# sparisi/pvr_habitat

Hardware: AMD Instinct MI355X
Metric: frames/sec embedded (ResNet50, 256x256) (higher is better)
Workload: dtype f16

## Files before the change

### include/pvr_hip.h

```cpp
#ifndef PVR_HIP_H
#define PVR_HIP_H

#include <stddef.h>
#include <stdint.h>

#ifdef __cplusplus
extern "C" {
#endif

typedef int pvr_status;
#define PVR_OK 0
#define PVR_ERR_INVALID 1
#define PVR_ERR_MISSING_WEIGHT 2
#define PVR_ERR_HIP 3
#define PVR_ERR_STATE 4

#define PVR_BF16 0
#define PVR_F16 1
#define PVR_F32 2

#define PVR_ARCH_RESNET50 0
#define PVR_ARCH_RESNET50_L4 1
#define PVR_ARCH_RESNET50_L3 2
#define PVR_ARCH_CLIP_VIT_B32 3
#define PVR_ARCH_CLIP_VIT_B16 4
#define PVR_ARCH_RANDOM5 6
#define PVR_ARCH_MAE_VIT_L16 7
#define PVR_ARCH_MAE_VIT_H14 8
#define PVR_ARCH_CLIP_RN50 9
#define PVR_ARCH_RESNET18 10
#define PVR_ARCH_RESNET34 11
#define PVR_ARCH_MAE_VIT_B16 5

const char *pvr_version(void);
int32_t pvr_has_experiments(void);
int32_t pvr_debug_stem_u8_geometry_ok(const void *frames, int32_t h, int32_t w, int32_t top, int32_t left);
float pvr_debug_sample_uniform(uint32_t bits);
size_t pvr_last_error(char *buf, size_t cap);

typedef struct pvr_encoder pvr_encoder;

typedef struct pvr_encoder_desc {
    int32_t arch;
    int32_t dtype;
    int32_t max_batch;
    int32_t chunk;
    int32_t resize;
    int32_t crop;
    float mean[3];
    float std_[3];
} pvr_encoder_desc;

pvr_status pvr_encoder_create(const pvr_encoder_desc *desc, pvr_encoder **out);
pvr_status pvr_encoder_load_weights(pvr_encoder *enc, const char *name, const float *host_data,
                                    const int64_t *shape, int32_t ndim);
pvr_status pvr_encoder_finalize(pvr_encoder *enc);
pvr_status pvr_encoder_set_host_backend(pvr_encoder *enc, int32_t on);
int32_t pvr_encoder_out_size(const pvr_encoder *enc);
pvr_status pvr_encoder_forward(pvr_encoder *enc, const uint8_t *frames_dev, int32_t n, int32_t h,
                               int32_t w, float *out_dev, int64_t out_stride, void *hip_stream);
pvr_status pvr_encoder_tap(pvr_encoder *enc, const char *name, float *out_dev, int64_t cap,
                           int64_t *count, void *hip_stream);
pvr_status pvr_encoder_debug_set_fusion(pvr_encoder *enc, int32_t on);
int32_t pvr_encoder_launch_name(const pvr_encoder *enc, int32_t index, char *buf, int32_t cap);
pvr_status pvr_encoder_set_crop_position(pvr_encoder *enc, int32_t pos);
pvr_status pvr_encoder_forward_lane(pvr_encoder *enc, int32_t lane, const uint8_t *frames_dev, int32_t n, int32_t h,
                                    int32_t w, float *out_dev, int64_t out_stride, void *hip_stream);
pvr_status pvr_encoder_set_low_latency(pvr_encoder *enc, int32_t on);
pvr_status pvr_encoder_debug_stop_after(pvr_encoder *enc, const char *tap);
pvr_status pvr_encoder_profile(pvr_encoder *enc, const uint8_t *frames_dev, int32_t n, int32_t h, int32_t w,
                               float *out_dev, int64_t out_stride, void *hip_stream, float *op_ms,
                               double *op_flops, int32_t cap, int32_t *n_ops);
pvr_status pvr_encoder_profile_span(pvr_encoder *enc, const uint8_t *frames_dev, int32_t n, int32_t h, int32_t w, float *out_dev,
                                    int64_t out_stride, void *hip_stream, int32_t first_op, int32_t last_op, float *span_ms);
pvr_status pvr_encoder_check_range(pvr_encoder *enc, const uint8_t *frames_dev, int32_t n, int32_t h, int32_t w, float *out_dev, int64_t out_stride,
                                   void *hip_stream, int32_t *first_bad);
pvr_status pvr_encoder_debug_set_switch(pvr_encoder *enc, const char *name, int32_t value);
int32_t pvr_encoder_launch_kernel(const pvr_encoder *enc, int32_t n, int32_t index, char *buf, int32_t cap);
void pvr_encoder_destroy(pvr_encoder *enc);

pvr_status pvr_op_preprocess(const uint8_t *frames_dev, int32_t n, int32_t h, int32_t w, int32_t resize,
                             int32_t crop, void *out_dev, int32_t dtype, void *hip_stream);
pvr_status pvr_op_stem(const void *img_dev, const void *wgt_dev, const float *bias_dev, void *out_dev,
                       int32_t n, int32_t dtype, void *hip_stream);
pvr_status pvr_op_maxpool(const void *in_dev, void *out_dev, int32_t n, int32_t h, int32_t w, int32_t c,
                          int32_t dtype, void *hip_stream);
pvr_status pvr_op_conv2d(const void *in_dev, const void *wgt_dev, const float *bias_dev,
                         const void *residual_dev, void *out_dev, int32_t n, int32_t h, int32_t w,
                         int32_t cin, int32_t cout, int32_t kh, int32_t kw, int32_t stride, int32_t pad,
                         int32_t relu, int32_t out_f32, int32_t dtype, void *hip_stream);
pvr_status pvr_op_bneck_frame(const void *t1_dev, const void *w2_dev, const float *b2_dev, const void *w3_dev, const float *b3_dev,
                              const void *residual_dev, void *y_dev, void *t2_out_dev, const void *w1n_dev, const float *b1n_dev, void *t1n_dev,
                              const void *w1f_dev, const float *b1f_dev, int32_t n, int32_t phases, int32_t dtype, void *hip_stream);
pvr_status pvr_op_pack_frag_weights(const void *w_dev, void *out_dev, int32_t rows, int32_t k, void *hip_stream);
pvr_status pvr_debug_bneck_frame_stamps(const void *t1_dev, const void *w2_dev, const float *b2_dev, const void *w3_dev, const float *b3_dev,
                                        const void *residual_dev, void *y_dev, const void *w1n_dev, const float *b1n_dev, void *t1n_dev,
                                        const void *w1f_dev, const float *b1f_dev, int32_t n, int32_t dtype, uint64_t *stamps_dev, void *hip_stream);
int64_t pvr_debug_bneck_frame_launches(void);
pvr_status pvr_debug_set_frame64(int32_t mode);
int64_t pvr_debug_bneck_frame64_launches(void);
pvr_status pvr_debug_bneck_frame64_stamps(const void *w1f_dev, const float *b1f_dev, const void *w2_dev, const float *b2_dev, const void *w3_dev, const float *b3_dev,
                                          const void *x_dev, void *y_dev, int32_t n, int32_t dtype, uint64_t *stamps_dev, void *hip_stream);
pvr_status pvr_op_conv_wfrag(const void *in_dev, const void *wgt_packed_dev, const float *bias_dev, const void *residual_dev, void *out_dev, int32_t n,
                             int32_t h, int32_t w, int32_t cin, int32_t cout, int32_t kh, int32_t kw, int32_t stride, int32_t pad, int32_t relu,
                             int32_t out_f32, int32_t dtype, void *hip_stream);
pvr_status pvr_op_conv2d_dual(const void *in_dev, const void *in2_dev, const void *wgt_dev, const float *bias_dev, void *out_dev, int32_t n, int32_t h,
                              int32_t w, int32_t cin, int32_t cout, int32_t kh, int32_t kw, int32_t stride, int32_t pad, int32_t h2, int32_t w2,
                              int32_t cin2, int32_t stride2, int32_t relu, int32_t dtype, void *hip_stream);
pvr_status pvr_op_conv_wfrag_pool(const void *in_dev, const void *wgt_packed_dev, const float *bias_dev, const void *residual_dev, float *pool_out_dev,
                                  int64_t pool_stride, int32_t n, int32_t cin, int32_t cout, int32_t dtype, void *hip_stream);
int64_t pvr_debug_conv_wfrag_launches(void);
pvr_status pvr_op_split16_pack_weights(const float *w_dev, void *out_dev, int32_t rows, int32_t k, void *hip_stream);
pvr_status pvr_op_conv2d_split16(const float *in_dev, const void *wgt_split_dev, const float *bias_dev, const float *residual_dev, float *out_dev, int32_t n,
                                 int32_t h, int32_t w, int32_t cin, int32_t cout, int32_t k, int32_t stride, int32_t pad, int32_t relu, void *hip_stream);
pvr_status pvr_op_conv2d_f32(const float *in_dev, const float *wgt_dev, const float *bias_dev, const float *residual_dev, float *out_dev, int32_t n,
                             int32_t h, int32_t w, int32_t cin, int32_t cout, int32_t k, int32_t stride, int32_t pad, int32_t relu, void *hip_stream);
int64_t pvr_debug_conv_split16_launches(void);
int64_t pvr_debug_chain_wave128_launches(void);
pvr_status pvr_debug_set_stem_regpool(int32_t mode);
pvr_status pvr_debug_set_conv_algo(int32_t algo);
pvr_status pvr_file_sizes(const char *const *paths, int32_t n, int64_t *sizes, int32_t threads);
pvr_status pvr_read_files(const char *const *paths, int32_t n, uint8_t *dst, const int64_t *offsets, int32_t threads);
pvr_status pvr_stage_copy(void *dst, const void *src, int64_t rows, int64_t row_bytes, int64_t src_row_stride, int64_t run_bytes,
                          int64_t run_stride, int32_t threads);
int64_t pvr_png_scratch_bytes(int32_t n, int32_t h, int32_t w);
pvr_status pvr_png_decode(const uint8_t *files_dev, const int64_t *offsets_dev, int32_t n, int32_t h, int32_t w, uint8_t *out_dev,
                          uint8_t *scratch_dev, int64_t scratch_bytes, int32_t *status_dev, void *hip_stream);

int64_t pvr_debug_conv_expand_launches(void);
int64_t pvr_debug_pp_persistent_launches(void);
pvr_status pvr_op_avgpool(const void *in_dev, float *out_dev, int64_t out_stride, int32_t n, int32_t hw,
                          int32_t c, int32_t in_f32, int32_t dtype, void *hip_stream);
pvr_status pvr_op_nonfinite_flag(const float *x_dev, int64_t rows, int64_t cols, int64_t stride, int32_t *flag_dev, void *hip_stream);

pvr_status pvr_debug_convert(const float *src, uint16_t *dst, int64_t n, int32_t dtype);


#ifdef __cplusplus
}
#endif
#endif
```

### pvr_habitat_amd/_lib.py

```python
import ctypes as C
import os

_HERE = os.path.dirname(os.path.abspath(__file__))
LIB_PATH = os.environ.get('PVR_LIB') or os.path.join(_HERE, 'lib', 'libpvr_hip.so')

PVR_BF16, PVR_F16, PVR_F32 = 0, 1, 2
ARCH_RESNET50, ARCH_RESNET50_L4, ARCH_RESNET50_L3 = 0, 1, 2


class EncoderDesc(C.Structure):
    _fields_ = [('arch', C.c_int32), ('dtype', C.c_int32), ('max_batch', C.c_int32), ('chunk', C.c_int32),
                ('resize', C.c_int32), ('crop', C.c_int32), ('mean', C.c_float * 3), ('std_', C.c_float * 3)]


_lib = None

_SIGS = {
    'pvr_version': (C.c_char_p, []),
    'pvr_has_experiments': (C.c_int32, []),
    'pvr_debug_stem_u8_geometry_ok': (C.c_int32, [C.c_void_p, C.c_int32, C.c_int32, C.c_int32, C.c_int32]),
    'pvr_encoder_set_host_backend': (C.c_int, [C.c_void_p, C.c_int32]),
    'pvr_stage_copy': (C.c_int, [C.c_void_p, C.c_void_p, C.c_int64, C.c_int64, C.c_int64, C.c_int64, C.c_int64, C.c_int32]),
    'pvr_last_error': (C.c_size_t, [C.c_char_p, C.c_size_t]),
    'pvr_encoder_create': (C.c_int, [C.POINTER(EncoderDesc), C.POINTER(C.c_void_p)]),
    'pvr_encoder_load_weights': (C.c_int, [C.c_void_p, C.c_char_p, C.c_void_p, C.POINTER(C.c_int64), C.c_int32]),
    'pvr_encoder_finalize': (C.c_int, [C.c_void_p]),
    'pvr_encoder_out_size': (C.c_int32, [C.c_void_p]),
    'pvr_encoder_forward': (C.c_int, [C.c_void_p, C.c_void_p, C.c_int32, C.c_int32, C.c_int32, C.c_void_p, C.c_int64, C.c_void_p]),
    'pvr_encoder_forward_lane': (C.c_int, [C.c_void_p, C.c_int32, C.c_void_p, C.c_int32, C.c_int32, C.c_int32, C.c_void_p, C.c_int64, C.c_void_p]),
    'pvr_debug_set_conv_algo': (C.c_int, [C.c_int32]),
    'pvr_file_sizes': (C.c_int, [C.c_void_p, C.c_int32, C.c_void_p, C.c_int32]),
    'pvr_read_files': (C.c_int, [C.c_void_p, C.c_int32, C.c_void_p, C.c_void_p, C.c_int32]),
    'pvr_png_scratch_bytes': (C.c_int64, [C.c_int32, C.c_int32, C.c_int32]),
    'pvr_png_decode': (C.c_int, [C.c_void_p, C.c_void_p, C.c_int32, C.c_int32, C.c_int32, C.c_void_p, C.c_void_p, C.c_int64, C.c_void_p, C.c_void_p]),
    'pvr_debug_conv_expand_launches': (C.c_int64, []),
    'pvr_debug_pp_persistent_launches': (C.c_int64, []),
    'pvr_encoder_set_crop_position': (C.c_int, [C.c_void_p, C.c_int32]),
    'pvr_encoder_set_low_latency': (C.c_int, [C.c_void_p, C.c_int32]),
    'pvr_encoder_tap': (C.c_int, [C.c_void_p, C.c_char_p, C.c_void_p, C.c_int64, C.POINTER(C.c_int64), C.c_void_p]),
    'pvr_encoder_debug_stop_after': (C.c_int, [C.c_void_p, C.c_char_p]),
    'pvr_encoder_debug_set_fusion': (C.c_int, [C.c_void_p, C.c_int32]),
    'pvr_encoder_launch_name': (C.c_int32, [C.c_void_p, C.c_int32, C.c_char_p, C.c_int32]),
    'pvr_encoder_destroy': (None, [C.c_void_p]),
    'pvr_encoder_profile': (C.c_int, [C.c_void_p, C.c_void_p, C.c_int32, C.c_int32, C.c_int32, C.c_void_p, C.c_int64, C.c_void_p,
                                      C.c_void_p, C.c_void_p, C.c_int32, C.POINTER(C.c_int32)]),
    'pvr_encoder_profile_span': (C.c_int, [C.c_void_p, C.c_void_p, C.c_int32, C.c_int32, C.c_int32, C.c_void_p, C.c_int64, C.c_void_p, C.c_int32, C.c_int32,
                                           C.POINTER(C.c_float)]),
    'pvr_op_preprocess': (C.c_int, [C.c_void_p, C.c_int32, C.c_int32, C.c_int32, C.c_int32, C.c_int32, C.c_void_p, C.c_int32, C.c_void_p]),
    'pvr_op_stem': (C.c_int, [C.c_void_p, C.c_void_p, C.c_void_p, C.c_void_p, C.c_int32, C.c_int32, C.c_void_p]),
    'pvr_op_maxpool': (C.c_int, [C.c_void_p, C.c_void_p, C.c_int32, C.c_int32, C.c_int32, C.c_int32, C.c_int32, C.c_void_p]),
    'pvr_op_conv2d': (C.c_int, [C.c_void_p, C.c_void_p, C.c_void_p, C.c_void_p, C.c_void_p] + [C.c_int32] * 12 + [C.c_void_p]),
    'pvr_op_avgpool': (C.c_int, [C.c_void_p, C.c_void_p, C.c_int64, C.c_int32, C.c_int32, C.c_int32, C.c_int32, C.c_int32, C.c_void_p]),
    'pvr_debug_convert': (C.c_int, [C.c_void_p, C.c_void_p, C.c_int64, C.c_int32]),
    'pvr_op_bneck_frame': (C.c_int, [C.c_void_p] * 13 + [C.c_int32] * 3 + [C.c_void_p]),
    'pvr_debug_bneck_frame_launches': (C.c_int64, []),
    'pvr_debug_set_frame64': (C.c_int, [C.c_int32]),
    'pvr_debug_bneck_frame64_launches': (C.c_int64, []),
    'pvr_debug_bneck_frame64_stamps': (C.c_int, [C.c_void_p] * 8 + [C.c_int32] * 2 + [C.c_void_p] * 2),
    'pvr_op_conv_wfrag': (C.c_int, [C.c_void_p] * 5 + [C.c_int32] * 12 + [C.c_void_p]),
    'pvr_debug_conv_wfrag_launches': (C.c_int64, []),
    'pvr_op_conv_wfrag_pool': (C.c_int, [C.c_void_p] * 5 + [C.c_int64] + [C.c_int32] * 4 + [C.c_void_p]),
    'pvr_op_conv2d_dual': (C.c_int, [C.c_void_p] * 5 + [C.c_int32] * 15 + [C.c_void_p]),
    'pvr_op_pack_frag_weights': (C.c_int, [C.c_void_p, C.c_void_p, C.c_int32, C.c_int32, C.c_void_p]),
    'pvr_debug_bneck_frame_stamps': (C.c_int, [C.c_void_p] * 12 + [C.c_int32] * 2 + [C.c_void_p] * 2),
    'pvr_encoder_check_range': (C.c_int, [C.c_void_p, C.c_void_p, C.c_int32, C.c_int32, C.c_int32, C.c_void_p, C.c_int64, C.c_void_p, C.POINTER(C.c_int32)]),
    'pvr_encoder_debug_set_switch': (C.c_int, [C.c_void_p, C.c_char_p, C.c_int32]),
    'pvr_encoder_launch_kernel': (C.c_int32, [C.c_void_p, C.c_int32, C.c_int32, C.c_char_p, C.c_int32]),
    'pvr_op_split16_pack_weights': (C.c_int, [C.c_void_p, C.c_void_p, C.c_int32, C.c_int32, C.c_void_p]),
    'pvr_op_conv2d_split16': (C.c_int, [C.c_void_p] * 5 + [C.c_int32] * 9 + [C.c_void_p]),
    'pvr_op_conv2d_f32': (C.c_int, [C.c_void_p] * 5 + [C.c_int32] * 9 + [C.c_void_p]),
    'pvr_debug_conv_split16_launches': (C.c_int64, []),
    'pvr_debug_set_stem_regpool': (C.c_int, [C.c_int32]),
    'pvr_debug_chain_wave128_launches': (C.c_int64, []),
    'pvr_op_nonfinite_flag': (C.c_int, [C.c_void_p, C.c_int64, C.c_int64, C.c_int64, C.c_void_p, C.c_void_p]),
}


def lib():
    global _lib
    if _lib is None:
        if not os.path.isfile(LIB_PATH):
            raise RuntimeError('libpvr_hip.so not found at %s: build it with `make -C pvr_habitat_amd/csrc` '
                               '(there is no CPU fallback for the HIP path)' % LIB_PATH)
        l = C.CDLL(LIB_PATH)
        for name, (res, args) in _SIGS.items():
            if not hasattr(l, name):
                continue
            f = getattr(l, name)
            f.restype, f.argtypes = res, args
        _lib = l
    return _lib


def last_error():
    buf = C.create_string_buffer(1024)
    lib().pvr_last_error(buf, 1024)
    return buf.value.decode(errors='replace')


def check(status):
    if status != 0:
        raise RuntimeError('libpvr_hip: %s (status %d)' % (last_error(), status))


def stream_ptr():
    import torch
    return C.c_void_p(torch.cuda.current_stream().cuda_stream)


def require_gpu():
    import torch
    if not torch.cuda.is_available():
        raise RuntimeError('pvr_habitat_amd needs an MI355X (gfx950) visible to PyTorch-ROCm; there is no CPU path')
```

### pvr_habitat_amd/csrc/api.hip

```cpp
#include <stdarg.h>
#include "common.h"
#include "sample_rng.h"
#include <dlfcn.h>

namespace pvr {

static thread_local std::string g_err;

void set_error(const char *fmt, ...) {
    char buf[1024];
    va_list ap;
    va_start(ap, fmt);
    vsnprintf(buf, sizeof buf, fmt, ap);
    va_end(ap);
    g_err = buf;
}
const std::string &last_error() { return g_err; }

namespace {
typedef int (*roctx_push_fn)(const char *);
typedef int (*roctx_pop_fn)();
struct Roctx {
    roctx_push_fn push = nullptr;
    roctx_pop_fn pop = nullptr;
    Roctx() {
        const char *e = getenv("PVR_ROCTX");
        if (!e || atoi(e) == 0) return;
        for (const char *name : {"librocprofiler-sdk-roctx.so", "librocprofiler-sdk-roctx.so.1", "libroctx64.so", "libroctx64.so.4"}) {
            if (void *h = dlopen(name, RTLD_NOW | RTLD_GLOBAL)) {
                push = (roctx_push_fn)dlsym(h, "roctxRangePushA");
                pop = (roctx_pop_fn)dlsym(h, "roctxRangePop");
                if (push && pop) return;
                push = nullptr; pop = nullptr;
            }
        }
    }
};
const Roctx &roctx() { static Roctx r; return r; }
}
void trace_push(const char *name) { if (roctx().push) roctx().push(name); }
void trace_pop() { if (roctx().pop) roctx().pop(); }

pvr_status launch_preprocess(const uint8_t *, int, int, int, int, int, void *, int, hipStream_t, int crop_pos = 0);
pvr_status launch_stem(const void *, const void *, const float *, void *, int, int, int, hipStream_t);
pvr_status launch_maxpool(const void *, void *, int, int, int, int, int, hipStream_t);
pvr_status launch_avgpool(const void *, float *, int64_t, int, int, int, int, int, hipStream_t);
bool stem_pool_u8_ok(const void *, int, int, int, int);
pvr_status launch_conv(const void *, const void *, const float *, const void *, void *, const void *, int, int, int, int,
                       int, int, int, int, int, int, int, int, hipStream_t);

void set_conv_algo(int a);
long long conv_expand_launches();
long long bneck_frame_launches();
pvr_status launch_pack_frag_weights(const void *w, void *out, int rows, int K, hipStream_t stream);
pvr_status launch_bneck_frame(const void *t1, const void *w2, const float *b2, const void *w3, const float *b3, const void *res, void *y,
                              void *t2_out, int n, int phases, int dtype, hipStream_t stream, unsigned long long *stamps = nullptr,
                              const void *w1np = nullptr, const float *b1n = nullptr, void *t1n = nullptr, const void *w1fp = nullptr, const float *b1f = nullptr);
pvr_status launch_bneck_frame64(const void *w1p, const float *b1, const void *w2p, const float *b2, const void *w3p, const float *b3, const void *x, void *y, int n,
                                int dtype, hipStream_t stream, unsigned long long *stamps);
void set_frame64(int mode);
long long bneck_frame64_launches();
long long pp_persistent_launches();
pvr_status launch_conv_pp256(const void *in, const void *wgt, const float *bias, const void *res, void *out, int n, int h, int w, int cin,
                             int cout, int kh, int kw, int stride, int pad, int act, int out_f32, int res_f32, int dtype, int bm, hipStream_t stream,
                             const void *in2 = nullptr, int h2 = 0, int w2 = 0, int cin2 = 0, int stride2 = 1);
long long conv_wfrag_launches();
pvr_status launch_conv_wfrag(const void *in, const void *wp, const float *bias, const void *res, void *out, int n, int h, int w, int cin, int cout,
                             int kh, int kw, int stride, int pad, int act, int out_f32, int dtype, hipStream_t stream, float *pool_out = nullptr,
                             int64_t pool_stride = 0);

void set_stem_regpool(int v);
long long conv_split16_launches();
long long chain_wave128_launches();
pvr_status launch_split16_pack(const float *w, void *out, int rows, int K, hipStream_t stream);
pvr_status launch_conv_split16(const float *in, const void *wsp, const float *bias, const float *res, float *out, int n, int h, int w, int cin,
                               int cout, int k, int stride, int pad, int relu, hipStream_t stream, float *out2 = nullptr, int n1 = 0, void *out16 = nullptr,
                               int terms = 3);
pvr_status launch_conv_f32(const float *, const float *, const float *, const float *, float *, int, int, int, int, int, int, int, int, int, hipStream_t);

static void *g_zero = nullptr;
static pvr_status zero_page(void **out) {
    if (!g_zero) {
        PVR_HIP_TRY(hipMalloc(&g_zero, 256));
        PVR_HIP_TRY(hipMemset(g_zero, 0, 256));
        PVR_HIP_TRY(hipDeviceSynchronize());
    }
    *out = g_zero;
    return PVR_OK;
}

}

using namespace pvr;

extern "C" {

const char *pvr_version(void) { return "pvr_hip 0.1.0 (gfx950)"; }

int64_t pvr_debug_conv_expand_launches(void) { return (int64_t)conv_expand_launches(); }
int64_t pvr_debug_bneck_frame_launches(void) { return (int64_t)bneck_frame_launches(); }
pvr_status pvr_op_pack_frag_weights(const void *w, void *out, int32_t rows, int32_t k, void *stream) {
    return launch_pack_frag_weights(w, out, rows, k, (hipStream_t)stream);
}

pvr_status pvr_op_bneck_frame(const void *t1, const void *w2, const float *b2, const void *w3, const float *b3, const void *residual, void *y,
                              void *t2_out, const void *w1n, const float *b1n, void *t1n, const void *w1f, const float *b1f, int32_t n, int32_t phases,
                              int32_t dtype, void *stream) {
    PVR_REQUIRE(n > 0 && n <= 1300, "pvr_op_bneck_frame: n must be 1..1300");
    return launch_bneck_frame(t1, w2, b2, w3, b3, residual, y, t2_out, n, phases, dtype, (hipStream_t)stream, nullptr, w1n, b1n, t1n, w1f, b1f);
}
pvr_status pvr_debug_bneck_frame_stamps(const void *t1, const void *w2, const float *b2, const void *w3, const float *b3, const void *residual, void *y,
                                        const void *w1n, const float *b1n, void *t1n, const void *w1f, const float *b1f, int32_t n, int32_t dtype,
                                        uint64_t *stamps_dev, void *stream) {
    PVR_REQUIRE(stamps_dev && n > 8, "pvr_debug_bneck_frame_stamps: needs a stamp buffer and more than 8 frames");
    return launch_bneck_frame(t1, w2, b2, w3, b3, residual, y, nullptr, n, (w1n ? 7 : 3) | (w1f ? 8 : 0), dtype, (hipStream_t)stream, (unsigned long long *)stamps_dev,
                              w1n, b1n, t1n, w1f, b1f);
}
pvr_status pvr_debug_set_frame64(int32_t mode) {
    PVR_REQUIRE(mode >= -1 && mode <= 1, "pvr_debug_set_frame64: -1 (environment: PVR_FRAME64, default off), 0 or 1");
    set_frame64(mode);
    return PVR_OK;
}
int64_t pvr_debug_bneck_frame64_launches(void) { return (int64_t)bneck_frame64_launches(); }
pvr_status pvr_debug_bneck_frame64_stamps(const void *w1f, const float *b1f, const void *w2, const float *b2, const void *w3, const float *b3, const void *x, void *y,
                                          int32_t n, int32_t dtype, uint64_t *stamps_dev, void *stream) {
    PVR_REQUIRE(stamps_dev && n > 8, "pvr_debug_bneck_frame64_stamps: needs a stamp buffer and more than 8 frames");
    return launch_bneck_frame64(w1f, b1f, w2, b2, w3, b3, x, y, n, dtype, (hipStream_t)stream, (unsigned long long *)stamps_dev);
}
pvr_status pvr_op_conv_wfrag(const void *in, const void *wgt_packed, const float *bias, const void *residual, void *out, int32_t n, int32_t h, int32_t w,
                             int32_t cin, int32_t cout, int32_t kh, int32_t kw, int32_t stride, int32_t pad, int32_t relu, int32_t out_f32, int32_t dtype,
                             void *stream) {
    PVR_REQUIRE(n > 0 && h > 0 && w > 0, "pvr_op_conv_wfrag: empty input");
    return launch_conv_wfrag(in, wgt_packed, bias, residual, out, n, h, w, cin, cout, kh, kw, stride, pad, relu, out_f32, dtype, (hipStream_t)stream);
}
pvr_status pvr_op_conv2d_dual(const void *in, const void *in2, const void *wgt, const float *bias, void *out, int32_t n, int32_t h, int32_t w, int32_t cin,
                              int32_t cout, int32_t kh, int32_t kw, int32_t stride, int32_t pad, int32_t h2, int32_t w2, int32_t cin2, int32_t stride2,
                              int32_t relu, int32_t dtype, void *stream) {
    PVR_REQUIRE(in && in2 && wgt && bias && out && n > 0, "pvr_op_conv2d_dual: null argument");
    PVR_REQUIRE(dtype == PVR_BF16 || dtype == PVR_F16, "pvr_op_conv2d_dual: 16-bit storage types only");
    return launch_conv_pp256(in, wgt, bias, nullptr, out, n, h, w, cin, cout, kh, kw, stride, pad, relu, 0, 0, dtype, 224, (hipStream_t)stream, in2, h2, w2,
                             cin2, stride2);
}
pvr_status pvr_op_conv_wfrag_pool(const void *in, const void *wgt_packed, const float *bias, const void *residual, float *pool_out, int64_t pool_stride,
                                  int32_t n, int32_t cin, int32_t cout, int32_t dtype, void *stream) {
    PVR_REQUIRE(n > 0 && pool_out, "pvr_op_conv_wfrag_pool: empty input");
    return launch_conv_wfrag(in, wgt_packed, bias, residual, nullptr, n, 7, 7, cin, cout, 1, 1, 1, 0, 1, 1, dtype, (hipStream_t)stream, pool_out, pool_stride);
}
int64_t pvr_debug_conv_wfrag_launches(void) { return (int64_t)conv_wfrag_launches(); }
pvr_status pvr_op_split16_pack_weights(const float *w, void *out, int32_t rows, int32_t k, void *stream) {
    return launch_split16_pack(w, out, rows, k, (hipStream_t)stream);
}
pvr_status pvr_op_conv2d_split16(const float *in, const void *wgt_split, const float *bias, const float *residual, float *out, int32_t n, int32_t h,
                                 int32_t w, int32_t cin, int32_t cout, int32_t k, int32_t stride, int32_t pad, int32_t relu, void *stream) {
    PVR_REQUIRE(n > 0 && h > 0 && w > 0, "pvr_op_conv2d_split16: empty input");
    return launch_conv_split16(in, wgt_split, bias, residual, out, n, h, w, cin, cout, k, stride, pad, relu, (hipStream_t)stream);
}
pvr_status pvr_op_conv2d_f32(const float *in, const float *wgt, const float *bias, const float *residual, float *out, int32_t n, int32_t h, int32_t w,
                             int32_t cin, int32_t cout, int32_t k, int32_t stride, int32_t pad, int32_t relu, void *stream) {
    PVR_REQUIRE(in && wgt && bias && out && n > 0, "pvr_op_conv2d_f32: null argument");
    return launch_conv_f32(in, wgt, bias, residual, out, n, h, w, cin, cout, k, stride, pad, relu, (hipStream_t)stream);
}
int64_t pvr_debug_conv_split16_launches(void) { return (int64_t)conv_split16_launches(); }
pvr_status pvr_debug_set_stem_regpool(int32_t mode) {
    PVR_REQUIRE(mode >= -1 && mode <= 1, "pvr_debug_set_stem_regpool: -1 (environment: PVR_STEM_REGPOOL, default on), 0 (LDS-tile pooling) or 1 (register pooling)");
    set_stem_regpool(mode);
    return PVR_OK;
}
int64_t pvr_debug_chain_wave128_launches(void) { return (int64_t)chain_wave128_launches(); }
int64_t pvr_debug_pp_persistent_launches(void) { return (int64_t)pp_persistent_launches(); }

size_t pvr_last_error(char *buf, size_t cap) {
    const std::string &e = last_error();
    if (buf && cap) {
        size_t n = e.size() < cap - 1 ? e.size() : cap - 1;
        memcpy(buf, e.data(), n);
        buf[n] = 0;
    }
    return e.size();
}

pvr_status pvr_op_preprocess(const uint8_t *frames, int32_t n, int32_t h, int32_t w, int32_t resize, int32_t crop,
                             void *out, int32_t dtype, void *stream) {
    PVR_REQUIRE(frames && out, "pvr_op_preprocess: null pointer");
    hipStream_t st = (hipStream_t)stream;
    PVR_HIP_TRY(hipMemsetAsync(out, 0, (size_t)n * (crop + 6) * (crop + 8) * 4 * 2, st));
    return launch_preprocess(frames, n, h, w, resize, crop, out, dtype, st);
}

pvr_status pvr_op_stem(const void *img, const void *wgt, const float *bias, void *out, int32_t n, int32_t dtype,
                       void *stream) {
    PVR_REQUIRE(img && wgt && bias && out, "pvr_op_stem: null pointer");
    return launch_stem(img, wgt, bias, out, n, 224, dtype, (hipStream_t)stream);
}

pvr_status pvr_op_maxpool(const void *in, void *out, int32_t n, int32_t h, int32_t w, int32_t c, int32_t dtype,
                          void *stream) {
    PVR_REQUIRE(in && out, "pvr_op_maxpool: null pointer");
    return launch_maxpool(in, out, n, h, w, c, dtype, (hipStream_t)stream);
}

pvr_status pvr_op_conv2d(const void *in, const void *wgt, const float *bias, const void *residual, void *out, int32_t n,
                         int32_t h, int32_t w, int32_t cin, int32_t cout, int32_t kh, int32_t kw, int32_t stride,
                         int32_t pad, int32_t relu, int32_t out_f32, int32_t dtype, void *stream) {
    PVR_REQUIRE(in && wgt && bias && out, "pvr_op_conv2d: null pointer");
    void *z;
    pvr_status s = zero_page(&z);
    if (s) return s;
    return launch_conv(in, wgt, bias, residual, out, z, n, h, w, cin, cout, kh, kw, stride, pad, relu, out_f32, dtype,
                       (hipStream_t)stream);
}

pvr_status pvr_debug_set_conv_algo(int32_t algo) {
    PVR_REQUIRE(algo >= -1 && algo <= 4, "pvr_debug_set_conv_algo: algo must be -1 (auto), 0 (conv_igemm), 1 / 2 / 3 (conv_pp256 with 256- / 128- / 224-pixel tiles), 4 (conv_w4)");
#ifndef PVR_EXPERIMENTS
    PVR_REQUIRE(algo != 4, "pvr_debug_set_conv_algo: conv_w4 is an experiment kernel; this library was built without it (make EXPERIMENTS=1)");
#endif
    set_conv_algo(algo);
    return PVR_OK;
}

pvr_status pvr_op_avgpool(const void *in, float *out, int64_t out_stride, int32_t n, int32_t hw, int32_t c, int32_t in_f32,
                          int32_t dtype, void *stream) {
    PVR_REQUIRE(in && out, "pvr_op_avgpool: null pointer");
    return launch_avgpool(in, out, out_stride, n, hw, c, in_f32, dtype, (hipStream_t)stream);
}

__global__ __launch_bounds__(256) void nonfinite_flag_kernel(const float *x, long long rows, long long cols, long long stride, int *flag) {
    const long long n = rows * cols;
    bool bad = false;
    for (long long i = (long long)blockIdx.x * 256 + threadIdx.x; i < n; i += (long long)gridDim.x * 256) {
        const float v = x[(i / cols) * stride + (i % cols)];
        bad |= (__builtin_bit_cast(unsigned, v) & 0x7f800000u) == 0x7f800000u;
    }
    if (__builtin_amdgcn_ballot_w64(bad) != 0 && (threadIdx.x & 63) == 0) atomicOr(flag, 1);
}

pvr_status pvr_op_nonfinite_flag(const float *x, int64_t rows, int64_t cols, int64_t stride, int32_t *flag, void *stream) {
    PVR_REQUIRE(x && flag && rows >= 0 && cols > 0 && stride >= cols, "pvr_op_nonfinite_flag: bad argument");
    if (rows == 0) return PVR_OK;
    const long long n = rows * cols;
    const int blocks = (int)((n + 255) / 256 < 2048 ? (n + 255) / 256 : 2048);
    hipLaunchKernelGGL(nonfinite_flag_kernel, dim3(blocks), dim3(256), 0, (hipStream_t)stream, x, (long long)rows, (long long)cols, (long long)stride, flag);
    PVR_LAUNCH_CHECK();
    return PVR_OK;
}

int32_t pvr_debug_stem_u8_geometry_ok(const void *frames, int32_t h, int32_t w, int32_t top, int32_t left) { return stem_pool_u8_ok(frames, h, w, top, left) ? 1 : 0; }

float pvr_debug_sample_uniform(uint32_t bits) { return pvr::uniform_open01(bits); }

int32_t pvr_has_experiments(void) {
#ifdef PVR_EXPERIMENTS
    return 1;
#else
    return 0;
#endif
}

pvr_status pvr_debug_convert(const float *src, uint16_t *dst, int64_t n, int32_t dtype) {
    PVR_REQUIRE(src && dst, "pvr_debug_convert: null pointer");
    for (int64_t i = 0; i < n; ++i) dst[i] = f32_to_h(src[i], dtype);
    return PVR_OK;
}

}
```

### pvr_habitat_amd/csrc/bottleneck_chain.hip

```cpp
#include "chain_params.h"

namespace pvr {


__device__ __forceinline__ void ch_dma16(__amdgpu_buffer_rsrc_t rs, char *lds, int voff, int soff) {
    __builtin_amdgcn_raw_ptr_buffer_load_lds(rs, (__attribute__((address_space(3))) void *)lds, 16, voff, soff, 0, 0);
}

#ifdef CHAIN_STAMP
__device__ unsigned long long chain_stamps[8192][12];
#define CH_T(i_) { if (threadIdx.x == 0) ch_tt[i_] = __builtin_amdgcn_s_memrealtime(); }
#else
#define CH_T(i_)
#endif

#ifndef CH_KNOCK
#define CH_KNOCK 0
#endif
template <int AUX = 0>
__device__ __forceinline__ void store_b128_imm(u32x4 v, __amdgpu_buffer_rsrc_t rs, int voff, int imm) {
    if constexpr (!(CH_KNOCK & 1)) __builtin_amdgcn_raw_buffer_store_b128(v, rs, voff + imm, 0, AUX);
}

template <int CM, int CMN, bool F16, int RD, int OCC, bool HALO, bool DS = false, int PFK = -1>
// ... 273 lines not shown
        for (int j = 0; j < TM; ++j) {
            const int row = wm * 64 + j * 16 + fr;
            const f32x4 a = acc2[i][j];
            const unsigned lo = pack2_h<F16>(fmaxf(a[0] + bv.x, 0.f), fmaxf(a[1] + bv.y, 0.f));
            const unsigned hi = pack2_h<F16>(fmaxf(a[2] + bv.z, 0.f), fmaxf(a[3] + bv.w, 0.f));
            const int cc = c & 63;
            char *dst = smem + T2_OFF + (c >> 6) * 16384 + row * 128 + ((((cc >> 3) ^ ((row >> 1) & 7))) << 4) + (cc & 4) * 2;
            *reinterpret_cast<uint2 *>(dst) = make_uint2(lo, hi);
        }
    }
#pragma unroll
    for (int i = 0; i < W3_CH; ++i) *reinterpret_cast<u32x4 *>(smem + W3_L(i)) = w3r[i];
    if constexpr (CMN > 0) {
#pragma unroll
        for (int i = 0; i < W1_CH; ++i) *reinterpret_cast<u32x4 *>(smem + W1_L(i)) = w1r[i];
    }
    if (G > 1) {
#pragma unroll
        for (int i = 0; i < W3_CH; ++i)
            w3r[i] = __builtin_bit_cast(u32x4, __builtin_amdgcn_raw_buffer_load_b128(rs_w3, W3_G(i), 64 * CM * 2, 0));
        if constexpr (CMN > 0) {
#pragma unroll
            for (int i = 0; i < W1_CH; ++i) w1r[i] = __builtin_bit_cast(u32x4, __builtin_amdgcn_raw_buffer_load_b128(rs_w1, W1_G(i), 128, 0));
        }
    }
    __syncthreads();
    CH_T(3);

    int w3_rd[2][2], w1_rd[2][CMN ? TN1 : 1], yg_wr[TM];
#pragma unroll
    for (int ks = 0; ks < 2; ++ks) {
#pragma unroll
        for (int t = 0; t < 2; ++t) {
            const int row = wn * 32 + t * 16 + fr;
            w3_rd[ks][t] = W3_OFF + row * 128 + (((ks * 4 + fq) ^ ((row >> 1) & 7)) << 4);
        }
        if constexpr (CMN > 0) {
#pragma unroll
            for (int i = 0; i < TN1; ++i) {
                const int row = wn * (CMN / 2) + i * 16 + fr;
                w1_rd[ks][i] = W1_OFF + row * 128 + (((ks * 4 + fq) ^ ((row >> 1) & 7)) << 4);
            }
        }
    }
#pragma unroll
    for (int j = 0; j < TM; ++j) {
        const int row = wm * 64 + j * 16 + fr;
        yg_wr[j] = YG_OFF + row * 128 + (((wn * 4 + fq) ^ ((row >> 1) & 7)) << 4);
    }
    f32x4 acc1[CMN ? TN1 : 1][TM];
    if constexpr (CMN > 0) {
#pragma unroll
        for (int i = 0; i < TN1; ++i)
#pragma unroll
            for (int j = 0; j < TM; ++j) acc1[i][j] = f32x4{0.f, 0.f, 0.f, 0.f};
    }

#pragma unroll
    for (int g = 0; g < G; ++g) {
        if (g == 1) CH_T(6);
        f32x4 acc3[2][TM];
#pragma unroll
        for (int t = 0; t < 2; ++t)
#pragma unroll
            for (int j = 0; j < TM; ++j) acc3[t][j] = f32x4{0.f, 0.f, 0.f, 0.f};
#pragma unroll
        for (int s = 0; s < KS3; ++s)
#pragma unroll
            for (int ks = 0; ks < 2; ++ks) {
                V8 xa[TM], wb[2];
#pragma unroll
                for (int j = 0; j < TM; ++j) xa[j] = *reinterpret_cast<const V8 *>(smem + T2_OFF + s * 16384 + x_rd[ks][j]);
#pragma unroll
                for (int t = 0; t < 2; ++t) wb[t] = *reinterpret_cast<const V8 *>(smem + s * 8192 + w3_rd[ks][t]);
#pragma unroll
                for (int t = 0; t < 2; ++t)
#pragma unroll
                    for (int j = 0; j < TM; ++j) acc3[t][j] = mfma16<F16>(wb[t], xa[j], acc3[t][j]);
            }
        if constexpr (DS) {
#pragma unroll
            for (int ks = 0; ks < 2; ++ks)
#pragma unroll
                for (int t = 0; t < 2; ++t)
#pragma unroll
                    for (int j = 0; j < TM; ++j) acc3[t][j] = mfma16<F16>(wdr[t][ks], xd[ks][j], acc3[t][j]);
            if (g + 1 < G) {
#pragma unroll
                for (int t = 0; t < 2; ++t)
#pragma unroll
                    for (int ks = 0; ks < 2; ++ks)
                        wdr[t][ks] = __builtin_bit_cast(V8, __builtin_amdgcn_raw_buffer_load_b128(rs_wd, wd_off[t] + ks * 64, (g + 1) * 8192, 0));
            }
        }
        if (g == 1) CH_T(7);
        const int c0 = g * 64 + wn * 32 + fq * 8;
        const float4 bA = *reinterpret_cast<const float4 *>(p.b3 + c0), bB = *reinterpret_cast<const float4 *>(p.b3 + c0 + 4);
#pragma unroll
        for (int j = 0; j < TM; ++j) {
            const f32x4 lo = acc3[0][j], hi = acc3[1][j];
            float v[8] = {lo[0] + bA.x, lo[1] + bA.y, lo[2] + bA.z, lo[3] + bA.w, hi[0] + bB.x, hi[1] + bB.y, hi[2] + bB.z, hi[3] + bB.w};
            u32x4 o;
            if constexpr (DS) {
#pragma unroll
                for (int e = 0; e < 4; ++e)
                    o[e] = pack2_h<F16>(fmaxf(v[2 * e], 0.f), fmaxf(v[2 * e + 1], 0.f));
            } else {
                const u32x4 r = rres[g % RD][j];
#pragma unroll
                for (int e = 0; e < 4; ++e) {
                    const float v0 = fmaxf(v[2 * e] + from_h<F16>((u16)(r[e] & 0xffffu)), 0.f);
                    const float v1 = fmaxf(v[2 * e + 1] + from_h<F16>((u16)(r[e] >> 16)), 0.f);
                    o[e] = pack2_h<F16>(v0, v1);
                }
            }
            if (p.y_blk) store_b128_imm<PVR_NT_AUX(4)>(o, rs_y, Y_OFF(j) + g * y_gs, 0);
            else store_b128_imm(o, rs_y, Y_OFF(j) + g * y_gs, 0);
            if constexpr (CMN > 0) *reinterpret_cast<u32x4 *>(smem + yg_wr[j]) = o;
        }
        if (!DS && g + RD < G) {
#pragma unroll
            for (int j = 0; j < TM; ++j)
                rres[g % RD][j] = __builtin_bit_cast(u32x4, __builtin_amdgcn_raw_buffer_load_b128(rs_res, (CH_KNOCK & 2) ? OOB : R_OFF(j), (g + RD) * r_gs, DS ? 0 : PVR_NT_AUX(16)));
        }
        if (g == 1) CH_T(8);
        __syncthreads();
        if (g == 1) CH_T(9);
        if (g + 1 < G) {
#pragma unroll
            for (int i = 0; i < W3_CH; ++i) *reinterpret_cast<u32x4 *>(smem + W3_L(i)) = w3r[i];
            if (g + 2 < G) {
#pragma unroll
                for (int i = 0; i < W3_CH; ++i)
                    w3r[i] = __builtin_bit_cast(u32x4, __builtin_amdgcn_raw_buffer_load_b128(rs_w3, W3_G(i), (g + 2) * (64 * CM * 2), 0));
            }
        }
        if (g == 1) CH_T(10);
        if constexpr (CMN == 0) __syncthreads();
        if constexpr (CMN > 0) {
#pragma unroll
            for (int ks = 0; ks < 2; ++ks) {
                V8 xa[TM], wb[TN1];
#pragma unroll
                for (int j = 0; j < TM; ++j) xa[j] = *reinterpret_cast<const V8 *>(smem + YG_OFF + x_rd[ks][j]);
#pragma unroll
                for (int i = 0; i < TN1; ++i) wb[i] = *reinterpret_cast<const V8 *>(smem + w1_rd[ks][i]);
#pragma unroll
                for (int i = 0; i < TN1; ++i)
#pragma unroll
                    for (int j = 0; j < TM; ++j) acc1[i][j] = mfma16<F16>(wb[i], xa[j], acc1[i][j]);
            }
            __syncthreads();
            if (g == 1) CH_T(11);
            if (g + 1 < G) {
#pragma unroll
                for (int i = 0; i < W1_CH; ++i) *reinterpret_cast<u32x4 *>(smem + W1_L(i)) = w1r[i];
                if (g + 2 < G) {
#pragma unroll
                    for (int i = 0; i < W1_CH; ++i)
                        w1r[i] = __builtin_bit_cast(u32x4, __builtin_amdgcn_raw_buffer_load_b128(rs_w1, W1_G(i), (g + 2) * 128, 0));
                }
            }
        }
    }

    CH_T(4);
    if constexpr (CMN > 0) {
#pragma unroll
        for (int q = 0; q < TN1 / 2; ++q) {
            const int c0 = wn * (CMN / 2) + q * 32 + fq * 8;
            const float4 bA = *reinterpret_cast<const float4 *>(p.b1n + c0), bB = *reinterpret_cast<const float4 *>(p.b1n + c0 + 4);
#pragma unroll
            for (int j = 0; j < TM; ++j) {
                const f32x4 lo = acc1[2 * q][j], hi = acc1[2 * q + 1][j];
                const float v[8] = {lo[0] + bA.x, lo[1] + bA.y, lo[2] + bA.z, lo[3] + bA.w, hi[0] + bB.x, hi[1] + bB.y, hi[2] + bB.z, hi[3] + bB.w};
                u32x4 o;
#pragma unroll
                for (int e = 0; e < 4; ++e)
                    o[e] = pack2_h<F16>(fmaxf(v[2 * e], 0.f), fmaxf(v[2 * e + 1], 0.f));
                if (p.t_blk) store_b128_imm<0>(o, rs_t, T_OFF(j) + q * 1024, 0);
                else store_b128_imm<PVR_NT_AUX(8)>(o, rs_t, T_OFF(j), q * 64);
            }
        }
    }
#undef PVR_PHASE_B_PREFETCH
#undef W3_G
#undef W3_L
#undef W1_G
#undef W1_L
#undef Y_OFF
#undef R_OFF
#undef T_OFF
#ifdef CHAIN_STAMP
    CH_T(5);
    if (threadIdx.x == 0 && blockIdx.x < 8192) { _Pragma("unroll") for (int k = 0; k < 12; ++k) chain_stamps[blockIdx.x][k] = ch_tt[k]; }
#endif
}

template <int CM, int CMN, bool F16, int RD, int OCC, bool HALO, bool DS = false, int PFK = -1>
static pvr_status launch_chain_one(ChainP &p, hipStream_t stream) {
    const int grid = (p.M + 127) / 128;
    const size_t pipe = HALO ? (size_t)(CM / 64) * (CM == 64 ? 256 : 192) * 128 + (size_t)2 * CM * 128 : (size_t)2 * (128 + CM) * 128;
    const size_t phase_b = (CM / 64) * 16384 + 16384 + (CM / 64) * 8192 + CMN * 128;
    const size_t lds = phase_b <= pipe ? pipe : phase_b;
    static DeviceOnce attr_done;
    if (attr_done.needed()) {
        PVR_HIP_TRY(hipFuncSetAttribute((const void *)bottleneck_chain_kernel<CM, CMN, F16, RD, OCC, HALO, DS, PFK>,
                                        hipFuncAttributeMaxDynamicSharedMemorySize, (int)lds));
        attr_done.mark();
    }
    hipLaunchKernelGGL((bottleneck_chain_kernel<CM, CMN, F16, RD, OCC, HALO, DS, PFK>), dim3(grid), dim3(256), lds, stream, p);
    PVR_LAUNCH_CHECK();
    return PVR_OK;
}

static bool chain_halo_enabled() {
    static int v = -1;
    if (v < 0) { const char *e = getenv("PVR_CHAIN_HALO"); v = e ? atoi(e) : 1; }
    return v != 0;
}

static int chain_ds_occ() {
    static int v = -1;
    if (v < 0) { const char *e = getenv("PVR_CHAIN_DS_OCC"); v = e ? atoi(e) : 3; }
    return v;
}

static int chain_pfk() {
    static int v = -2;
    if (v < -1) { const char *e = getenv("PVR_CHAIN_PFK"); v = e ? atoi(e) : 12; }
    return v;
}

template <int CM, int CMN, bool F16, int RD, int OCC, bool DS = false>
static pvr_status launch_chain_inst(ChainP &p, hipStream_t stream) {
    const bool halo = p.stride == 1 && 128 + 2 * p.W + 2 <= (CM == 64 ? 256 : 192) - 1 && chain_halo_enabled();
    if constexpr (DS) {
        if (halo) return chain_ds_occ() == 3 ? launch_chain_one<CM, CMN, F16, RD, 3, true, true>(p, stream) : launch_chain_one<CM, CMN, F16, RD, 2, true, true>(p, stream);
        return launch_chain_one<CM, CMN, F16, RD, 2, false, true>(p, stream);
    } else {
        if (halo) {
            if constexpr (CM == 128) {
                if (chain_pfk() == 12) return launch_chain_one<CM, CMN, F16, RD, 2, true, false, 12>(p, stream);
            }
            return launch_chain_one<CM, CMN, F16, RD, (CM == 64 ? OCC : 2), true>(p, stream);
        }
        return launch_chain_one<CM, CMN, F16, RD, OCC, false>(p, stream);
    }
}

static int chain_cfg() {
    static int v = -1;
    if (v < 0) { const char *e = getenv("PVR_CHAIN_CFG"); v = e ? atoi(e) : 12; }
    return v;
}

template <bool F16>
static pvr_status launch_chain_dt(ChainP &p, int cm, int cmn, hipStream_t stream) {
    if (p.xds) {
        if (cm == 64 && cmn == 64) return launch_chain_inst<64, 64, F16, 1, 2, true>(p, stream);
        set_error("bottleneck chain with downsample: no instance for Cm=%d, next Cm=%d", cm, cmn);
        return PVR_ERR_INVALID;
    }
    const int cfg = chain_cfg();
#define PVR_CHAIN64(CMN_)                                                                 \
    switch (cfg) {                                                                        \
    case 12: return launch_chain_inst<64, CMN_, F16, 1, 2>(p, stream);                    \
    case 13: return launch_chain_inst<64, CMN_, F16, 1, 3>(p, stream);                    \
    case 22: return launch_chain_inst<64, CMN_, F16, 2, 2>(p, stream);                    \
    case 23: return launch_chain_inst<64, CMN_, F16, 2, 3>(p, stream);                    \
    default: return launch_chain_inst<64, CMN_, F16, 4, 2>(p, stream);                    \
    }
    if (cm == 64 && cmn == 64) PVR_CHAIN64(64)
    if (cm == 64 && cmn == 128) {
        if (cfg / 10 == 1) return launch_chain_inst<64, 128, F16, 1, 2>(p, stream);
        if (cfg / 10 == 2) return launch_chain_inst<64, 128, F16, 2, 2>(p, stream);
        return launch_chain_inst<64, 128, F16, 4, 2>(p, stream);
    }
    if (cm == 64 && cmn == 0) PVR_CHAIN64(0)
#undef PVR_CHAIN64
    if (cm == 128 && cmn == 128) return launch_chain_inst<128, 128, F16, 1, 2>(p, stream);
    if (cm == 128 && cmn == 0) return launch_chain_inst<128, 0, F16, 1, 2>(p, stream);
    set_error("bottleneck chain: no instance for Cm=%d, next Cm=%d", cm, cmn);
    return PVR_ERR_INVALID;
}

static bool chain_wave_enabled() {
    const char *e = getenv("PVR_CHAIN_WAVE");
    return !e || atoi(e) != 0;
}

bool chain_uses_wave_form(int cm, int cmn, int stride, bool ds) { return chain_wave_enabled() && chain_wave_supported(cm, cmn, stride, ds); }

bool chain_uses_wave128(int cm, int cmn, int stride, int64_t M) { return chain_wave_enabled() && chain_wave128_supported(cm, cmn, stride, M); }

bool chain_ds_supported(int cm, int cmn, int cin, int stride) { return cm == 64 && cmn == 64 && cin == 64 && stride == 1; }
bool chain_supported(int cm, int cmn) { return (cm == 64 && (cmn == 0 || cmn == 64 || cmn == 128)) || (cm == 128 && (cmn == 0 || cmn == 128)); }

int chain_row_source(int row) { return (row & ~31) + 8 * ((row >> 2) & 3) + 4 * ((row >> 4) & 1) + (row & 3); }

pvr_status launch_bottleneck_chain(const void *t1, const void *w2, const float *b2, const void *w3p, const float *b3, const void *res,
                                   void *y, const void *w1np, const float *b1n, void *t1n, int n, int h, int w, int cm, int cmn,
                                   int stride, int dtype, hipStream_t stream, const void *xds, const void *wdsp, const void *w3pb, const void *wdspb,
                                   int wave, int in_blk, int out_blk, const void *wpk) {
    PVR_REQUIRE(chain_supported(cm, cmn), "bottleneck chain: unsupported widths Cm=%d next=%d", cm, cmn);
    PVR_REQUIRE(t1 && w2 && b2 && w3p && b3 && (res || xds) && y && (cmn == 0 || (w1np && b1n && t1n)), "bottleneck chain: null argument");
    PVR_REQUIRE(!xds || (wdsp && chain_ds_supported(cm, cmn, 64, stride)), "bottleneck chain with downsample: unsupported shape");
    ChainP p;
    p.in = (const u16 *)t1; p.w2 = (const u16 *)w2; p.w3 = (const u16 *)w3p; p.w1n = (const u16 *)w1np; p.res = (const u16 *)res;
    p.b2 = b2; p.b3 = b3; p.b1n = b1n; p.y = (u16 *)y; p.t1n = (u16 *)t1n;
    p.N = n; p.H = h; p.W = w; p.stride = stride;
    p.Ho = (h + 2 - 3) / stride + 1; p.Wo = (w + 2 - 3) / stride + 1;
    const int64_t M = (int64_t)n * p.Ho * p.Wo;
    const int64_t inb = (int64_t)n * h * w * cm * 2, yb = M * 4 * cm * 2, tb = M * (cmn ? cmn : 1) * 2;
    PVR_REQUIRE(inb < 0x7ffffff0ll && yb < 0x7ffffff0ll && tb < 0x7ffffff0ll, "bottleneck chain: operand larger than 2 GiB (use a smaller chunk)");
    p.M = (int)M; p.in_bytes = (unsigned)inb; p.y_bytes = (unsigned)yb; p.t1n_bytes = (unsigned)tb;
    p.xds = (const u16 *)xds; p.wds = (const u16 *)wdsp;
    p.xds_bytes = xds ? (unsigned)(M * 64 * 2) : 0; p.wds_bytes = xds ? (unsigned)(4 * cm * 64 * 2) : 0;
    p.w2_bytes = (unsigned)(cm * 9 * cm * 2); p.w3_bytes = (unsigned)(4 * cm * cm * 2); p.w1n_bytes = (unsigned)(cmn * 4 * cm * 2);
    if (wave == 2) {
        PVR_REQUIRE(chain_wave128_supported(cm, cmn, stride, M) && !xds, "bottleneck chain: no layer2 wave form for Cm=%d next=%d stride=%d", cm, cmn, stride);
        p.wpk = (const u16 *)wpk; p.in_blk = in_blk; p.out_blk = out_blk & 1;
        return launch_chain_wave128(p, cmn, dtype, stream);
    }
    if (wave) {
        PVR_REQUIRE(chain_wave_supported(cm, cmn, stride, xds != nullptr), "bottleneck chain: no wave form for Cm=%d next=%d stride=%d", cm, cmn, stride);
        p.w3b = (const u16 *)w3pb; p.wdsb = (const u16 *)wdspb; p.in_blk = in_blk; p.out_blk = out_blk;
        return launch_chain_wave(p, cmn, dtype, stream);
    }
    PVR_REQUIRE(!(in_blk || out_blk) || M % 16 == 0, "bottleneck chain: the blocked layout needs a multiple of 16 pixels");
    p.res_blk = xds ? 0 : in_blk; p.y_blk = out_blk & 1;
    p.t_blk = (out_blk & 2) && cmn > 0;
    return dtype == PVR_F16 ? launch_chain_dt<true>(p, cm, cmn, stream) : launch_chain_dt<false>(p, cm, cmn, stream);
}

}
```

### pvr_habitat_amd/csrc/chain_params.h

```cpp
#pragma once
#include "common.h"

namespace pvr {

struct ChainP {
    const u16 *in, *w2, *w3, *w1n, *res;
    const float *b2, *b3, *b1n;
    u16 *y, *t1n;
    int N, H, W, Ho, Wo, stride, M;
    unsigned in_bytes, w2_bytes, w3_bytes, w1n_bytes, y_bytes, t1n_bytes;
    const u16 *xds = nullptr, *wds = nullptr;
    unsigned xds_bytes = 0, wds_bytes = 0;
    int in_blk = 0, out_blk = 0;
    int res_blk = 0, y_blk = 0;
    const u16 *w3b = nullptr, *wdsb = nullptr;
    const u16 *wpk = nullptr;
    unsigned wpk_bytes = 0;
    int t_blk = 0;
};

bool chain_supported(int cm, int cmn);
bool chain_ds_supported(int cm, int cmn, int cin, int stride);
bool chain_uses_wave_form(int cm, int cmn, int stride, bool ds);
int chain_row_source(int row);
pvr_status launch_bottleneck_chain(const void *t1, const void *w2, const float *b2, const void *w3p, const float *b3, const void *res,
                                   void *y, const void *w1np, const float *b1n, void *t1n, int n, int h, int w, int cm, int cmn,
                                   int stride, int dtype, hipStream_t stream, const void *xds = nullptr, const void *wdsp = nullptr,
                                   const void *w3pb = nullptr, const void *wdspb = nullptr, int wave = 0, int in_blk = 0, int out_blk = 0,
                                   const void *wpk = nullptr);


bool chain_wave_supported(int cm, int cmn, int stride, bool ds);
bool chain_wave_blocked_ok(int cmn_first, int h, int w);
bool chain_wave_halo_enabled();
pvr_status launch_chain_wave(ChainP &p, int cmn, int dtype, hipStream_t stream);

bool chain_wave128_supported(int cm, int cmn, int stride, int64_t M);
bool chain_uses_wave128(int cm, int cmn, int stride, int64_t M);
size_t chain_wave128_pack_bytes();
pvr_status launch_chain_wave128_pack(const void *w2, const void *w3p, const void *w1np, void *out, hipStream_t stream);
pvr_status launch_chain_wave128(ChainP &p, int cmn, int dtype, hipStream_t stream);

}
```

### pvr_habitat_amd/csrc/chain_wave.hip

```cpp
#include "chain_params.h"

namespace pvr {

__device__ __forceinline__ int cw_row_source(int row) { return (row & ~31) + 8 * ((row >> 2) & 3) + 4 * ((row >> 4) & 1) + (row & 3); }

#ifndef CW_KNOCK
#define CW_KNOCK 0
#endif
#ifndef CW_AUX_ST
#define CW_AUX_ST PVR_NT_AUX(1)
#endif
#ifndef CW_AUX_RES
#define CW_AUX_RES PVR_NT_AUX(2)
#endif
template <int AUX = CW_AUX_ST>
__device__ __forceinline__ void cw_store(u32x4 v, __amdgpu_buffer_rsrc_t rs, int voff, int imm, int never = 0) {
    if constexpr (CW_KNOCK & 1) { if (never) __builtin_amdgcn_raw_buffer_store_b128(v, rs, voff + imm, 0, AUX); }
    else __builtin_amdgcn_raw_buffer_store_b128(v, rs, voff + imm, 0, AUX);
}
#ifndef CW_AUX_T1
#define CW_AUX_T1 CW_AUX_ST
#endif

typedef float cw_f32x2 __attribute__((ext_vector_type(2)));
typedef __bf16 cw_bf16x2 __attribute__((ext_vector_type(2)));
typedef _Float16 cw_f16x2 __attribute__((ext_vector_type(2)));
template <bool F16> __device__ __forceinline__ unsigned cw_pack2(float a, float b) {
    const cw_f32x2 v = {a, b};
    if constexpr (F16) return __builtin_bit_cast(unsigned, __builtin_convertvector(v, cw_f16x2));
    else return __builtin_bit_cast(unsigned, __builtin_convertvector(v, cw_bf16x2));
}

__device__ __forceinline__ u32x4 cw_m2f(char *slot, int lane, int foff, u32x4 v) {
    *reinterpret_cast<u32x4 *>(slot + lane * 16) = v;
    return *reinterpret_cast<const u32x4 *>(slot + foff);
}
__device__ __forceinline__ void cw_f2m_pair(char *slot, int lane, u32x4 even, u32x4 odd, u32x4 &lo, u32x4 &hi) {
    const int fr = lane & 15, fq = lane >> 4, base = fr * 128, sw = fr & 7;
    *reinterpret_cast<u32x4 *>(slot + base + ((fq ^ sw) << 4)) = even;
    *reinterpret_cast<u32x4 *>(slot + base + (((4 + fq) ^ sw) << 4)) = odd;
    lo = *reinterpret_cast<const u32x4 *>(slot + lane * 16);
    hi = *reinterpret_cast<const u32x4 *>(slot + 1024 + lane * 16);
}

__device__ __forceinline__ unsigned cw_row_shift(unsigned lo, unsigned hi, int d) {
#define CW_SH(D_) case D_: { const int a_ = __builtin_amdgcn_update_dpp(0, (int)lo, 0x100 + D_, 0xf, 0xf, true); \
                             return (unsigned)__builtin_amdgcn_update_dpp(a_, (int)hi, 0x110 + (16 - D_), 0xf, 0xf, false); }
    switch (d) {
        CW_SH(1) CW_SH(2) CW_SH(3) CW_SH(4) CW_SH(5) CW_SH(6) CW_SH(7) CW_SH(8) CW_SH(9) CW_SH(10) CW_SH(11) CW_SH(12) CW_SH(13) CW_SH(14) CW_SH(15)
        default: return lo;
    }
#undef CW_SH
}

struct CwTile {
    int xb[2];
    int mk[2];
    int yi[2];
    int yo[2];
    int to[2];
    int hb;
    int xs[2];
};

template <int CMN, bool INB, bool OUTB>
__device__ __forceinline__ void cw_setup(CwTile &a, int m0, int lane, int M, int H, int W) {
    const int fr = lane & 15, fq = lane >> 4, lp = lane >> 2, lc = (lane & 3) ^ ((lane >> 3) & 3);
    a.hb = ((m0 >> 4) - 4) * 2048 + fq * 256 + fr * 16;
#pragma unroll
    for (int j = 0; j < 2; ++j) {
        const int m = m0 + 16 * j + (INB ? fr : lp);
        const bool ok = m < M;
        const int mm = ok ? m : 0;
        const int wo = mm % W, ho = (mm / W) % H;
        int hb = 0, wb = 0;
#pragma unroll
        for (int t3 = 0; t3 < 3; ++t3) {
            hb |= (int)(ok && (unsigned)(ho - 1 + t3) < (unsigned)H) << t3;
            wb |= (int)((unsigned)(wo - 1 + t3) < (unsigned)W) << t3;
        }
        int mask = 0;
#pragma unroll
        for (int t3 = 0; t3 < 3; ++t3) mask |= ((hb >> t3) & 1) ? (wb << (t3 * 3)) : 0;
        a.mk[j] = mask;
        a.xb[j] = INB ? m : m * 128 + lc * 16;
        a.xs[j] = (m0 + 16 * j + lp) * 128 + lc * 16;
        const int blk = (m0 >> 4) + j;
        a.yi[j] = INB ? blk * 8192 + fq * 256 + fr * 16 : (m0 + 16 * j + lp) * 512 + lc * 16;
        a.yo[j] = OUTB ? blk * 8192 + fq * 256 + fr * 16 : (m0 + 16 * j + (lane >> 3)) * 512 + (((lane & 7) ^ (lane >> 3)) << 4);
        a.to[j] = OUTB ? blk * (CMN * 32) + fq * 256 + fr * 16 : (m0 + 16 * j + (lane >> 3)) * (CMN * 2) + (((lane & 7) ^ (lane >> 3)) << 4);
    }
}

template <int CMN, bool F16, bool DS, bool W3G, bool INB, bool OUTB, bool HALO, int XD, int RD, int WD>
__global__ __launch_bounds__(512, 2) void chain_wave_kernel(ChainP p) {
    typedef typename HT<F16>::V8 V8;
    constexpr int WW = 56, HB = 10;
    constexpr int NH = 8, NK = 18;
    constexpr int TN1 = CMN / 16;
    constexpr int W2L = 0, W3L = 73728, W1L = W3G ? 73728 : 73728 + 32768;
    constexpr int B2L = W1L + CMN * 512, B3L = B2L + 256, B1L = B3L + 1024, SCR = B1L + 512;
    constexpr int OOB = 0x7ffffff0;
    constexpr int YH = INB ? 1024 : 64;
    static_assert(XD >= 1 && XD <= NK && RD >= 1 && RD <= NH && NH % RD == 0 && WD >= 1 && WD <= NH, "prefetch depths (the residual ring must close over a tile)");
    static_assert(!HALO || INB, "the halo form reads the blocked layout");
    extern __shared__ __attribute__((aligned(16))) char smem[];

    const int tid = threadIdx.x, lane = tid & 63, wave = tid >> 6, fr = lane & 15, fq = lane >> 4;
    const int foff = fr * 64 + ((fq ^ ((fr >> 1) & 3)) << 4);
    char *const slot0 = smem + SCR + wave * 2048, *const slot1 = slot0 + 1024;
    const auto rs_in = __builtin_amdgcn_make_buffer_rsrc(const_cast<u16 *>(p.in), 0, p.in_bytes, 0x00020000);
    const auto rs_w2 = __builtin_amdgcn_make_buffer_rsrc(const_cast<u16 *>(p.w2), 0, p.w2_bytes, 0x00020000);
    const auto rs_w3 = __builtin_amdgcn_make_buffer_rsrc(const_cast<u16 *>(p.w3), 0, p.w3_bytes, 0x00020000);
    const auto rs_w1 = __builtin_amdgcn_make_buffer_rsrc(const_cast<u16 *>(p.w1n), 0, p.w1n_bytes, 0x00020000);
    const auto rs_res = __builtin_amdgcn_make_buffer_rsrc(const_cast<u16 *>(DS ? p.xds : p.res), 0, DS ? p.xds_bytes : p.y_bytes, 0x00020000);
    const auto rs_wd = __builtin_amdgcn_make_buffer_rsrc(const_cast<u16 *>(DS ? p.wdsb : p.w3b), 0, DS ? p.wds_bytes : p.w3_bytes, 0x00020000);
    const auto rs_y = __builtin_amdgcn_make_buffer_rsrc(p.y, 0, p.y_bytes, 0x00020000);
    const auto rs_t = __builtin_amdgcn_make_buffer_rsrc(p.t1n, 0, p.t1n_bytes, 0x00020000);

#pragma unroll
    for (int q = 0; q < 9; ++q) {
        const int r = tid >> 3, c = tid & 7;
        const u32x4 v = __builtin_bit_cast(u32x4, __builtin_amdgcn_raw_buffer_load_b128(rs_w2, (cw_row_source(r) * 576 + c * 8) * 2, q * 128, 0));
        *reinterpret_cast<u32x4 *>(smem + W2L + q * 8192 + r * 128 + ((c ^ ((r >> 1) & 7)) << 4)) = v;
    }
    if constexpr (!W3G) {
#pragma unroll
        for (int q = 0; q < 4; ++q) {
            const int idx = tid + 512 * q, r = idx >> 3, c = idx & 7;
            const u32x4 v = __builtin_bit_cast(u32x4, __builtin_amdgcn_raw_buffer_load_b128(rs_w3, idx * 16, 0, 0));
            *reinterpret_cast<u32x4 *>(smem + W3L + r * 128 + ((c ^ ((r >> 1) & 7)) << 4)) = v;
        }
    }
    if constexpr (CMN > 0) {
#pragma unroll
        for (int q = 0; q < CMN * 32 / 512; ++q) {
            const int idx = tid + 512 * q, r = idx >> 5, c32 = idx & 31;
            const u32x4 v = __builtin_bit_cast(u32x4, __builtin_amdgcn_raw_buffer_load_b128(rs_w1, idx * 16, 0, 0));
            *reinterpret_cast<u32x4 *>(smem + W1L + (c32 >> 3) * (CMN * 128) + r * 128 + (((c32 & 7) ^ ((r >> 1) & 7)) << 4)) = v;
        }
    }
    if (tid < 64) *reinterpret_cast<float *>(smem + B2L + tid * 4) = p.b2[tid];
    if (tid < 256) *reinterpret_cast<float *>(smem + B3L + tid * 4) = p.b3[tid];
    if constexpr (CMN > 0) { if (tid < CMN) *reinterpret_cast<float *>(smem + B1L + tid * 4) = p.b1n[tid]; }
    __syncthreads();

    const int nch = (p.M + 255) >> 8, cx = (nch + 7) >> 3, L = gridDim.x >> 3;
    const int xcd = blockIdx.x & 7, c_end = min((xcd + 1) * cx, nch);
    int chunk = xcd * cx + (blockIdx.x >> 3);
    if (chunk >= c_end) return;

    int lb0 = fr * 128 + ((fq ^ ((fr >> 1) & 7)) << 4), lb1 = lb0 ^ 64;
    const int Wb = p.W * 128;

    CwTile cur, nxt;
    cw_setup<CMN, INB, OUTB>(cur, chunk * 256 + wave * 32, lane, p.M, p.H, p.W);

    u32x4 xr[HALO ? 1 : XD][2];
    u32x4 xh[HALO ? HB : 1][2];
    u32x4 rres[DS ? 1 : RD][2];
    V8 xd[2][2];
    u32x4 wg[(W3G || DS) ? WD : 1][2][2];
#define CW_ISSUE_X(slot_, kt_, A_)                                                                                      \
    {                                                                                                                   \
        const int tp_ = (kt_) >> 1;                                                                                     \
        _Pragma("unroll") for (int j = 0; j < 2; ++j) {                                                                 \
            int vo_;                                                                                                    \
            if constexpr (INB) {                                   \
                const int pm_ = A_.xb[j] + (tp_ / 3 - 1) * p.W + (tp_ % 3 - 1);                                         \
                vo_ = (pm_ >> 4) * 2048 + (pm_ & 15) * 16 + (((kt_) & 1) * 4 + fq) * 256;                               \
            } else vo_ = A_.xb[j] + (tp_ / 3 - 1) * Wb + (tp_ % 3 - 1) * 128 + ((kt_) & 1) * 64;                        \
            vo_ = ((A_.mk[j] >> tp_) & 1) ? vo_ : OOB;                                                                  \
            if constexpr (CW_KNOCK & 4) vo_ = OOB;                                                                      \
            xr[slot_][j] = __builtin_bit_cast(u32x4, __builtin_amdgcn_raw_buffer_load_b128(rs_in, vo_, 0, 0));          \
        }                                                                                                               \
    }
#define CW_ISSUE_HALO(A_)                                                                                               \
    {                                                                                                                   \
        _Pragma("unroll") for (int k = 0; k < HB; ++k)                                                                  \
            _Pragma("unroll") for (int ks = 0; ks < 2; ++ks)                                                            \
                xh[k][ks] = __builtin_bit_cast(u32x4, __builtin_amdgcn_raw_buffer_load_b128(rs_in, (CW_KNOCK & 4) ? OOB : A_.hb + k * 2048 + ks * 1024, 0, 0)); \
    }
#define CW_FRAG(dst_, kt_, j_)                                                                                          \
    {                                                                                                                   \
        const int tp_ = (kt_) >> 1, ks_ = (kt_) & 1, o_ = 64 + 16 * (j_) + (tp_ / 3 - 1) * WW + tp_ % 3 - 1, k0_ = o_ >> 4, d_ = o_ & 15; \
        const bool in_ = (cur.mk[j_] >> tp_) & 1;                                                                       \
        _Pragma("unroll") for (int e = 0; e < 4; ++e) {                                                                 \
            const unsigned v_ = cw_row_shift(xh[k0_][ks_][e], xh[k0_ + 1 < HB ? k0_ + 1 : k0_][ks_][e], d_);            \
            dst_[e] = in_ ? v_ : 0u;                                                                                    \
        }                                                                                                               \
    }
#define CW_ISSUE_RES(slot_, h_, A_)                                                                                     \
    {                                                                                                                   \
        _Pragma("unroll") for (int j = 0; j < 2; ++j)                                                                   \
            rres[slot_][j] = __builtin_bit_cast(u32x4, __builtin_amdgcn_raw_buffer_load_b128(rs_res, (CW_KNOCK & 2) ? OOB : A_.yi[j], (h_) * YH, CW_AUX_RES)); \
    }
#define CW_ISSUE_WG(slot_, h_)                                                                                          \
    {                                                                                                                   \
        _Pragma("unroll") for (int t = 0; t < 2; ++t)                                                                   \
            _Pragma("unroll") for (int ks = 0; ks < 2; ++ks)                                                            \
                wg[slot_][t][ks] = __builtin_bit_cast(u32x4, __builtin_amdgcn_raw_buffer_load_b128(rs_wd, wg_off + t * 2048 + ks * 1024, (h_) * 4096, 0)); \
    }
    const int wg_off = fq * 256 + fr * 16;

    if constexpr (HALO) CW_ISSUE_HALO(cur)
    else {
#pragma unroll
        for (int k = 0; k < XD; ++k) CW_ISSUE_X(k, k, cur);
    }
    if constexpr (!DS) {
#pragma unroll
        for (int d = 0; d < RD; ++d) CW_ISSUE_RES(d, d, cur);
    }

    for (;;) {
        const int chunk_n = chunk + L;
        const bool more = chunk_n < c_end;
        asm volatile("" : "+v"(lb0), "+v"(lb1));

        u32x4 xdr[2][2];
        if constexpr (DS) {
#pragma unroll
            for (int ks = 0; ks < 2; ++ks)
#pragma unroll
                for (int j = 0; j < 2; ++j)
                    xdr[ks][j] = __builtin_bit_cast(u32x4, __builtin_amdgcn_raw_buffer_load_b128(rs_res, cur.xs[j], ks * 64, 0));
        }

        f32x4 acc2[4][2];
#pragma unroll
        for (int i = 0; i < 4; ++i)
#pragma unroll
            for (int j = 0; j < 2; ++j) acc2[i][j] = f32x4{0.f, 0.f, 0.f, 0.f};
        u32x4 xc[2], xn[2];
        if constexpr (HALO) { CW_FRAG(xc[0], 0, 0); CW_FRAG(xc[1], 0, 1); }
        else {
#pragma unroll
            for (int j = 0; j < 2; ++j) xc[j] = INB ? xr[0][j] : cw_m2f(j ? slot1 : slot0, lane, foff, xr[0][j]);
            if (XD < NK) CW_ISSUE_X(0, XD, cur);
        }
#pragma unroll
        for (int kt = 0; kt < NK; ++kt) {
            if (kt + 1 < NK) {
                if constexpr (HALO) { CW_FRAG(xn[0], kt + 1, 0); CW_FRAG(xn[1], kt + 1, 1); }
                else {
#pragma unroll
                    for (int j = 0; j < 2; ++j) xn[j] = INB ? xr[(kt + 1) % XD][j] : cw_m2f(j ? slot1 : slot0, lane, foff, xr[(kt + 1) % XD][j]);
                    if (kt + 1 + XD < NK) CW_ISSUE_X((kt + 1) % XD, kt + 1 + XD, cur);
                }
            }
            const char *wbase = smem + W2L + (kt >> 1) * 8192 + ((kt & 1) ? lb1 : lb0);
            V8 wb[4];
#pragma unroll
            for (int i = 0; i < 4; ++i) wb[i] = *reinterpret_cast<const V8 *>(wbase + i * 2048);
#pragma unroll
            for (int i = 0; i < 4; ++i) {
                acc2[i][0] = mfma16<F16>(wb[i], __builtin_bit_cast(V8, xc[0]), acc2[i][0]);
                acc2[i][1] = mfma16<F16>(wb[i], __builtin_bit_cast(V8, xc[1]), acc2[i][1]);
            }
            if (kt + 1 < NK) { xc[0] = xn[0]; xc[1] = xn[1]; }
            __builtin_amdgcn_sched_barrier(0);
        }
        u32x4 t2[2][2];
#pragma unroll
        for (int q = 0; q < 2; ++q) {
            const float4 bA = *reinterpret_cast<const float4 *>(smem + B2L + (32 * q + 8 * fq) * 4);
            const float4 bB = *reinterpret_cast<const float4 *>(smem + B2L + (32 * q + 8 * fq + 4) * 4);
#pragma unroll
            for (int j = 0; j < 2; ++j) {
                const f32x4 lo = acc2[2 * q][j], hi = acc2[2 * q + 1][j];
                const float v[8] = {lo[0] + bA.x, lo[1] + bA.y, lo[2] + bA.z, lo[3] + bA.w, hi[0] + bB.x, hi[1] + bB.y, hi[2] + bB.z, hi[3] + bB.w};
                u32x4 o;
#pragma unroll
                for (int e = 0; e < 4; ++e)
                    o[e] = cw_pack2<F16>(fmaxf(v[2 * e], 0.f), fmaxf(v[2 * e + 1], 0.f));
                t2[q][j] = o;
            }
        }

        cw_setup<CMN, INB, OUTB>(nxt, more ? chunk_n * 256 + wave * 32 : ((p.M + 31) & ~31), lane, p.M, p.H, p.W);
        if (!more) nxt.hb = OOB;
        if constexpr (HALO) CW_ISSUE_HALO(nxt)
        else {
#pragma unroll
            for (int k = 0; k < XD; ++k) CW_ISSUE_X(k, k, nxt);
        }
        if constexpr (W3G || DS) {
#pragma unroll
            for (int d = 0; d < WD; ++d) CW_ISSUE_WG(d, d);
        }
        if constexpr (DS) {
#pragma unroll
            for (int ks = 0; ks < 2; ++ks)
#pragma unroll
                for (int j = 0; j < 2; ++j) xd[ks][j] = __builtin_bit_cast(V8, cw_m2f(j ? slot1 : slot0, lane, foff, xdr[ks][j]));
        }

        f32x4 acc1[CMN ? TN1 : 1][2];
        if constexpr (CMN > 0) {
#pragma unroll
            for (int i = 0; i < TN1; ++i)
#pragma unroll
                for (int j = 0; j < 2; ++j) acc1[i][j] = f32x4{0.f, 0.f, 0.f, 0.f};
        }
        u32x4 oe[2];
#pragma unroll
        for (int h = 0; h < NH; ++h) {
            u32x4 rp[2], wp[2][2];
            if constexpr (!DS) {
#pragma unroll
                for (int j = 0; j < 2; ++j) rp[j] = INB ? rres[h % RD][j] : cw_m2f(j ? slot1 : slot0, lane, foff, rres[h % RD][j]);
                if (h + RD < NH) CW_ISSUE_RES(h % RD, h + RD, cur)
                else CW_ISSUE_RES(h % RD, h + RD - NH, nxt)
            }
            if constexpr (W3G || DS) {
#pragma unroll
                for (int t = 0; t < 2; ++t)
#pragma unroll
                    for (int ks = 0; ks < 2; ++ks) wp[t][ks] = wg[h % WD][t][ks];
                if (h + WD < NH) CW_ISSUE_WG(h % WD, h + WD);
            }
            f32x4 acc3[2][2];
#pragma unroll
            for (int t = 0; t < 2; ++t)
#pragma unroll
                for (int j = 0; j < 2; ++j) acc3[t][j] = f32x4{0.f, 0.f, 0.f, 0.f};
#pragma unroll
            for (int ks = 0; ks < 2; ++ks) {
                V8 wb[2];
#pragma unroll
                for (int t = 0; t < 2; ++t) {
                    if constexpr (W3G) wb[t] = __builtin_bit_cast(V8, wp[t][ks]);
                    else wb[t] = *reinterpret_cast<const V8 *>(smem + W3L + h * 4096 + t * 2048 + (ks ? lb1 : lb0));
                }
#pragma unroll
                for (int t = 0; t < 2; ++t)
#pragma unroll
                    for (int j = 0; j < 2; ++j) acc3[t][j] = mfma16<F16>(wb[t], __builtin_bit_cast(V8, t2[ks][j]), acc3[t][j]);
            }
            if constexpr (DS) {
#pragma unroll
                for (int ks = 0; ks < 2; ++ks)
#pragma unroll
                    for (int t = 0; t < 2; ++t)
#pragma unroll
                        for (int j = 0; j < 2; ++j) acc3[t][j] = mfma16<F16>(__builtin_bit_cast(V8, wp[t][ks]), xd[ks][j], acc3[t][j]);
            }
            const float4 bA = *reinterpret_cast<const float4 *>(smem + B3L + (32 * h + 8 * fq) * 4);
            const float4 bB = *reinterpret_cast<const float4 *>(smem + B3L + (32 * h + 8 * fq + 4) * 4);
            u32x4 o[2];
#pragma unroll
            for (int j = 0; j < 2; ++j) {
                const f32x4 lo = acc3[0][j], hi = acc3[1][j];
                const float v[8] = {lo[0] + bA.x, lo[1] + bA.y, lo[2] + bA.z, lo[3] + bA.w, hi[0] + bB.x, hi[1] + bB.y, hi[2] + bB.z, hi[3] + bB.w};
                if constexpr (DS) {
#pragma unroll
                    for (int e = 0; e < 4; ++e)
                        o[j][e] = cw_pack2<F16>(fmaxf(v[2 * e], 0.f), fmaxf(v[2 * e + 1], 0.f));
                } else {
                    const u32x4 r = rp[j];
#pragma unroll
                    for (int e = 0; e < 4; ++e) {
                        const float v0 = fmaxf(v[2 * e] + from_h<F16>((u16)(r[e] & 0xffffu)), 0.f);
                        const float v1 = fmaxf(v[2 * e + 1] + from_h<F16>((u16)(r[e] >> 16)), 0.f);
                        o[j][e] = cw_pack2<F16>(v0, v1);
                    }
                }
            }
#pragma unroll
            for (int j = 0; j < 2; ++j) {
                if constexpr (OUTB) cw_store(o[j], rs_y, cur.yo[j], h * 1024, p.stride == 77);
                else if (h & 1) {
                    u32x4 lo, hi;
                    cw_f2m_pair(slot0, lane, oe[j], o[j], lo, hi);
                    cw_store(lo, rs_y, cur.yo[j], (h >> 1) * 128, p.stride == 77);
                    cw_store(hi, rs_y, cur.yo[j], (h >> 1) * 128 + 8 * 512, p.stride == 77);
                } else oe[j] = o[j];
            }
            if constexpr (CMN > 0) {
#pragma unroll
                for (int i = 0; i < TN1; ++i) {
                    const V8 wb = *reinterpret_cast<const V8 *>(smem + W1L + (h >> 1) * (CMN * 128) + i * 2048 + ((h & 1) ? lb1 : lb0));
#pragma unroll
                    for (int j = 0; j < 2; ++j) acc1[i][j] = mfma16<F16>(wb, __builtin_bit_cast(V8, o[j]), acc1[i][j]);
                }
            }
            __builtin_amdgcn_sched_barrier(0);
        }

        if constexpr (CMN > 0) {
            u32x4 te[2];
#pragma unroll
            for (int q = 0; q < TN1 / 2; ++q) {
                const float4 bA = *reinterpret_cast<const float4 *>(smem + B1L + (32 * q + 8 * fq) * 4);
                const float4 bB = *reinterpret_cast<const float4 *>(smem + B1L + (32 * q + 8 * fq + 4) * 4);
#pragma unroll
                for (int j = 0; j < 2; ++j) {
                    const f32x4 lo = acc1[2 * q][j], hi = acc1[2 * q + 1][j];
                    const float v[8] = {lo[0] + bA.x, lo[1] + bA.y, lo[2] + bA.z, lo[3] + bA.w, hi[0] + bB.x, hi[1] + bB.y, hi[2] + bB.z, hi[3] + bB.w};
                    u32x4 o;
#pragma unroll
                    for (int e = 0; e < 4; ++e) o[e] = cw_pack2<F16>(fmaxf(v[2 * e], 0.f), fmaxf(v[2 * e + 1], 0.f));
                    if constexpr (OUTB) cw_store<CW_AUX_T1>(o, rs_t, cur.to[j], q * 1024, p.stride == 77);
                    else if (q & 1) {
                        u32x4 l0, l1;
                        cw_f2m_pair(slot0, lane, te[j], o, l0, l1);
                        cw_store<CW_AUX_T1>(l0, rs_t, cur.to[j], (q >> 1) * 128, p.stride == 77);
                        cw_store<CW_AUX_T1>(l1, rs_t, cur.to[j], (q >> 1) * 128 + 8 * (CMN * 2), p.stride == 77);
                    } else te[j] = o;
                }
            }
        }
        if (!more) break;
        cur = nxt;
        chunk = chunk_n;
    }
#undef CW_ISSUE_X
#undef CW_ISSUE_HALO
#undef CW_FRAG
#undef CW_ISSUE_RES
#undef CW_ISSUE_WG
}

static int cw_num_cus() {
    static int v = 0;
    if (!v) {
        int dev = 0, n = 0;
        if (hipGetDevice(&dev) == hipSuccess && hipDeviceGetAttribute(&n, hipDeviceAttributeMultiprocessorCount, dev) == hipSuccess && n > 0) v = n;
        else v = 256;
    }
    return v;
}

template <int CMN, bool F16, bool DS, bool W3G, bool INB, bool OUTB, bool HALO, int XD, int RD, int WD>
static pvr_status launch_cw_one(ChainP &p, hipStream_t stream) {
    const size_t lds = (size_t)(W3G ? 73728 : 73728 + 32768) + (size_t)CMN * 512 + 256 + 1024 + 512 + 8 * 2048;
    static DeviceOnce attr_done;
    if (attr_done.needed()) {
        PVR_HIP_TRY(hipFuncSetAttribute((const void *)chain_wave_kernel<CMN, F16, DS, W3G, INB, OUTB, HALO, XD, RD, WD>, hipFuncAttributeMaxDynamicSharedMemorySize, (int)lds));
        attr_done.mark();
    }
    const int nch = (p.M + 255) / 256;
    int grid = cw_num_cus() & ~7;
    if (grid < 8) grid = 8;
    const int need = ((nch + 7) / 8) * 8;
    if (grid > need) grid = need;
    hipLaunchKernelGGL((chain_wave_kernel<CMN, F16, DS, W3G, INB, OUTB, HALO, XD, RD, WD>), dim3(grid), dim3(512), lds, stream, p);
    PVR_LAUNCH_CHECK();
    return PVR_OK;
}

static int cw_halo() {
    const char *e = getenv("PVR_CHAIN_WAVE_HALO");
    return e ? atoi(e) : 1;
}

template <bool F16>
static pvr_status launch_cw_dt(ChainP &p, int cmn, hipStream_t stream) {
    const bool ib = p.in_blk, ob = p.out_blk, halo = ib && p.W == 56 && cw_halo();
    if (p.xds) {
        if (cmn == 64 && halo && ob) return launch_cw_one<64, F16, true, false, true, true, true, 1, 1, 2>(p, stream);
        if (cmn == 64 && !ib) return ob ? launch_cw_one<64, F16, true, false, false, true, false, 4, 1, 2>(p, stream)
                                        : launch_cw_one<64, F16, true, false, false, false, false, 4, 1, 2>(p, stream);
    } else if (cmn == 64) {
        if (ib && ob) return halo ? launch_cw_one<64, F16, false, false, true, true, true, 1, 4, 1>(p, stream)
                                  : launch_cw_one<64, F16, false, false, true, true, false, 4, 4, 1>(p, stream);
        if (!ib && !ob) return launch_cw_one<64, F16, false, false, false, false, false, 4, 4, 1>(p, stream);
        if (!ib && ob) return launch_cw_one<64, F16, false, false, false, true, false, 4, 4, 1>(p, stream);
        return halo ? launch_cw_one<64, F16, false, false, true, false, true, 1, 4, 1>(p, stream)
                    : launch_cw_one<64, F16, false, false, true, false, false, 4, 4, 1>(p, stream);
    } else if (cmn == 128 && !ob) {
        if (halo) return launch_cw_one<128, F16, false, true, true, false, true, 1, 1, 1>(p, stream);
        return ib ? launch_cw_one<128, F16, false, true, true, false, false, 3, 4, 2>(p, stream)
                  : launch_cw_one<128, F16, false, true, false, false, false, 3, 4, 2>(p, stream);
    } else if (cmn == 0 && !ob) {
        if (ib) return halo ? launch_cw_one<0, F16, false, false, true, false, true, 1, 4, 1>(p, stream)
                            : launch_cw_one<0, F16, false, false, true, false, false, 4, 4, 1>(p, stream);
        return launch_cw_one<0, F16, false, false, false, false, false, 4, 4, 1>(p, stream);
    }
    set_error("bottleneck chain (wave form): no instance for next Cm=%d%s, blocked in/out %d/%d", cmn, p.xds ? " with downsample" : "", (int)ib, (int)ob);
    return PVR_ERR_INVALID;
}

bool chain_wave_supported(int cm, int cmn, int stride, bool ds) {
    if (cm != 64 || stride != 1) return false;
    if (ds) return cmn == 64;
    if (cmn == 128) { const char *e = getenv("PVR_CHAIN_WAVE_128"); return !e || atoi(e) != 0; }
    return cmn == 0 || cmn == 64;
}

bool chain_wave_blocked_ok(int cmn_first, int h, int w) { return cmn_first == 64 && (h * w) % 32 == 0; }
bool chain_wave_halo_enabled() { return cw_halo() != 0; }

pvr_status launch_chain_wave(ChainP &p, int cmn, int dtype, hipStream_t stream) {
    PVR_REQUIRE((int64_t)(p.M + 64) * 512 < 0x7ffffff0ll, "bottleneck chain (wave form): operand larger than 2 GiB (use a smaller chunk)");
    PVR_REQUIRE(p.xds ? p.wdsb != nullptr : (cmn != 128 || p.w3b != nullptr), "bottleneck chain (wave form): the blocked copy of W3 / Wd is missing");
    PVR_REQUIRE(!(p.in_blk || p.out_blk) || p.M % 32 == 0, "bottleneck chain (wave form): the blocked layout needs a multiple of 32 pixels");
    return dtype == PVR_F16 ? launch_cw_dt<true>(p, cmn, stream) : launch_cw_dt<false>(p, cmn, stream);
}

}
```

### pvr_habitat_amd/csrc/encoder.hip

```cpp
#include "encoder_internal.h"

namespace pvr {

pvr_status launch_split16_pack(const float *w, void *out, int rows, int K, hipStream_t stream);
bool conv_split16_supported(int cin, int cout, int k);
pvr_status launch_conv_split16(const float *in, const void *wsp, const float *bias, const float *res, float *out, int n, int h, int w, int cin,
                               int cout, int k, int stride, int pad, int relu, hipStream_t stream, float *out2 = nullptr, int n1 = 0, void *out16 = nullptr,
                               int terms = 3);

static void read_switches(PlanSwitches &sw) {
    auto get = [](const char *name, int def) { const char *v = getenv(name); return v ? atoi(v) : def; };
    sw.pool_fuse = get("PVR_POOL_FUSE", 1);
    sw.stem_u8 = get("PVR_STEM_U8", 1);
    sw.stem_lds = get("PVR_STEM_LDS", 1);
    sw.frame_front1 = get("PVR_FRAME_FRONT1", 1);
    sw.frame_next1 = get("PVR_FRAME_NEXT1", 0);
    sw.dual_ds = get("PVR_DUAL_DS", 1);
    sw.chain_ds = get("PVR_CHAIN_DS", 1);
    sw.chain_blocked = get("PVR_CHAIN_BLOCKED", 1);
    sw.splitk = get("PVR_SPLITK", 1);
    sw.smallk_div = get("PVR_SMALLK_DIV", 4);
    if (sw.smallk_div < 1) sw.smallk_div = 1;
    sw.frame_min_n = get("PVR_FRAME_MIN_N", 128);
    sw.frame_run = get("PVR_FRAME_RUN", 0);
    sw.frame_stagger = get("PVR_FRAME_RUN_STAGGER", 0);
    sw.split16 = get("PVR_SPLIT16", 1);
    sw.stem_conv1 = get("PVR_STEM_CONV1", 1);
    sw.resid32 = get("PVR_RESID32", 1);
    sw.tail_f32 = get("PVR_TAIL_F32", 1);
    sw.fuse = get("PVR_FUSE", 1);
}

template <bool F32>
__global__ __launch_bounds__(256) void range_flag_kernel(const void *x, size_t n8, int dtype, int *flags, int idx) {
    bool bad = false;
    for (size_t i = (size_t)blockIdx.x * 256 + threadIdx.x; i < n8; i += (size_t)gridDim.x * 256) {
        if constexpr (F32) {
            const u32x4 a = reinterpret_cast<const u32x4 *>(x)[2 * i], b = reinterpret_cast<const u32x4 *>(x)[2 * i + 1];
#pragma unroll
            for (int e = 0; e < 4; ++e) bad |= (a[e] & 0x7f800000u) == 0x7f800000u || (b[e] & 0x7f800000u) == 0x7f800000u;
        } else {
            const u32x4 a = reinterpret_cast<const u32x4 *>(x)[i];
            const unsigned em = dtype == PVR_F16 ? 0x7c00u : 0x7f80u;
#pragma unroll
            for (int e = 0; e < 4; ++e) bad |= ((a[e] & em) == em) || (((a[e] >> 16) & em) == em);
        }
    }
    if (__builtin_amdgcn_ballot_w64(bad) != 0 && (threadIdx.x & 63) == 0) atomicOr(flags + idx, 1);
}

const char *launch_kind_name(int k) {
    static const char *nm[] = {"conv", "bneck_frame(front1)", "bneck_frame", "bneck_frame(run)", "(in the run)", "frame_members", "conv_pp256(dual)", "dual_members", "chain", "cast",
                               "conv_f32", "conv_split16", "conv_split16(pair)", "conv_split16(in32)", "splitk(small)", "splitk", "conv_expand(blocked)",
                               "conv_wfrag(pool)", "conv_wfrag"};
    return k >= 0 && k < (int)(sizeof nm / sizeof nm[0]) ? nm[k] : "?";
}

static void add_conv(pvr_encoder *e, const std::string &conv, const std::string &bn, int in_buf, int out_buf,
                     int res_buf, int h, int w, int cin, int cin_real, int cout, int cout_real, int k, int stride,
                     int relu, int out_f32 = 0) {
    ConvOp op;
    op.conv = conv; op.bn = bn; op.in_buf = in_buf; op.out_buf = out_buf; op.res_buf = res_buf;
    op.h = h; op.w = w; op.cin = cin; op.cin_real = cin_real; op.cout = cout; op.cout_real = cout_real;
    op.k = k; op.stride = stride; op.pad = k / 2; op.relu = relu; op.out_f32 = out_f32;
    e->ops.push_back(op);
}

static void add_cast(pvr_encoder *e, int in_buf, int out_buf, int hw, int c) {
    ConvOp op;
    op.kind = 2; op.conv = "cast"; op.in_buf = in_buf; op.out_buf = out_buf; op.res_buf = B_NONE;
    op.h = hw; op.w = hw; op.cin = op.cout = op.cout_real = c; op.cin_real = 0; op.k = 1; op.stride = 1; op.pad = 0; op.relu = 0; op.out_f32 = 0;
    e->ops.push_back(op);
}

static void build_resnet50(pvr_encoder *e) {
    const int arch = e->desc.arch;
    const int stages = arch == PVR_ARCH_RESNET50_L3 ? 3 : 4;
    const int nblk[4] = {3, 4, 6, 3};
    e->resid32 = e->desc.dtype == PVR_F16 && arch != PVR_ARCH_RESNET50 && e->sw.resid32 != 0;
    e->tail32 = e->resid32 && e->sw.tail_f32 != 0;
    const int r32_from = e->tail32 ? 1 : 2;
    const bool in32 = e->resid32 && e->sw.split16 != 0;
    bool x_is_32 = false;
    int hw = 56, inpl = 64, x = B_X0, x32 = B_NONE;
    for (int li = 0; li < stages; ++li) {
        const int planes = 64 << li;
        const bool nested = (arch == PVR_ARCH_RESNET50_L4 && li == 3) || (arch == PVR_ARCH_RESNET50_L3 && li == 2);
        const bool r32 = e->resid32 && li >= r32_from;
        const bool f32stage = e->tail32 && li == stages - 1;
        for (int bi = 0; bi < nblk[li]; ++bi) {
            char pfx[64];
            if (nested) snprintf(pfx, sizeof pfx, "layer%d.0.%d", li + 1, bi);
            else snprintf(pfx, sizeof pfx, "layer%d.%d", li + 1, bi);
            const std::string p = pfx;
            const int stride = (bi == 0 && li > 0) ? 2 : 1;
            const int ohw = hw / stride;
            const int y = x == B_X0 ? B_X1 : B_X0;
            const bool last = (li == stages - 1 && bi == nblk[li] - 1);
            char tn[16]; snprintf(tn, sizeof tn, "layer%d", li + 1);
            if (f32stage) {
                const size_t first = e->ops.size();
                const int y32 = x32 == B_Y0 ? B_Y1 : B_Y0;
                add_conv(e, p + ".conv1", p + ".bn1", x32, B_T1, B_NONE, hw, hw, inpl, inpl, planes, planes, 1, 1, 1);
                add_conv(e, p + ".conv2", p + ".bn2", B_T1, B_T2, B_NONE, hw, hw, planes, planes, planes, planes, 3, stride, 1);
                int res32 = x32;
                if (bi == 0) {
                    add_conv(e, p + ".downsample.0", p + ".downsample.1", x32, B_DS, B_NONE, hw, hw, inpl, inpl, planes * 4, planes * 4, 1, stride, 0, 1);
                    res32 = B_DS;
                }
                add_conv(e, p + ".conv3", p + ".bn3", B_T2, y32, res32, ohw, ohw, planes, planes, planes * 4, planes * 4, 1, 1, 1, 1 | 2);
                for (size_t i = first; i < e->ops.size(); ++i) e->ops[i].f32op = true;
                if (bi == nblk[li] - 1) {
                    e->ops.back().tap = tn;
                    e->taps[tn] = {y32, {ohw, ohw, planes * 4, 1}};
                }
                x32 = y32; hw = ohw; inpl = planes * 4;
                continue;
            }
            add_conv(e, p + ".conv1", p + ".bn1", x_is_32 ? x32 : x, B_T1, B_NONE, hw, hw, inpl, inpl, planes, planes, 1, 1, 1);
            e->ops.back().from32 = x_is_32;
            add_conv(e, p + ".conv2", p + ".bn2", B_T1, B_T2, B_NONE, hw, hw, planes, planes, planes, planes, 3, stride, 1);
            int res = r32 ? x32 : x;
            if (bi == 0) {
                add_conv(e, p + ".downsample.0", p + ".downsample.1", x_is_32 ? x32 : x, B_DS, B_NONE, hw, hw, inpl, inpl, planes * 4,
                         planes * 4, 1, stride, 0, r32 ? 1 : 0);
                e->ops.back().from32 = x_is_32;
                res = B_DS;
            }
            if (r32) {
                const int y32 = x32 == B_Y0 ? B_Y1 : B_Y0;
                add_conv(e, p + ".conv3", p + ".bn3", B_T2, y32, res, ohw, ohw, planes, planes, planes * 4, planes * 4, 1, 1, 1, 1 | 2);
                const bool next_f32 = e->tail32 && li == stages - 2 && bi == nblk[li] - 1;
                if (!last && !next_f32 && !in32) add_cast(e, y32, y, ohw, planes * 4);
                if (bi == nblk[li] - 1) {
                    e->ops.back().tap = tn;
                    e->taps[tn] = {y32, {ohw, ohw, planes * 4, 1}};
                }
                x32 = y32; x = y; hw = ohw; inpl = planes * 4;
                x_is_32 = in32;
                continue;
            }
            const int f32 = (last && arch == PVR_ARCH_RESNET50) ? 1 : 0;
            add_conv(e, p + ".conv3", p + ".bn3", B_T2, f32 ? B_F32 : y, res, ohw, ohw, planes, planes, planes * 4,
                     planes * 4, 1, 1, 1, f32);
            if (bi == nblk[li] - 1) {
                e->ops.back().tap = tn;
                e->taps[tn] = {f32 ? B_F32 : y, {ohw, ohw, planes * 4, f32}};
            }
            x = y; hw = ohw; inpl = planes * 4;
        }
    }
    if (arch == PVR_ARCH_RESNET50) {
        e->out_size = 2048; e->final_hw = 49; e->final_c = 2048; e->final_creal = 2048;
        return;
    }
    const int cin = arch == PVR_ARCH_RESNET50_L3 ? 1024 : 2048;
    const int c = arch == PVR_ARCH_RESNET50_L3 ? 11 : 42;
    const std::string p = arch == PVR_ARCH_RESNET50_L3 ? "layer3.1" : "layer4.1";
    const int hx = e->resid32 ? x32 : x;
    add_conv(e, p + ".conv1", p + ".bn1", hx, B_T1, B_NONE, hw, hw, cin, cin, 64, c, 3, 1, 1);
    add_conv(e, p + ".downsample.0", p + ".downsample.1", hx, B_DS, B_NONE, hw, hw, cin, cin, 64, c, 3, 1, 0);
    add_conv(e, p + ".conv2", p + ".bn2", B_T1, B_F32, B_DS, hw, hw, 64, c, 64, c, 3, 1, 1, 1);
    if (e->resid32) for (size_t i = e->ops.size() - 3; i < e->ops.size(); ++i) e->ops[i].f32op = true;
    e->out_size = c * hw * hw; e->final_hw = hw * hw; e->final_c = 64; e->final_creal = c;
}

static void build_basic_resnet(pvr_encoder *e) {
    const int nb18[4] = {2, 2, 2, 2}, nb34[4] = {3, 4, 6, 3};
    const int *nblk = e->desc.arch == PVR_ARCH_RESNET18 ? nb18 : nb34;
    int hw = 56, inpl = 64, x = B_X0;
    for (int li = 0; li < 4; ++li) {
        const int planes = 64 << li;
        for (int bi = 0; bi < nblk[li]; ++bi) {
            char pfx[64];
            snprintf(pfx, sizeof pfx, "layer%d.%d", li + 1, bi);
            const std::string p = pfx;
            const int stride = (bi == 0 && li > 0) ? 2 : 1;
            const int ohw = hw / stride;
            const int y = x == B_X0 ? B_X1 : B_X0;
            const bool last = (li == 3 && bi == nblk[li] - 1);
            add_conv(e, p + ".conv1", p + ".bn1", x, B_T1, B_NONE, hw, hw, inpl, inpl, planes, planes, 3, stride, 1);
            int res = x;
            if (stride > 1 || inpl != planes) {
                add_conv(e, p + ".downsample.0", p + ".downsample.1", x, B_DS, B_NONE, hw, hw, inpl, inpl, planes, planes, 1, stride, 0);
                res = B_DS;
            }
            add_conv(e, p + ".conv2", p + ".bn2", B_T1, last ? B_F32 : y, res, ohw, ohw, planes, planes, planes, planes, 3, 1, 1, last ? 1 : 0);
            if (bi == nblk[li] - 1) {
                char tn[16]; snprintf(tn, sizeof tn, "layer%d", li + 1);
                e->ops.back().tap = tn;
                e->taps[tn] = {last ? B_F32 : y, {ohw, ohw, planes, last ? 1 : 0}};
            }
            x = y; hw = ohw; inpl = planes;
        }
    }
    e->out_size = 512; e->final_hw = 49; e->final_c = 512; e->final_creal = 512;
}

static void add_pool(pvr_encoder *e, int in_buf, int out_buf, int h, int c) {
    ConvOp op;
    op.kind = 1; op.conv = "avgpool2"; op.in_buf = in_buf; op.out_buf = out_buf; op.res_buf = B_NONE;
    op.h = h; op.w = h; op.cin = op.cin_real = op.cout = op.cout_real = c; op.k = 2; op.stride = 2; op.pad = 0; op.relu = 0; op.out_f32 = 0;
    e->ops.push_back(op);
}

static void build_clip_rn50(pvr_encoder *e) {
    const std::string v = "visual.";
    add_conv(e, v + "conv2", v + "bn2", B_STEM, B_X0, B_NONE, 112, 112, 64, 32, 64, 32, 3, 1, 1);
    add_conv(e, v + "conv3", v + "bn3", B_X0, B_X1, B_NONE, 112, 112, 64, 32, 64, 64, 3, 1, 1);
    add_pool(e, B_X1, B_X0, 112, 64);
    e->ops.back().tap = "stem3";
    e->taps["stem3"] = {B_X0, {56, 56, 64, 0}};
    const int nblk[4] = {3, 4, 6, 3};
    int hw = 56, inpl = 64, x = B_X0;
    for (int li = 0; li < 4; ++li) {
        const int planes = 64 << li;
        for (int bi = 0; bi < nblk[li]; ++bi) {
            char pfx[64];
            snprintf(pfx, sizeof pfx, "visual.layer%d.%d", li + 1, bi);
            const std::string p = pfx;
            const int stride = (bi == 0 && li > 0) ? 2 : 1;
            const int ohw = hw / stride;
            const int y = x == B_X0 ? B_X1 : B_X0;
            const bool last = (li == 3 && bi == nblk[li] - 1);
            add_conv(e, p + ".conv1", p + ".bn1", x, B_T1, B_NONE, hw, hw, inpl, inpl, planes, planes, 1, 1, 1);
            add_conv(e, p + ".conv2", p + ".bn2", B_T1, B_T2, B_NONE, hw, hw, planes, planes, planes, planes, 3, 1, 1);
            int c3_in = B_T2, res = x;
            if (stride > 1) { add_pool(e, B_T2, B_T1, hw, planes); c3_in = B_T1; }
            if (stride > 1 || inpl != planes * 4) {
                int ds_in = x;
                if (stride > 1) { add_pool(e, x, B_T2, hw, inpl); ds_in = B_T2; }
                add_conv(e, p + ".downsample.0", p + ".downsample.1", ds_in, B_DS, B_NONE, ohw, ohw, inpl, inpl, planes * 4, planes * 4, 1, 1, 0);
                res = B_DS;
            }
            add_conv(e, p + ".conv3", p + ".bn3", c3_in, last ? B_F32 : y, res, ohw, ohw, planes, planes, planes * 4, planes * 4, 1, 1, 1, last ? 1 : 0);
            if (bi == nblk[li] - 1) {
                char tn[16]; snprintf(tn, sizeof tn, "layer%d", li + 1);
                e->ops.back().tap = tn;
                e->taps[tn] = {last ? B_F32 : y, {ohw, ohw, planes * 4, last ? 1 : 0}};
            }
            x = y; hw = ohw; inpl = planes * 4;
        }
    }
    e->out_size = 1024; e->final_hw = 49; e->final_c = 2048; e->final_creal = 2048;
}

const HostTensor *enc_find(pvr_encoder *e, const std::string &name) {
    auto it = e->weights.find(name);
    return it == e->weights.end() ? nullptr : &it->second;
}

pvr_status enc_need(pvr_encoder *e, const std::string &name, const HostTensor **out, size_t numel) {
    const HostTensor *t = enc_find(e, name);
    if (!t) { set_error("missing weight: %s", name.c_str()); return PVR_ERR_MISSING_WEIGHT; }
    if (t->data.size() != numel) {
        set_error("weight %s has %zu elements, expected %zu", name.c_str(), t->data.size(), numel);
        return PVR_ERR_INVALID;
    }
    *out = t;
    return PVR_OK;
}

static pvr_status bn_fold(pvr_encoder *e, const std::string &bn, int c, std::vector<float> &scale,
                          std::vector<float> &shift) {
    const HostTensor *g, *b, *m, *v;
    pvr_status s;
    if ((s = enc_need(e, bn + ".weight", &g, c))) return s;
    if ((s = enc_need(e, bn + ".bias", &b, c))) return s;
    if ((s = enc_need(e, bn + ".running_mean", &m, c))) return s;
    if ((s = enc_need(e, bn + ".running_var", &v, c))) return s;
    scale.resize(c); shift.resize(c);
    for (int i = 0; i < c; ++i) {
        scale[i] = g->data[i] / sqrtf(v->data[i] + 1e-5f);
        shift[i] = b->data[i] - m->data[i] * scale[i];
    }
    return PVR_OK;
}


static pvr_status finalize_conv(pvr_encoder *e, ConvOp &op) {
    const int k = op.k, cr = op.cin_real, cor = op.cout_real;
    const HostTensor *w;
    pvr_status s;
    if ((s = enc_need(e, op.conv + ".weight", &w, (size_t)cor * cr * k * k))) return s;
    std::vector<float> scale, shift;
    if ((s = bn_fold(e, op.bn, cor, scale, shift))) return s;
    if (const HostTensor *cb = enc_find(e, op.conv + ".bias")) {
        if ((int)cb->data.size() != cor) { set_error("bad bias size for %s", op.conv.c_str()); return PVR_ERR_INVALID; }
        for (int i = 0; i < cor; ++i) shift[i] += scale[i] * cb->data[i];
    }
    const int cout_pad = (op.cout + 63) / 64 * 64;
    const size_t K = (size_t)k * k * op.cin;
    std::vector<u16> hw(cout_pad * K, 0);
    for (int co = 0; co < cor; ++co)
        for (int ci = 0; ci < cr; ++ci)
            for (int a = 0; a < k; ++a)
                for (int b = 0; b < k; ++b) {
                    const float v = w->data[(((size_t)co * cr + ci) * k + a) * k + b] * scale[co];
                    hw[co * K + ((size_t)a * k + b) * op.cin + ci] = f32_to_h(v, e->desc.dtype);
                }
    std::vector<float> hb(cout_pad, 0.f);
    for (int co = 0; co < cor; ++co) hb[co] = shift[co];
    if (e->desc.dtype == PVR_F32 || op.f32op || op.from32) {
        std::vector<float> hf(cout_pad * K, 0.f);
        for (int co = 0; co < cor; ++co)
            for (int ci = 0; ci < cr; ++ci)
                for (int a = 0; a < k; ++a)
                    for (int b = 0; b < k; ++b)
                        hf[co * K + ((size_t)a * k + b) * op.cin + ci] = w->data[(((size_t)co * cr + ci) * k + a) * k + b] * scale[co];
        if ((s = enc_upload(&op.d_wf, hf))) return s;
        if ((op.f32op || op.from32) && e->desc.dtype == PVR_F16 && e->sw.split16 && conv_split16_supported(op.cin, op.cout, op.k)) {
            PVR_HIP_TRY(hipMalloc((void **)&op.d_wsp, (size_t)cout_pad * K * 4));
            if ((s = launch_split16_pack(op.d_wf, op.d_wsp, cout_pad, (int)K, nullptr))) return s;
        }
        if (op.from32 && !op.d_wsp) { set_error("%s: a convolution that reads the fp32 stream needs the conv_split16 weight image (cin %d, cout %d)", op.conv.c_str(), op.cin, op.cout); return PVR_ERR_INVALID; }
        op.h_b = hb;
        return enc_upload(&op.d_b, hb);
    }
    if ((s = enc_upload(&op.d_w, hw))) return s;
    op.h_w = std::move(hw);
    op.h_b = hb;
    return enc_upload(&op.d_b, hb);
}

static bool ends_with(const std::string &s, const char *suf) {
    const size_t n = strlen(suf);
    return s.size() >= n && s.compare(s.size() - n, n, suf) == 0;
}

static void plan_splitk(pvr_encoder *e) {
    if (!e->sw.splitk || e->desc.dtype == PVR_F32) return;
    const int n = (int)e->ops.size();
    for (int i = 0; i < n; ++i) {
        ConvOp &op = e->ops[i];
        if (op.kind != 0 || op.f32op || op.from32 || op.cout > 64 || op.k * op.k * op.cin < 16384 || (op.out_f32 & 2)) continue;
        const int ho = (op.h + 2 * op.pad - op.k) / op.stride + 1;
        const size_t need = (size_t)8 * e->desc.chunk * ho * ho * op.cout * sizeof(float);
        if (need > e->buf_elems * 2) continue;
        for (int b = 0; b < B_F32 && op.ks_buf == B_NONE; ++b) {
            if (b == op.in_buf || b == op.out_buf || b == op.res_buf) continue;
            bool dead = true;
            for (int j = i + 1; j < n; ++j) {
                if (e->ops[j].in_buf == b || e->ops[j].res_buf == b) { dead = false; break; }
                if (e->ops[j].out_buf == b) break;
            }
            if (dead) { op.ks_buf = b; op.ksplit = 8; }
        }

    }
}

static pvr_status build_schedules(pvr_encoder *e) {
    const int n = (int)e->ops.size();
    for (int i = 0; i < n; ++i) { Launch l; l.conv2 = i; e->sched_plain.push_back(l); }
    if (e->desc.dtype == PVR_F32 || e->desc.arch == PVR_ARCH_CLIP_RN50) { e->sched_fused = e->sched_plain; return PVR_OK; }
    int cur_t1 = B_T1;
    bool conv1_done = false;
    int conv1_frame_out = -1;
    for (int i = 0; i < n;) {
        ConvOp &op = e->ops[i];
        if (ends_with(op.conv, ".conv1") && conv1_done) { conv1_done = false; ++i; continue; }
        auto chain_end = [&](int j) -> int {
            if (j < 0 || j >= n) return -1;
            const ConvOp &o2 = e->ops[j];
            if (!(ends_with(o2.conv, ".conv2") && o2.k == 3 && o2.cin == o2.cout && o2.cin_real == o2.cin && o2.cout_real == o2.cout) || o2.f32op) return -1;
            int c = j + 1;
            if (c < n && ends_with(e->ops[c].conv, ".downsample.0")) ++c;
            if (!(c < n && ends_with(e->ops[c].conv, ".conv3") && e->ops[c].cout == 4 * o2.cout && e->ops[c].relu &&
                  !e->ops[c].out_f32 && e->ops[c].res_buf != B_NONE && chain_supported(o2.cout, 0)))
                return -1;
            return c;
        };
        {
            const bool front_on = e->sw.frame_front1 && !e->sw.frame_next1;
            if (front_on && ends_with(op.conv, ".conv1") && op.k == 1 && op.stride == 1 && op.relu == 1 && !op.f32op && !op.out_f32 && op.tap.empty() && i + 2 < n &&
                op.cin_real == op.cin && op.cout_real == op.cout) {
                const ConvOp &o2 = e->ops[i + 1], &o3 = e->ops[i + 2];
                if (ends_with(o2.conv, ".conv2") && o2.k == 3 && !o2.f32op && o2.relu == 1 && o2.cin == o2.cout && o2.cin_real == o2.cin && o2.in_buf == op.out_buf &&
                    ends_with(o3.conv, ".conv3") && !o3.f32op && !o3.out_f32 && o3.relu == 1 && o3.res_buf == op.in_buf && o3.cout == op.cin && o3.cout_real == o3.cout &&
                    o3.in_buf == o2.out_buf && op.cout == o2.cin && bneck_frame_supported(e->desc.chunk, o2.h, o2.w, o2.cout, o3.cout, o2.stride)) {
                    Launch l;
                    l.conv1 = i; l.conv2 = i + 1; l.conv3 = i + 2; l.frame = 1; l.t1_in = op.out_buf;
                    e->sched_fused.push_back(l);
                    for (int oi : {l.conv1, l.conv2, l.conv3}) {
                        ConvOp &o = e->ops[oi];
                        if (o.d_wfb) continue;
                        const size_t K = (size_t)o.k * o.k * o.cin;
                        PVR_HIP_TRY(hipMalloc((void **)&o.d_wfb, (size_t)o.cout * K * 2));
                        pvr_status s = launch_pack_frag_weights(o.d_w, o.d_wfb, o.cout, (int)K, nullptr);
                        if (s) return s;
                    }
                    i += 3;
                    continue;
                }
            }
        }
        if (ends_with(op.conv, ".conv2") && op.k == 3 && !op.f32op && i + 1 < n && ends_with(e->ops[i + 1].conv, ".conv3") && !e->ops[i + 1].f32op &&
            !e->ops[i + 1].out_f32 && e->ops[i + 1].relu == 1 && e->ops[i + 1].res_buf != B_NONE && op.relu == 1 && op.cin == op.cout && op.cin_real == op.cin &&
            e->ops[i + 1].cout_real == e->ops[i + 1].cout && bneck_frame_supported(e->desc.chunk, op.h, op.w, op.cout, e->ops[i + 1].cout, op.stride)) {
            Launch l;
            l.conv2 = i; l.conv3 = i + 1; l.frame = 1; l.t1_in = conv1_frame_out >= 0 ? conv1_frame_out : op.in_buf;
            conv1_frame_out = -1;
            const bool next1_on = e->sw.frame_next1 != 0;
            const int nx = i + 2;
            if (next1_on && nx + 2 < n && ends_with(e->ops[nx].conv, ".conv1") && e->ops[nx].k == 1 && e->ops[nx].stride == 1 && e->ops[nx].relu == 1 && !e->ops[nx].f32op &&
                e->ops[nx].cin == e->ops[i + 1].cout && e->ops[nx].cout == op.cout && e->ops[nx].in_buf == e->ops[i + 1].out_buf && e->ops[nx].cout_real == e->ops[nx].cout &&
                e->ops[i + 1].tap.empty() && ends_with(e->ops[nx + 1].conv, ".conv2") && ends_with(e->ops[nx + 2].conv, ".conv3") &&
                bneck_frame_supported(e->desc.chunk, e->ops[nx + 1].h, e->ops[nx + 1].w, e->ops[nx + 1].cout, e->ops[nx + 2].cout, e->ops[nx + 1].stride)) {
                l.next1 = nx;
                l.t1_out = l.t1_in == B_T1 ? B_T2 : B_T1;
                conv1_frame_out = l.t1_out;
                conv1_done = true;
            }
            e->sched_fused.push_back(l);
            for (int oi : {l.conv2, l.conv3, l.next1}) {
                if (oi < 0 || e->ops[oi].d_wfb) continue;
                ConvOp &o = e->ops[oi];
                const size_t K = (size_t)o.k * o.k * o.cin;
                PVR_HIP_TRY(hipMalloc((void **)&o.d_wfb, (size_t)o.cout * K * 2));
                pvr_status s = launch_pack_frag_weights(o.d_w, o.d_wfb, o.cout, (int)K, nullptr);
                if (s) return s;
            }
            i += 2;
            continue;
        }
        const int c3 = chain_end(i);
        if (c3 < 0) {
            const bool dual_on = e->sw.dual_ds != 0;
            if (dual_on && ends_with(op.conv, ".downsample.0") && op.kind == 0 && !op.f32op && op.k == 1 && op.pad == 0 && !op.relu && !op.out_f32 &&
                op.res_buf == B_NONE && op.tap.empty() && op.cin_real == op.cin && op.cout_real == op.cout && op.cin % 64 == 0 && i + 1 < n) {
                ConvOp &o3 = e->ops[i + 1];
                if (ends_with(o3.conv, ".conv3") && o3.kind == 0 && !o3.f32op && o3.k == 1 && o3.stride == 1 && o3.pad == 0 && o3.relu == 1 && !o3.out_f32 &&
                    o3.res_buf == op.out_buf && o3.cout == op.cout && o3.cout_real == o3.cout && o3.cin_real == o3.cin && o3.cin % 64 == 0 &&
                    (op.h - 1) / op.stride + 1 == o3.h && (op.w - 1) / op.stride + 1 == o3.w && o3.cout >= 256 && o3.ksplit <= 1 && op.ksplit <= 1) {
                    const size_t K1 = (size_t)o3.cin, K2 = (size_t)op.cin, cp = ((size_t)o3.cout + 63) / 64 * 64;
                    std::vector<u16> wc(cp * (K1 + K2), 0);
                    for (int r = 0; r < o3.cout; ++r) {
                        memcpy(&wc[(size_t)r * (K1 + K2)], &o3.h_w[(size_t)r * K1], K1 * 2);
                        memcpy(&wc[(size_t)r * (K1 + K2) + K1], &op.h_w[(size_t)r * K2], K2 * 2);
                    }
                    std::vector<float> bs(cp, 0.f);
                    for (int c = 0; c < o3.cout; ++c) bs[c] = o3.h_b[c] + op.h_b[c];
                    pvr_status s = enc_upload(&o3.d_wcat, wc);
                    if (!s) s = enc_upload(&o3.d_bsum, bs);
                    if (s) return s;
                    Launch l; l.conv2 = i + 1; l.ds = i;
                    e->sched_fused.push_back(l);
                    i += 2;
                    continue;
                }
            }
            if (op.f32op && op.d_wsp && op.d_wf && i + 1 < n) {
                ConvOp &od = e->ops[i + 1];
                if (od.f32op && od.d_wsp && od.d_wf && od.in_buf == op.in_buf && od.k == op.k && od.stride == op.stride && od.pad == op.pad && od.cin == op.cin && od.h == op.h &&
                    op.cout == 64 && od.cout == 64 && op.relu == 1 && od.relu == 0 && op.res_buf == B_NONE && od.res_buf == B_NONE && op.tap.empty() && od.tap.empty() &&
                    ends_with(op.conv, ".conv1") && ends_with(od.conv, ".downsample.0")) {
                    const size_t K = (size_t)op.k * op.k * op.cin;
                    float *cat = nullptr;
                    PVR_HIP_TRY(hipMalloc((void **)&cat, 128 * K * 4));
                    PVR_HIP_TRY(hipMemcpy(cat, op.d_wf, 64 * K * 4, hipMemcpyDeviceToDevice));
                    PVR_HIP_TRY(hipMemcpy(cat + 64 * K, od.d_wf, 64 * K * 4, hipMemcpyDeviceToDevice));
                    PVR_HIP_TRY(hipMalloc((void **)&op.d_wsp_pair, 128 * K * 4));
                    pvr_status s = launch_split16_pack(cat, op.d_wsp_pair, 128, (int)K, nullptr);
                    PVR_HIP_TRY(hipDeviceSynchronize());
                    (void)hipFree(cat);
                    if (s) return s;
                    std::vector<float> bb(128, 0.f);
                    for (int c = 0; c < 64; ++c) { bb[c] = op.h_b[c]; bb[64 + c] = od.h_b[c]; }
                    if ((s = enc_upload(&op.d_b_pair, bb))) return s;
                    Launch l; l.conv2 = i; l.pair = i + 1;
                    e->sched_fused.push_back(l);
                    i += 2;
                    continue;
                }
            }
            Launch l; l.conv2 = i;
            e->sched_fused.push_back(l);
            if (op.kind == 0 && !op.f32op && !op.from32 && !op.d_wfb && op.h == op.w && op.h <= 14 && op.cout_real == op.cout && (int64_t)op.k * op.k * op.cin >= 512 &&
                conv_wfrag_supported(1, 1, op.cin, op.cout, op.k, op.k, op.pad, op.relu, op.out_f32)) {
                const size_t K = (size_t)op.k * op.k * op.cin;
                PVR_HIP_TRY(hipMalloc((void **)&op.d_wfb, (size_t)op.cout * K * 2));
                pvr_status s = launch_pack_frag_weights(op.d_w, op.d_wfb, op.cout, (int)K, nullptr);
                if (s) return s;
            }
            if (ends_with(op.conv, ".conv1")) cur_t1 = B_T1;
            ++i;
            continue;
        }
        Launch l;
        l.conv2 = i; l.conv3 = c3; l.t1_in = cur_t1;
        const int nx = c3 + 1;
        const bool ds_on = e->sw.chain_ds != 0;
        if (c3 == i + 2 && ds_on && nx < n) {
            const ConvOp &d = e->ops[i + 1];
            if (d.k == 1 && d.pad == 0 && !d.relu && !d.out_f32 && !d.f32op && d.cin_real == d.cin && d.cout == 4 * op.cout &&
                d.out_buf == e->ops[c3].res_buf && chain_ds_supported(op.cout, e->ops[nx].cout, d.cin, d.stride) && op.stride == 1)
                l.ds = i + 1;
        }
        if (l.ds < 0)
            for (int d = i + 1; d < c3; ++d) { Launch l2; l2.conv2 = d; e->sched_fused.push_back(l2); }
        if (nx < n && ends_with(e->ops[nx].conv, ".conv1") && e->ops[nx].k == 1 && e->ops[nx].stride == 1 && e->ops[nx].relu &&
            e->ops[nx].cin == 4 * op.cout && e->ops[nx].in_buf == e->ops[c3].out_buf && e->ops[nx].cout_real == e->ops[nx].cout &&
            chain_supported(op.cout, e->ops[nx].cout) && chain_end(nx + 1) >= 0) {
            l.next1 = nx;
            l.t1_out = cur_t1 == B_T1 ? B_T2 : B_T1;
            cur_t1 = l.t1_out;
            conv1_done = true;
        }
        if (l.ds >= 0 && l.next1 < 0) {
            for (int d = i + 1; d < c3; ++d) { Launch l2; l2.conv2 = d; e->sched_fused.push_back(l2); }
            l.ds = -1;
        }
        e->sched_fused.push_back(l);
        if (l.ds >= 0) {
            ConvOp &o3 = e->ops[c3];
            std::vector<float> bs(o3.h_b);
            for (size_t c = 0; c < bs.size(); ++c) bs[c] += e->ops[l.ds].h_b[c];
            pvr_status s = enc_upload(&o3.d_bsum, bs);
            if (s) return s;
        }
        for (int which = 0; which < 3; ++which) {
            const int oi = which == 0 ? c3 : which == 1 ? l.next1 : l.ds;
            if (oi < 0) continue;
            ConvOp &o = e->ops[oi];
            if (o.d_wp) continue;
            const size_t K = (size_t)o.cin;
            std::vector<u16> hp((size_t)o.cout * K);
            for (int r = 0; r < o.cout; ++r) memcpy(&hp[(size_t)r * K], &o.h_w[(size_t)chain_row_source(r) * K], K * 2);
            pvr_status s = enc_upload(&o.d_wp, hp);
            if (s) return s;
            if (which != 1) {
                std::vector<u16> hb(hp.size());
                for (int r = 0; r < o.cout; ++r)
                    for (size_t c = 0; c < K; ++c) hb[(((size_t)(r >> 4) * (K / 8) + (c >> 3)) * 16 + (r & 15)) * 8 + (c & 7)] = hp[(size_t)r * K + c];
                if ((s = enc_upload(&o.d_wpb, hb))) return s;
            }
        }
        i = c3 + 1;
    }
    for (Launch &l : e->sched_fused)
        if (l.conv3 >= 0 && !l.frame) {
            const ConvOp &c2 = e->ops[l.conv2];
            l.wave = chain_uses_wave_form(c2.cout, l.next1 >= 0 ? e->ops[l.next1].cout : 0, c2.stride, l.ds >= 0);
        }
    {
        std::vector<Launch> &sc = e->sched_fused;
        const int ns = (int)sc.size();
        auto linked = [&](int a, int b) {
            if (a < 0 || b >= ns) return false;
            const Launch &A = sc[a], &B = sc[b];
            if (A.conv3 < 0 || B.conv3 < 0 || A.next1 < 0 || A.frame || B.frame || B.ds >= 0) return false;
            const ConvOp &a2 = e->ops[A.conv2], &a3 = e->ops[A.conv3], &b2 = e->ops[B.conv2], &b3 = e->ops[B.conv3];
            return B.t1_in == A.t1_out && b3.res_buf == a3.out_buf && a3.tap.empty() && b2.h == a2.h / a2.stride && b2.w == a2.w / a2.stride && A.next1 + 1 == B.conv2;
        };
        auto eligible = [&](int b) {
            const Launch &B = sc[b];
            if (B.conv3 < 0 || B.frame || B.ds >= 0 || B.wave) return false;
            const ConvOp &b2 = e->ops[B.conv2];
            return (b2.h * b2.w) % 16 == 0 && e->sw.chain_blocked && chain_uses_wave128(b2.cout, B.next1 >= 0 ? e->ops[B.next1].cout : 0, b2.stride, (int64_t)b2.h * b2.w);
        };
        std::vector<char> can(ns, 0);
        for (int b = ns - 1; b >= 1; --b)
            can[b] = eligible(b) && linked(b - 1, b) && (sc[b].next1 < 0 || (b + 1 < ns && can[b + 1] && linked(b, b + 1)));
        for (int b = 1; b < ns; ++b) {
            if (!can[b] || !(sc[b - 1].wave == 0 || sc[b - 1].wave == 2)) continue;
            Launch &B = sc[b];
            B.wave = 2;
            ConvOp &c2 = e->ops[B.conv2];
            if (!c2.d_wpk) {
                PVR_HIP_TRY(hipMalloc((void **)&c2.d_wpk, chain_wave128_pack_bytes()));
                pvr_status s = launch_chain_wave128_pack(c2.d_w, e->ops[B.conv3].d_wp, B.next1 >= 0 ? e->ops[B.next1].d_wp : nullptr, c2.d_wpk, nullptr);
                if (s) return s;
            }
        }
    }
    for (size_t a = 0; a + 1 < e->sched_fused.size(); ++a) {
        Launch &A = e->sched_fused[a], &B = e->sched_fused[a + 1];
        if (A.conv3 < 0 || B.conv3 < 0 || A.next1 < 0 || B.ds >= 0 || A.frame || B.frame) continue;
        const ConvOp &a2 = e->ops[A.conv2], &a3 = e->ops[A.conv3], &b2 = e->ops[B.conv2], &b3 = e->ops[B.conv3];
        const int a_cmn = e->ops[A.next1].cout;
        if (!e->sw.chain_blocked) continue;
        if (B.t1_in != A.t1_out || b3.res_buf != a3.out_buf || !a3.tap.empty() || b2.h != a2.h / a2.stride || b2.w != a2.w / a2.stride || b2.stride != 1) continue;
        if (B.wave == 2) {
            A.out_blk = A.wave == 2 ? 1 : 3; B.in_blk = 1;
            continue;
        }
        if (!A.wave && !B.wave) {
            if ((b2.h * b2.w) % 16 == 0) { A.out_blk = 1; B.in_blk = 1; }
            continue;
        }
        if (!A.wave || !B.wave) continue;
        if (!chain_wave_blocked_ok(a_cmn, a2.h, a2.w)) continue;
        A.out_blk = 1; B.in_blk = 1;
        if (A.ds >= 0 && a > 0 && a2.w == 56 && chain_wave_halo_enabled()) {
            Launch &C = e->sched_fused[a - 1];
            if (C.conv3 < 0 && C.conv2 >= 0) {
                const ConvOp &c1 = e->ops[C.conv2];
                if (c1.kind == 0 && !c1.f32op && c1.k == 1 && c1.stride == 1 && c1.out_buf == A.t1_in && c1.tap.empty() && c1.res_buf == B_NONE && !c1.out_f32 &&
                    c1.ksplit <= 1) { C.out_blk = 1; A.in_blk = 1; }
            }
        }
    }
    if (e->sw.stem_conv1 && !e->sched_fused.empty() && (e->desc.arch == PVR_ARCH_RESNET50 || e->desc.arch == PVR_ARCH_RESNET50_L3 || e->desc.arch == PVR_ARCH_RESNET50_L4)) {
        const Launch &L0 = e->sched_fused[0];
        if (L0.conv3 < 0 && L0.ds < 0 && L0.pair < 0 && !L0.frame && L0.conv2 == 0) {
            const ConvOp &c1 = e->ops[0];
            if (c1.kind == 0 && !c1.f32op && !c1.from32 && c1.k == 1 && c1.stride == 1 && c1.cin == 64 && c1.cout == 64 && c1.cin_real == 64 && c1.cout_real == 64 && c1.relu == 1 &&
                c1.in_buf == B_X0 && c1.out_buf == B_T1 && c1.res_buf == B_NONE && !c1.out_f32 && c1.tap.empty() && c1.ksplit <= 1 && c1.h == 56 && (int)c1.h_w.size() == 64 * 64) {
                std::vector<u16> img(64 * 64);
                stem_c1_pack(c1.h_w.data(), img.data());
                pvr_status s = enc_upload(&e->d_stem_c1w, img);
                if (s) return s;
                e->stem_c1 = 0; e->stem_c1_blk = L0.out_blk;
                e->sched_fused.erase(e->sched_fused.begin());
            }
        }
    }
    return PVR_OK;
}

static pvr_status finalize_stem(pvr_encoder *e, const std::string &conv_name = "conv1.weight", const std::string &bn_name = "bn1",
                                int cout_real = 64, int ks = 7) {
    const HostTensor *w;
    pvr_status s;
    if ((s = enc_need(e, conv_name, &w, (size_t)cout_real * 3 * ks * ks))) return s;
    std::vector<float> scale, shift;
    if ((s = bn_fold(e, bn_name, cout_real, scale, shift))) return s;
    scale.resize(64, 0.f); shift.resize(64, 0.f);
    const int t0 = (7 - ks) / 2;
    auto wat = [&](int co, int c, int a, int b) -> double {
        const int aa = a - t0, bb = b - t0;
        if (co >= cout_real || aa < 0 || aa >= ks || bb < 0 || bb >= ks) return 0.0;
        return (double)w->data[(((size_t)co * 3 + c) * ks + aa) * ks + bb];
    };
    if (e->desc.dtype == PVR_F32) {
        std::vector<float> hf(64 * 49 * 4, 0.f);
        for (int co = 0; co < 64; ++co)
            for (int c = 0; c < 3; ++c)
                for (int t = 0; t < 49; ++t) hf[((size_t)co * 49 + t) * 4 + c] = (float)wat(co, c, t / 7, t % 7) * scale[co];
        if ((s = enc_upload(&e->d_stem_wf, hf))) return s;
        return enc_upload(&e->d_stem_b, shift);
    }
    std::vector<u16> hw(64 * 224, 0);
    for (int co = 0; co < 64; ++co)
        for (int a = 0; a < 7; ++a)
            for (int b = 0; b < 7; ++b) {
                double vsum = 0.0;
                for (int c = 0; c < 3; ++c) {
                    const double wv = wat(co, c, a, b) * scale[co];
                    hw[co * 224 + (a * 8 + b) * 4 + c] = f32_to_h((float)(wv / (255.0 * e->desc.std_[c])), e->desc.dtype);
                    vsum += wv * (128.0 - 255.0 * e->desc.mean[c]) / (255.0 * e->desc.std_[c]);
                }
                hw[co * 224 + (a * 8 + b) * 4 + 3] = f32_to_h((float)vsum, e->desc.dtype);
            }
    if ((s = enc_upload(&e->d_stem_w, hw))) return s;
    return enc_upload(&e->d_stem_b, shift);
}

static pvr_status finalize_attnpool(pvr_encoder *e) {
    const int C = 2048, O = 1024, dt = e->desc.dtype;
    const std::string a = "visual.attnpool.";
    pvr_status s;
    std::vector<u16> wq((size_t)3 * C * C);
    std::vector<float> bq((size_t)3 * C);
    const char *nm[3] = {"q_proj", "k_proj", "v_proj"};
    for (int i = 0; i < 3; ++i) {
        const HostTensor *w, *b;
        if ((s = enc_need(e, a + nm[i] + ".weight", &w, (size_t)C * C))) return s;
        if ((s = enc_need(e, a + nm[i] + ".bias", &b, (size_t)C))) return s;
        for (size_t k = 0; k < (size_t)C * C; ++k) wq[(size_t)i * C * C + k] = f32_to_h(w->data[k], dt);
        for (int k = 0; k < C; ++k) bq[(size_t)i * C + k] = b->data[k];
    }
    const HostTensor *wc, *bc, *pos;
    if ((s = enc_need(e, a + "c_proj.weight", &wc, (size_t)O * C))) return s;
    if ((s = enc_need(e, a + "c_proj.bias", &bc, (size_t)O))) return s;
    if ((s = enc_need(e, a + "positional_embedding", &pos, (size_t)50 * C))) return s;
    std::vector<u16> wch((size_t)O * C);
    for (size_t k = 0; k < wch.size(); ++k) wch[k] = f32_to_h(wc->data[k], dt);
    if ((s = enc_upload(&e->ap_wqkv, wq)) || (s = enc_upload(&e->ap_bqkv, bq)) || (s = enc_upload(&e->ap_wc, wch)) ||
        (s = enc_upload(&e->ap_bc, bc->data)) || (s = enc_upload(&e->ap_pos, pos->data))) return s;
    PVR_HIP_TRY(hipMalloc((void **)&e->ap_out, (size_t)e->desc.chunk * O * sizeof(float) * PVR_MAX_LANES));
    return PVR_OK;
}

}

static bool pooled_head(const pvr_encoder *enc) {
    return enc->desc.arch == PVR_ARCH_RESNET50 || enc->desc.arch == PVR_ARCH_RESNET18 || enc->desc.arch == PVR_ARCH_RESNET34;
}

static void *bufp(pvr_encoder *enc, int id) { return id == B_STEM ? (void *)enc->d_stem : enc->d_buf[id]; }

constexpr size_t SMALLK_BYTES = (size_t)32 << 20;
static int small_batch_ksplit(const pvr_encoder *enc, const ConvOp &op, int nb) {
    if (!enc->low_latency || nb > 4 || op.kind != 0 || op.f32op || op.from32 || op.ksplit > 1 || op.relu > 1 || (op.out_f32 & 2)) return 0;
    const int K = op.k * op.k * op.cin, nk = K / 64;
    if (nk < 8) return 0;
    const int ho = (op.h + 2 * op.pad - op.k) / op.stride + 1;
    const long long M = (long long)nb * ho * ho, blocks = ((M + 127) / 128) * ((op.cout + 127) / 128);
    if (blocks > 64) return 0;
    const int div = enc->sw.smallk_div;
    int ks = nk / div;
    if (ks > (div >= 4 ? 16 : 32)) ks = div >= 4 ? 16 : 32;
    if ((size_t)ks * M * op.cout * sizeof(float) > SMALLK_BYTES) return 0;
    return ks;
}

static pvr_status ensure_smallk(pvr_encoder *enc) {
    if (!enc->low_latency || enc->vit || enc->rnd || enc->host) return PVR_OK;
    for (int l = 0; l < PVR_MAX_LANES; ++l)
        if (enc->lane_ws[l].valid && !enc->d_smallk[l]) PVR_HIP_TRY(hipMalloc((void **)&enc->d_smallk[l], SMALLK_BYTES));
    return PVR_OK;
}

static uint8_t resolve_kind(const pvr_encoder *enc, const std::vector<Launch> &plan, size_t li, int nb, bool allow_pool = true) {
    const Launch &l = plan[li];
    const ConvOp &op = enc->ops[l.conv3 >= 0 ? l.conv3 : l.conv2];
    const bool ll = enc->low_latency && nb <= 4;
    const bool autoalgo = conv_algo() == -1;
    if (l.frame) {
        if (nb >= enc->sw.frame_min_n && !enc->low_latency) return l.conv1 >= 0 ? LK_FRAME_FRONT1 : LK_FRAME;
        return LK_FRAME_MEMBERS;
    }
    if (l.conv3 < 0 && l.ds >= 0) return (!ll && autoalgo) ? LK_DUAL : LK_DUAL_MEMBERS;
    if (l.conv3 >= 0) return LK_CHAIN;
    if (op.kind == 2) return LK_CAST;
    if (l.pair >= 0) return LK_SPLIT16_PAIR;
    if (op.f32op) return op.d_wsp ? LK_SPLIT16 : LK_F32;
    if (op.from32) return LK_SPLIT16_IN32;
    if (small_batch_ksplit(enc, op, nb)) return LK_SPLITK_SMALL;
    if (op.ksplit > 1) return LK_SPLITK;
    const int ho = (op.h + 2 * op.pad - op.k) / op.stride + 1, wo = (op.w + 2 * op.pad - op.k) / op.stride + 1;
    if (l.out_blk && autoalgo && op.cin == 64 &&
        conv_expand_supported((int64_t)nb * op.h * op.w, op.h, op.w, op.cin, op.cout, 1, 1, 1, 0, op.relu, 0, false))
        return LK_EXPAND_BLOCKED;
    if (allow_pool && enc->sw.pool_fuse && li + 1 == plan.size() && op.d_wfb && pooled_head(enc) && enc->final_hw == 49 && op.h == 7 && op.w == 7 && op.k == 1 &&
        op.stride == 1 && op.relu == 1 && (op.out_f32 & 1) && !(op.out_f32 & 2) && op.res_buf != B_NONE && op.out_buf == B_F32 && enc->final_c == op.cout &&
        autoalgo && !ll)
        return LK_WFRAG_POOL;
    if (op.d_wfb && autoalgo && !ll && conv_wfrag_preferred((int64_t)nb * ho * wo, op.cin, op.cout, op.k, op.k) &&
        conv_wfrag_supported((int64_t)nb * ho * wo, (int64_t)nb * op.h * op.w * op.cin * 2, op.cin, op.cout, op.k, op.k, op.pad, op.relu, op.out_f32))
        return LK_WFRAG;
    return LK_CONV;
}

static const std::vector<Launch> &cur_plan(const pvr_encoder *enc) { return enc->fuse ? enc->sched_fused : enc->sched_plain; }

static void resolve_kinds(pvr_encoder *enc) {
    const std::vector<Launch> &plan = cur_plan(enc);
    const int chunk = enc->desc.chunk;
    enc->kinds_stride = plan.size();
    enc->kinds.assign((size_t)chunk * plan.size(), LK_CONV);
    if (enc->desc.dtype == PVR_F32 || enc->desc.arch == PVR_ARCH_CLIP_RN50 || enc->vit || enc->rnd || enc->host) { enc->kinds_algo = conv_algo(); return; }
    for (int nb = 1; nb <= chunk; ++nb)
        for (size_t i = 0; i < plan.size(); ++i) enc->kinds[(size_t)(nb - 1) * plan.size() + i] = resolve_kind(enc, plan, i, nb);
    if (enc->sw.frame_run)
        for (int nb = 1; nb <= chunk; ++nb) {
            uint8_t *k = enc->kinds.data() + (size_t)(nb - 1) * plan.size();
            for (size_t i = 0; i + 1 < plan.size(); ++i) {
                if (k[i] != LK_FRAME_FRONT1) continue;
                size_t j = i;
                while (j + 1 < plan.size() && j + 1 - i < 6 && k[j + 1] == LK_FRAME_FRONT1 &&
                       enc->ops[plan[j + 1].conv3].res_buf == enc->ops[plan[j].conv3].out_buf && enc->ops[plan[j + 1].conv1].in_buf == enc->ops[plan[j].conv3].out_buf) ++j;
                if (j > i) { k[i] = LK_FRAME_RUN; for (size_t t = i + 1; t <= j; ++t) k[t] = LK_FRAME_RUN_TAIL; }
                i = j;
            }
        }
    enc->kinds_algo = conv_algo();
}

static pvr_status alloc_workspace(pvr_encoder *enc) {
    const int C = enc->desc.chunk, crop = enc->desc.crop;
    const bool f32 = enc->desc.dtype == PVR_F32;
    const size_t esz = f32 ? 4 : 2;
    const size_t img = (size_t)C * (crop + 6) * (crop + 8) * 4;
    PVR_HIP_TRY(hipMalloc((void **)&enc->d_img, img * 2));
    PVR_HIP_TRY(hipMemset(enc->d_img, 0, img * 2));
    PVR_HIP_TRY(hipMalloc((void **)&enc->d_stem, (size_t)C * 112 * 112 * 64 * esz));
    if (f32) PVR_HIP_TRY(hipMalloc((void **)&enc->d_imgf, (size_t)C * crop * crop * 4 * sizeof(float)));
    enc->buf_elems = (size_t)C * 56 * 56 * 256;
    for (int b = 0; b < B_COUNT; ++b) {
        size_t bytes = enc->buf_elems * esz;
        if (b == B_F32) bytes = (size_t)C * enc->final_hw * enc->final_c * 4;
        if ((b == B_Y0 || b == B_Y1) && !enc->resid32) continue;
        PVR_HIP_TRY(hipMalloc(&enc->d_buf[b], bytes));
    }
    return PVR_OK;
}
static void save_lane(pvr_encoder *enc, int lane) {
    auto &l = enc->lane_ws[lane];
    l.d_img = enc->d_img; l.d_stem = enc->d_stem; l.d_imgf = enc->d_imgf;
    for (int b = 0; b < B_COUNT; ++b) l.d_buf[b] = enc->d_buf[b];
    l.valid = true; enc->cur_lane = lane;
}
static pvr_status use_lane(pvr_encoder *enc, int lane) {
    if (lane == enc->cur_lane) return PVR_OK;
    if (!enc->lane_ws[lane].valid) {
        const int prev = enc->cur_lane;
        enc->d_img = nullptr; enc->d_stem = nullptr; enc->d_imgf = nullptr;
        for (int b = 0; b < B_COUNT; ++b) enc->d_buf[b] = nullptr;
        pvr_status s = alloc_workspace(enc);
        if (!s && hipDeviceSynchronize() != hipSuccess) { set_error("use_lane: device sync failed"); s = PVR_ERR_HIP; }
        if (s) {
            for (int b = 0; b < B_COUNT; ++b) if (enc->d_buf[b]) (void)hipFree(enc->d_buf[b]);
            if (enc->d_img) (void)hipFree(enc->d_img);
            if (enc->d_stem) (void)hipFree(enc->d_stem);
            if (enc->d_imgf) (void)hipFree(enc->d_imgf);
            const auto &l = enc->lane_ws[prev];
            enc->d_img = l.d_img; enc->d_stem = l.d_stem; enc->d_imgf = l.d_imgf;
            for (int b = 0; b < B_COUNT; ++b) enc->d_buf[b] = l.d_buf[b];
            return s;
        }
        save_lane(enc, lane);
        return ensure_smallk(enc);
    }
    const auto &l = enc->lane_ws[lane];
    enc->d_img = l.d_img; enc->d_stem = l.d_stem; enc->d_imgf = l.d_imgf;
    for (int b = 0; b < B_COUNT; ++b) enc->d_buf[b] = l.d_buf[b];
    enc->cur_lane = lane;
    return PVR_OK;
}

extern "C" {

pvr_status pvr_encoder_create(const pvr_encoder_desc *desc, pvr_encoder **out) {
    PVR_REQUIRE(desc && out, "pvr_encoder_create: null argument");
    PVR_REQUIRE(desc->arch >= PVR_ARCH_RESNET50 && desc->arch <= PVR_ARCH_RESNET34, "unknown arch %d", desc->arch);
    PVR_REQUIRE(desc->dtype == PVR_BF16 || desc->dtype == PVR_F16 || (desc->dtype == PVR_F32 && (desc->arch <= PVR_ARCH_RESNET50_L3 || desc->arch == PVR_ARCH_RESNET18 || desc->arch == PVR_ARCH_RESNET34)),
                "dtype must be PVR_BF16 or PVR_F16 (PVR_F32 is built for the ResNet50 family only)");
    PVR_REQUIRE(desc->max_batch > 0, "max_batch must be positive");
    PVR_REQUIRE(desc->crop == 224, "crop must be 224 (reference embeddings.py:82; CLIP input_resolution 224)");
    PVR_REQUIRE(desc->resize >= desc->crop, "resize must be >= crop");
    pvr_encoder *e = new pvr_encoder();
    e->desc = *desc;
    read_switches(e->sw);
    if (e->desc.chunk <= 0 || e->desc.chunk > e->desc.max_batch) e->desc.chunk = e->desc.max_batch;
    if (e->desc.arch == PVR_ARCH_RANDOM5) {
        random5_create(e);
    } else if (e->desc.arch == PVR_ARCH_RESNET18 || e->desc.arch == PVR_ARCH_RESNET34) {
        build_basic_resnet(e);
    } else if (e->desc.arch == PVR_ARCH_CLIP_RN50) {
        build_clip_rn50(e);
        resizer_create(e);
    } else if (e->desc.arch >= PVR_ARCH_CLIP_VIT_B32 && e->desc.arch <= PVR_ARCH_MAE_VIT_H14) {
        pvr_status s = vit_create(e);
        if (s) { delete e; return s; }
    } else {
        build_resnet50(e);
    }
    *out = e;
    return PVR_OK;
}

pvr_status pvr_encoder_load_weights(pvr_encoder *enc, const char *name, const float *host_data, const int64_t *shape,
                                    int32_t ndim) {
    PVR_REQUIRE(enc && name && host_data, "pvr_encoder_load_weights: null argument");
    PVR_REQUIRE(!enc->finalized, "encoder already finalized");
    HostTensor t;
    size_t n = 1;
    for (int i = 0; i < ndim; ++i) { t.shape.push_back(shape[i]); n *= (size_t)shape[i]; }
    t.data.assign(host_data, host_data + n);
    enc->weights[name] = std::move(t);
    return PVR_OK;
}

pvr_status pvr_encoder_set_host_backend(pvr_encoder *enc, int32_t on) {
    PVR_REQUIRE(enc, "null encoder");
    PVR_REQUIRE(!enc->finalized, "pvr_encoder_set_host_backend: call between create and finalize");
    enc->host = on != 0;
    return PVR_OK;
}

pvr_status pvr_encoder_finalize(pvr_encoder *enc) {
    PVR_REQUIRE(enc, "null encoder");
    PVR_REQUIRE(!enc->finalized, "encoder already finalized");
    pvr_status s;
    if (enc->host) return host_finalize(enc);
    if (enc->vit || enc->rnd) {
        if ((s = enc->vit ? vit_finalize(enc) : random5_finalize(enc))) return s;
        PVR_HIP_TRY(hipDeviceSynchronize());
        enc->weights.clear();
        enc->finalized = true;
        return PVR_OK;
    }
    const bool rn50c = enc->desc.arch == PVR_ARCH_CLIP_RN50;
    if ((s = rn50c ? finalize_stem(enc, "visual.conv1.weight", "visual.bn1", 32, 3) : finalize_stem(enc))) return s;
    if (rn50c && (s = finalize_attnpool(enc))) return s;
    for (auto &op : enc->ops)
        if (op.kind == 0 && (s = finalize_conv(enc, op))) return s;
    if ((s = build_schedules(enc))) return s;
    PVR_HIP_TRY(hipDeviceSynchronize());
    for (auto &op : enc->ops) {
        op.h_w.clear(); op.h_w.shrink_to_fit(); op.h_b.clear(); op.h_b.shrink_to_fit();
        if (op.d_wsp && op.d_wf) { (void)hipFree(op.d_wf); op.d_wf = nullptr; }
    }
    enc->fuse = enc->sw.fuse != 0;
    pvr_status ws = alloc_workspace(enc);
    if (ws) return ws;
    plan_splitk(enc);
    PVR_HIP_TRY(hipMalloc((void **)&enc->d_zero, PVR_ZERO_BYTES));
    PVR_HIP_TRY(hipMemset(enc->d_zero, 0, PVR_ZERO_BYTES));
    save_lane(enc, 0);
    if ((s = ensure_smallk(enc))) return s;
    resolve_kinds(enc);
    PVR_HIP_TRY(hipDeviceSynchronize());
    enc->weights.clear();
    enc->finalized = true;
    return PVR_OK;
}

int32_t pvr_encoder_out_size(const pvr_encoder *enc) { return enc ? enc->out_size : 0; }

}


static pvr_status clip_rn50_chunk(pvr_encoder *enc, const uint8_t *fr, int nb, int h, int w, float *out, int64_t out_stride, hipStream_t st) {
    const int dt = enc->desc.dtype, crop = enc->desc.crop;
    pvr_status s;
    const uint8_t *u8; int oh, ow;
    if ((s = resizer_run(enc, enc->cur_lane, fr, nb, h, w, st, &u8, &oh, &ow))) return s;
    if ((s = launch_preprocess(u8, nb, oh, ow, enc->desc.resize, crop, enc->d_img, dt, st))) return s;
    enc->last_n = nb;
    if (enc->stop_after == "pre") return PVR_OK;
    if ((s = launch_stem(enc->d_img, enc->d_stem_w, enc->d_stem_b, enc->d_stem, nb, crop, dt, st))) return s;
    for (const ConvOp &op : enc->ops) {
        if (op.kind == 1) s = launch_avgpool2(bufp(enc, op.in_buf), bufp(enc, op.out_buf), nb, op.h, op.w, op.cin, dt, st);
        else s = launch_conv(bufp(enc, op.in_buf), op.d_w, op.d_b, op.res_buf == B_NONE ? nullptr : bufp(enc, op.res_buf), bufp(enc, op.out_buf),
                             enc->d_zero, nb, op.h, op.w, op.cin, op.cout, op.k, op.k, op.stride, op.pad, op.relu, op.out_f32, dt, st);
        if (s) return s;
        if (!enc->stop_after.empty() && op.tap == enc->stop_after) return PVR_OK;
    }
    const int C = 2048, T = 50;
    if ((s = launch_attnpool_tokens((const float *)enc->d_buf[B_F32], enc->ap_pos, enc->d_buf[B_T1], nb, 49, C, dt, st))) return s;
    if ((s = launch_conv(enc->d_buf[B_T1], enc->ap_wqkv, enc->ap_bqkv, nullptr, enc->d_buf[B_X0], enc->d_zero, nb * T, 1, 1, C, 3 * C, 1, 1, 1, 0, 0, 0, dt, st))) return s;
    if ((s = launch_attention(enc->d_buf[B_X0], enc->d_buf[B_T2], T, C, 32, nb, dt, st))) return s;
    float *dense = enc->ap_out + (size_t)enc->cur_lane * enc->desc.chunk * 1024;
    if ((s = launch_conv(enc->d_buf[B_T2], enc->ap_wc, enc->ap_bc, nullptr, dense, enc->d_zero, nb, T, 1, C, 1024, 1, 1, T, 0, 0, 1, dt, st))) return s;
    PVR_HIP_TRY(hipMemcpy2DAsync(out, (size_t)out_stride * 4, dense, 1024 * 4, 1024 * 4, nb, hipMemcpyDeviceToDevice, st));
    return PVR_OK;
}

static pvr_status forward_impl(pvr_encoder *enc, const uint8_t *frames, int32_t n, int32_t h, int32_t w, float *out,
                               int64_t out_stride, void *hip_stream, std::vector<hipEvent_t> *ev) {
    PVR_REQUIRE(enc && frames && out, "pvr_encoder_forward: null argument");
    if (!enc->finalized) { set_error("encoder not finalized"); return PVR_ERR_STATE; }
    PVR_REQUIRE(n > 0 && n <= enc->desc.max_batch, "n=%d outside 1..max_batch=%d", n, enc->desc.max_batch);
    PVR_REQUIRE(out_stride >= enc->out_size, "out_stride %lld < out_size %d", (long long)out_stride, enc->out_size);
    hipStream_t st = (hipStream_t)hip_stream;
    const int dt = enc->desc.dtype;
    pvr_status s;
    if (enc->vit) return vit_forward(enc, frames, n, h, w, out, out_stride, st);
    if (enc->rnd) return random5_forward(enc, frames, n, h, w, out, out_stride, st);
    for (int f0 = 0; f0 < n; f0 += enc->desc.chunk) {
        const int nb = (n - f0 < enc->desc.chunk) ? n - f0 : enc->desc.chunk;
        const uint8_t *fr = frames + (size_t)f0 * h * w * 3;
        auto mark = [&]() -> pvr_status {
            if (ev && f0 == 0) {
                hipEvent_t e;
                PVR_HIP_TRY(hipEventCreate(&e));
                const int idx = (int)ev->size();
                if (enc->span_first < 0 || idx == enc->span_first || idx == enc->span_last) PVR_HIP_TRY(hipEventRecord(e, st));
                ev->push_back(e);
            }
            return PVR_OK;
        };
        if ((s = mark())) return s;
        if (dt == PVR_F32) {
            const int crop = enc->desc.crop;
            if ((s = launch_preprocess(fr, nb, h, w, enc->desc.resize, crop, enc->d_img, PVR_BF16, st, enc->crop_pos))) return s;
            if ((s = launch_normalize_nhwc4(enc->d_img, enc->d_imgf, nb, crop, enc->desc.mean, enc->desc.std_, PVR_BF16, st))) return s;
            if ((s = mark())) return s;
            if ((s = launch_stem_f32(enc->d_imgf, enc->d_stem_wf, enc->d_stem_b, (float *)enc->d_stem, nb, crop, st))) return s;
            if ((s = mark())) return s;
            if ((s = launch_maxpool_f32((const float *)enc->d_stem, (float *)enc->d_buf[B_X0], nb, 112, 112, 64, st))) return s;
            if ((s = mark())) return s;
            enc->last_n = nb;
            for (auto &op : enc->ops) {
                const float *res = op.res_buf == B_NONE ? nullptr : (const float *)enc->d_buf[op.res_buf];
                if ((s = launch_conv_f32((const float *)enc->d_buf[op.in_buf], op.d_wf, op.d_b, res, (float *)enc->d_buf[op.out_buf], nb,
                                         op.h, op.w, op.cin, op.cout, op.k, op.stride, op.pad, op.relu, st)))
                    return s;
                if ((s = mark())) return s;
            }
            float *o32 = out + (size_t)f0 * out_stride;
            if (pooled_head(enc))
                s = launch_avgpool(enc->d_buf[B_F32], o32, out_stride, nb, enc->final_hw, enc->final_c, 1, dt, st);
            else
                s = launch_nhwc_to_chw((const float *)enc->d_buf[B_F32], o32, out_stride, nb, enc->final_hw, enc->final_c,
                                       enc->final_creal, st);
            if (s) return s;
            if ((s = mark())) return s;
            continue;
        }
        if (enc->desc.arch == PVR_ARCH_CLIP_RN50) {
            if ((s = clip_rn50_chunk(enc, fr, nb, h, w, out + (size_t)f0 * out_stride, out_stride, st))) return s;
            continue;
        }
        int fused_u8 = 0;
        const bool c1_pending = enc->fuse && enc->stem_c1 >= 0;
        const bool c1_in_stem = c1_pending && enc->stop_after.empty() && stem_conv1_capable();
        if (enc->sw.stem_u8 && enc->sw.stem_lds && enc->stop_after.empty() && enc->desc.crop == 224 && enc->crop_pos >= 0 && enc->crop_pos <= 4) {
            int rn = 1, top = 0, left = 0;
            preprocess_geometry(h, w, enc->desc.resize, enc->desc.crop, enc->crop_pos, &rn, &top, &left);
            if (!rn && stem_pool_u8_ok(fr, h, w, top, left)) {
                if ((s = mark())) return s;
                if ((s = launch_stem_pool_u8(fr, nb, h, w, top, left, enc->d_stem_w, enc->d_stem_b, enc->d_buf[B_X0], dt, st, c1_in_stem ? enc->d_stem_c1w : nullptr,
                                             c1_in_stem ? enc->ops[enc->stem_c1].d_b : nullptr, c1_in_stem ? enc->d_buf[B_T1] : nullptr, enc->stem_c1_blk))) return s;
                fused_u8 = 1;
            }
        }
        if (!fused_u8) {
        if ((s = launch_preprocess(fr, nb, h, w, enc->desc.resize, enc->desc.crop, enc->d_img, dt, st, enc->crop_pos))) return s;
        if ((s = mark())) return s;
        }
        enc->last_n = nb;
        if (enc->stop_after == "pre") return PVR_OK;
        if (enc->stop_after == "stem") {
            if ((s = launch_stem(enc->d_img, enc->d_stem_w, enc->d_stem_b, enc->d_stem, nb, enc->desc.crop, dt, st))) return s;
            return PVR_OK;
        }
        if (!fused_u8 && (s = launch_stem_pool(enc->d_img, enc->d_stem_w, enc->d_stem_b, enc->d_buf[B_X0], nb, enc->desc.crop, dt, st, c1_in_stem ? enc->d_stem_c1w : nullptr,
                                               c1_in_stem ? enc->ops[enc->stem_c1].d_b : nullptr, c1_in_stem ? enc->d_buf[B_T1] : nullptr, enc->stem_c1_blk))) return s;
        if (enc->range_flags) {
            const size_t n8 = (size_t)nb * 56 * 56 * 64 / 8;
            hipLaunchKernelGGL(range_flag_kernel<false>, dim3(2048), dim3(256), 0, st, enc->d_buf[B_X0], n8, dt, enc->range_flags, (int)cur_plan(enc).size());
        }
        if ((s = mark())) return s;
        if ((s = mark())) return s;
        if (enc->stop_after == "pool") return PVR_OK;
        bool stopped = false, t1_blocked = false;
        if (c1_in_stem) t1_blocked = enc->stem_c1_blk != 0;
        else if (c1_pending && enc->stop_after != "pool") {
            const ConvOp &c1 = enc->ops[enc->stem_c1];
            if (enc->stem_c1_blk && conv_algo() == -1 && conv_expand_supported((int64_t)nb * c1.h * c1.w, c1.h, c1.w, c1.cin, c1.cout, 1, 1, 1, 0, c1.relu, 0, false)) {
                s = launch_conv_expand(enc->d_buf[c1.in_buf], c1.d_w, c1.d_b, nullptr, enc->d_buf[c1.out_buf], nb, c1.h, c1.w, c1.cin, c1.cout, 1, c1.relu, dt, st, 1);
                t1_blocked = true;
            } else
                s = launch_conv(enc->d_buf[c1.in_buf], c1.d_w, c1.d_b, nullptr, enc->d_buf[c1.out_buf], enc->d_zero, nb, c1.h, c1.w, c1.cin, c1.cout, 1, 1, 1, 0, c1.relu, 0, dt, st);
            if (s) return s;
        }
        bool pooled = false;
        const std::vector<Launch> &plan_ = cur_plan(enc);
        if (enc->kinds_algo != conv_algo() || enc->kinds_stride != plan_.size()) resolve_kinds(enc);
        const uint8_t *kinds = enc->kinds.data() + (size_t)(nb - 1) * plan_.size();
        float *smallk = enc->d_smallk[enc->cur_lane];
        const bool pool_args_ok = enc->stop_after.empty() && out_stride % 4 == 0 && (((size_t)(out + (size_t)f0 * out_stride)) & 15) == 0;
        int launch_idx = 0;
        const bool run_ok = enc->stop_after.empty() && !enc->range_flags;
        const int stop_idx = enc->stop_after.size() > 1 && enc->stop_after[0] == '#' ? atoi(enc->stop_after.c_str() + 1) : -1;
        auto member = [&](const ConvOp &o, const void *in, const void *r_, void *out_) -> pvr_status {
            if (const int ks = small_batch_ksplit(enc, o, nb)) {
                if (!smallk) { set_error("low-latency plan without its scratch (pvr_encoder_set_low_latency allocates it)"); return PVR_ERR_STATE; }
                return launch_conv_splitk(in, o.d_w, o.d_b, r_, out_, enc->d_zero, smallk, ks, nb, o.h, o.w, o.cin, o.cout, o.k, o.k, o.stride, o.pad, o.relu, o.out_f32, dt, st);
            }
            return launch_conv(in, o.d_w, o.d_b, r_, out_, enc->d_zero, nb, o.h, o.w, o.cin, o.cout, o.k, o.k, o.stride, o.pad, o.relu, o.out_f32, dt, st);
        };
        for (size_t li = 0; li < plan_.size(); ++li) {
            const Launch &l = plan_[li];
            const ConvOp &op = enc->ops[l.conv3 >= 0 ? l.conv3 : l.conv2];
            const void *res = op.res_buf == B_NONE ? nullptr : enc->d_buf[op.res_buf];
            int kind = kinds[li];
            if (kind == LK_WFRAG_POOL && !pool_args_ok) kind = resolve_kind(enc, plan_, li, nb, false);
            if ((kind == LK_FRAME_RUN || kind == LK_FRAME_RUN_TAIL) && !run_ok) kind = LK_FRAME_FRONT1;
            switch (kind) {
            case LK_FRAME_RUN: {
                BFBlk blks[6];
                int nblk = 0;
                for (size_t t = li; t < plan_.size() && nblk < 6 && (t == li || kinds[t] == LK_FRAME_RUN_TAIL); ++t, ++nblk) {
                    const Launch &lt = plan_[t];
                    const ConvOp &o3 = enc->ops[lt.conv3], &o2 = enc->ops[lt.conv2], &o1 = enc->ops[lt.conv1];
                    blks[nblk] = BFBlk{(const u16 *)o1.d_wfb, (const u16 *)o2.d_wfb, (const u16 *)o3.d_wfb, (const u16 *)enc->d_buf[o3.res_buf], o1.d_b, o2.d_b, o3.d_b,
                                       (u16 *)enc->d_buf[o3.out_buf]};
                }
                s = launch_bneck_frame_run(blks, nblk, nb, dt, st, enc->sw.frame_stagger);
                break;
            }
            case LK_FRAME_RUN_TAIL:
                s = PVR_OK;
                break;
            case LK_FRAME_FRONT1: {
                const ConvOp &c2 = enc->ops[l.conv2], &cf = enc->ops[l.conv1];
                s = launch_bneck_frame(nullptr, c2.d_wfb, c2.d_b, op.d_wfb, op.d_b, res, enc->d_buf[op.out_buf], nullptr, nb, 3 | 8, dt, st,
                                       nullptr, nullptr, nullptr, nullptr, cf.d_wfb, cf.d_b);
                break;
            }
            case LK_FRAME: {
                const ConvOp &c2 = enc->ops[l.conv2];
                const ConvOp *c1 = l.next1 >= 0 ? &enc->ops[l.next1] : nullptr;
                s = launch_bneck_frame(enc->d_buf[l.t1_in], c2.d_wfb, c2.d_b, op.d_wfb, op.d_b, res, enc->d_buf[op.out_buf], nullptr, nb, c1 ? 7 : 3, dt, st,
                                       nullptr, c1 ? c1->d_wfb : nullptr, c1 ? c1->d_b : nullptr, c1 ? enc->d_buf[l.t1_out] : nullptr);
                break;
            }
            case LK_FRAME_MEMBERS: {
                const ConvOp &c2 = enc->ops[l.conv2];
                const ConvOp *c1 = l.next1 >= 0 ? &enc->ops[l.next1] : nullptr;
                const ConvOp *cf = l.conv1 >= 0 ? &enc->ops[l.conv1] : nullptr;
                const int t2b = l.t1_in == B_T1 ? B_T2 : B_T1;
                s = PVR_OK;
                if (cf) s = member(*cf, enc->d_buf[cf->in_buf], nullptr, enc->d_buf[l.t1_in]);
                if (!s) s = member(c2, enc->d_buf[l.t1_in], nullptr, enc->d_buf[t2b]);
                if (!s) s = member(op, enc->d_buf[t2b], res, enc->d_buf[op.out_buf]);
                if (!s && c1) s = member(*c1, enc->d_buf[op.out_buf], nullptr, enc->d_buf[l.t1_out]);
                break;
            }
            case LK_DUAL: {
                const ConvOp &cd = enc->ops[l.ds];
                s = launch_conv_pp256(enc->d_buf[op.in_buf], op.d_wcat, op.d_bsum, nullptr, enc->d_buf[op.out_buf], nb, op.h, op.w, op.cin, op.cout, 1, 1, 1, 0,
                                      op.relu, 0, 0, dt, 224, st, enc->d_buf[cd.in_buf], cd.h, cd.w, cd.cin, cd.stride);
                break;
            }
            case LK_DUAL_MEMBERS: {
                const ConvOp &cd = enc->ops[l.ds];
                s = member(cd, enc->d_buf[cd.in_buf], nullptr, enc->d_buf[cd.out_buf]);
                if (!s) s = member(op, enc->d_buf[op.in_buf], res, enc->d_buf[op.out_buf]);
                break;
            }
            case LK_CHAIN: {
                const ConvOp &c2 = enc->ops[l.conv2];
                const ConvOp *c1 = l.next1 >= 0 ? &enc->ops[l.next1] : nullptr;
                const ConvOp *cd = l.ds >= 0 ? &enc->ops[l.ds] : nullptr;
                s = launch_bottleneck_chain(enc->d_buf[l.t1_in], c2.d_w, c2.d_b, op.d_wp, cd ? op.d_bsum : op.d_b, res, enc->d_buf[op.out_buf],
                                            c1 ? c1->d_wp : nullptr, c1 ? c1->d_b : nullptr, c1 ? enc->d_buf[l.t1_out] : nullptr, nb,
                                            c2.h, c2.w, c2.cout, c1 ? c1->cout : 0, c2.stride, dt, st,
                                            cd ? enc->d_buf[cd->in_buf] : nullptr, cd ? cd->d_wp : nullptr, op.d_wpb, cd ? cd->d_wpb : nullptr,
                                            l.wave, cd ? (l.in_blk && t1_blocked) : l.in_blk, l.out_blk, c2.d_wpk);
                t1_blocked = false;
                break;
            }
            case LK_CAST:
                s = launch_f32_to_h((const float *)enc->d_buf[op.in_buf], enc->d_buf[op.out_buf], (size_t)nb * op.h * op.w * op.cin, dt, st);
                break;
            case LK_F32:
                s = launch_conv_f32((const float *)enc->d_buf[op.in_buf], op.d_wf, op.d_b, (const float *)res, (float *)enc->d_buf[op.out_buf], nb,
                                    op.h, op.w, op.cin, op.cout, op.k, op.stride, op.pad, op.relu, st);
                break;
            case LK_SPLIT16:
                s = launch_conv_split16((const float *)enc->d_buf[op.in_buf], op.d_wsp, op.d_b, (const float *)res, (float *)enc->d_buf[op.out_buf], nb,
                                        op.h, op.w, op.cin, op.cout, op.k, op.stride, op.pad, op.relu, st);
                break;
            case LK_SPLIT16_PAIR: {
                const ConvOp &od = enc->ops[l.pair];
                s = launch_conv_split16((const float *)enc->d_buf[op.in_buf], op.d_wsp_pair, op.d_b_pair, nullptr, (float *)enc->d_buf[op.out_buf], nb, op.h, op.w, op.cin,
                                        128, op.k, op.stride, op.pad, 1, st, (float *)enc->d_buf[od.out_buf], 64);
                break;
            }
            case LK_SPLIT16_IN32:
                s = launch_conv_split16((const float *)enc->d_buf[op.in_buf], op.d_wsp, op.d_b, nullptr, (op.out_f32 & 1) ? (float *)enc->d_buf[op.out_buf] : nullptr, nb,
                                        op.h, op.w, op.cin, op.cout, op.k, op.stride, op.pad, op.relu, st, nullptr, 0, (op.out_f32 & 1) ? nullptr : enc->d_buf[op.out_buf], 1);
                break;
            case LK_SPLITK_SMALL:
                s = member(op, enc->d_buf[op.in_buf], res, enc->d_buf[op.out_buf]);
                break;
            case LK_SPLITK:
                s = launch_conv_splitk(enc->d_buf[op.in_buf], op.d_w, op.d_b, res, enc->d_buf[op.out_buf], enc->d_zero, (float *)enc->d_buf[op.ks_buf],
                                       op.ksplit, nb, op.h, op.w, op.cin, op.cout, op.k, op.k, op.stride, op.pad, op.relu, op.out_f32, dt, st);
                break;
            case LK_EXPAND_BLOCKED:
                s = launch_conv_expand(enc->d_buf[op.in_buf], op.d_w, op.d_b, nullptr, enc->d_buf[op.out_buf], nb, op.h, op.w, op.cin, op.cout, 1, op.relu, dt, st, 1);
                t1_blocked = true;
                break;
            case LK_WFRAG_POOL:
                s = launch_conv_wfrag(enc->d_buf[op.in_buf], op.d_wfb, op.d_b, res, nullptr, nb, op.h, op.w, op.cin, op.cout, 1, 1, 1, 0, 1, 1, dt, st,
                                      out + (size_t)f0 * out_stride, out_stride);
                pooled = true;
                break;
            case LK_WFRAG:
                s = launch_conv_wfrag(enc->d_buf[op.in_buf], op.d_wfb, op.d_b, res, enc->d_buf[op.out_buf], nb, op.h, op.w, op.cin, op.cout, op.k, op.k,
                                      op.stride, op.pad, op.relu, op.out_f32, dt, st);
                break;
            default:
                s = launch_conv(enc->d_buf[op.in_buf], op.d_w, op.d_b, res, enc->d_buf[op.out_buf], enc->d_zero, nb, op.h, op.w,
                                op.cin, op.cout, op.k, op.k, op.stride, op.pad, op.relu, op.out_f32, dt, st);
            }
            if (s) return s;
            if (enc->range_flags && kind != LK_WFRAG_POOL) {
                const int ho_ = (op.h + 2 * op.pad - op.k) / op.stride + 1, wo_ = (op.w + 2 * op.pad - op.k) / op.stride + 1;
                const size_t n8 = (size_t)nb * ho_ * wo_ * op.cout / 8;
                const int blocks = (int)((n8 + 255) / 256 < 2048 ? (n8 + 255) / 256 : 2048);
                if ((op.out_f32 & 1) || op.f32op) hipLaunchKernelGGL(range_flag_kernel<true>, dim3(blocks), dim3(256), 0, st, enc->d_buf[op.out_buf], n8, dt, enc->range_flags, (int)li);
                else hipLaunchKernelGGL(range_flag_kernel<false>, dim3(blocks), dim3(256), 0, st, enc->d_buf[op.out_buf], n8, dt, enc->range_flags, (int)li);
            }
            if ((s = mark())) return s;
            if (!enc->stop_after.empty() && op.tap == enc->stop_after) { stopped = true; break; }
            if (launch_idx++ == stop_idx) { stopped = true; break; }
        }
        enc->last_pooled = pooled;
        if (stopped) return PVR_OK;
        float *o = out + (size_t)f0 * out_stride;
        if (pooled)
            s = PVR_OK;
        else if (pooled_head(enc))
            s = launch_avgpool(enc->d_buf[B_F32], o, out_stride, nb, enc->final_hw, enc->final_c, 1, dt, st);
        else
            s = launch_nhwc_to_chw((const float *)enc->d_buf[B_F32], o, out_stride, nb, enc->final_hw, enc->final_c,
                                   enc->final_creal, st);
        if (s) return s;
        if ((s = mark())) return s;
    }
    return PVR_OK;
}

static pvr_status lane_wait(pvr_encoder *enc, int lane, void *hip_stream) {
    hipStream_t st = (hipStream_t)hip_stream;
    if (enc->lane_done[lane] && enc->lane_stream[lane] != st) PVR_HIP_TRY(hipStreamWaitEvent(st, enc->lane_done[lane], 0));
    return PVR_OK;
}
static pvr_status lane_mark(pvr_encoder *enc, int lane, void *hip_stream) {
    hipStream_t st = (hipStream_t)hip_stream;
    if (!enc->lane_done[lane]) PVR_HIP_TRY(hipEventCreateWithFlags(&enc->lane_done[lane], hipEventDisableTiming));
    PVR_HIP_TRY(hipEventRecord(enc->lane_done[lane], st));
    enc->lane_stream[lane] = st;
    return PVR_OK;
}
static pvr_status lane_forward(pvr_encoder *enc, int lane, const uint8_t *frames, int32_t n, int32_t h, int32_t w, float *out,
                               int64_t out_stride, void *hip_stream) {
    pvr_status s = lane_wait(enc, lane, hip_stream);
    if (!s) s = forward_impl(enc, frames, n, h, w, out, out_stride, hip_stream, nullptr);
    if (!s) s = lane_mark(enc, lane, hip_stream);
    return s;
}

extern "C" {

#define PVR_NO_HOST(enc_, what_) PVR_REQUIRE(!((enc_) && (enc_)->host), what_ ": not available on a host-backend encoder")

pvr_status pvr_encoder_forward(pvr_encoder *enc, const uint8_t *frames, int32_t n, int32_t h, int32_t w, float *out,
                               int64_t out_stride, void *hip_stream) {
    if (enc && enc->host) {
        PVR_REQUIRE(enc->finalized, "encoder not finalized");
        PVR_REQUIRE(n <= enc->desc.max_batch, "n=%d exceeds max_batch=%d", n, enc->desc.max_batch);
        return host_forward(enc, frames, n, h, w, out, out_stride);
    }
    PVR_REQUIRE(enc, "pvr_encoder_forward: null encoder");
    TraceScope trace("pvr_encoder_forward");
    if (enc->finalized && !enc->vit && !enc->rnd) { pvr_status s = use_lane(enc, 0); if (s) return s; }
    if (enc->finalized && enc->vit) { pvr_status s = vit_use_lane(enc, 0); if (s) return s; }
    if (!enc->finalized) { set_error("encoder not finalized"); return PVR_ERR_STATE; }
    return lane_forward(enc, 0, frames, n, h, w, out, out_stride, hip_stream);
}

pvr_status pvr_encoder_forward_lane(pvr_encoder *enc, int32_t lane, const uint8_t *frames, int32_t n, int32_t h, int32_t w, float *out,
                                    int64_t out_stride, void *hip_stream) {
    if (enc && enc->host) return pvr_encoder_forward(enc, frames, n, h, w, out, out_stride, hip_stream);
    PVR_REQUIRE(enc, "pvr_encoder_forward_lane: null encoder");
    TraceScope trace(lane == 0 ? "pvr_encoder_forward_lane 0" : "pvr_encoder_forward_lane 1+");
    PVR_REQUIRE(lane >= 0 && lane < PVR_MAX_LANES, "pvr_encoder_forward_lane: lane must be 0..%d", PVR_MAX_LANES - 1);
    if (!enc->finalized) { set_error("encoder not finalized"); return PVR_ERR_STATE; }
    if (enc->vit) { pvr_status s = vit_use_lane(enc, lane); if (s) return s; }
    else if (!enc->rnd) { pvr_status s = use_lane(enc, lane); if (s) return s; }
    else PVR_REQUIRE(lane == 0, "pvr_encoder_forward_lane: the 'random' PVR plan has a single workspace");
    return lane_forward(enc, lane, frames, n, h, w, out, out_stride, hip_stream);
}

pvr_status pvr_encoder_profile(pvr_encoder *enc, const uint8_t *frames, int32_t n, int32_t h, int32_t w, float *out,
                               int64_t out_stride, void *hip_stream, float *op_ms, double *op_flops, int32_t cap,
                               int32_t *n_ops) {
    PVR_REQUIRE(enc && op_ms && op_flops && n_ops, "pvr_encoder_profile: null argument");
    PVR_NO_HOST(enc, "pvr_encoder_profile");
    PVR_REQUIRE(n <= enc->desc.chunk, "profile: n=%d must fit one chunk (%d)", n, enc->desc.chunk);
    std::vector<hipEvent_t> ev;
    pvr_status s = (enc->finalized && !enc->vit && !enc->rnd) ? use_lane(enc, 0) : PVR_OK;
    if (!s && enc->finalized && enc->vit) s = vit_use_lane(enc, 0);
    if (!s) s = lane_wait(enc, 0, hip_stream);
    if (!s) s = forward_impl(enc, frames, n, h, w, out, out_stride, hip_stream, &ev);
    if (!s && hipStreamSynchronize((hipStream_t)hip_stream) != hipSuccess) { set_error("profile: sync failed"); s = PVR_ERR_HIP; }
    const int nl = (int)ev.size() - 1;
    if (!s && nl > cap) { set_error("profile: %d launches > cap %d", nl, cap); s = PVR_ERR_INVALID; }
    if (!s) {
        for (int i = 0; i < nl; ++i) {
            float ms = 0.f;
            (void)hipEventElapsedTime(&ms, ev[i], ev[i + 1]);
            op_ms[i] = ms;
            op_flops[i] = 0.0;
        }
        if (nl > 1) op_flops[1] = 2.0 * n * 112.0 * 112.0 * 64.0 * 147.0;
        if (nl > 1 && enc->fuse && enc->stem_c1 >= 0 && enc->desc.dtype != PVR_F32) op_flops[1] += 2.0 * n * 56.0 * 56.0 * 64.0 * 64.0;
        int i = 3;
        auto flops = [&](int oi) {
            if (oi < 0) return 0.0;
            const ConvOp &op = enc->ops[oi];
            const double ho = (op.h + 2 * op.pad - op.k) / op.stride + 1;
            return 2.0 * n * ho * ho * (double)op.cout_real * op.k * op.k * op.cin_real;
        };
        const bool fused = enc->fuse && enc->desc.dtype != PVR_F32;
        for (const Launch &l : (fused ? enc->sched_fused : enc->sched_plain)) {
            if (i >= nl) break;
            op_flops[i++] = flops(l.conv1) + flops(l.conv2) + flops(l.conv3) + flops(l.next1) + flops(l.ds) + flops(l.pair);
        }
        *n_ops = nl;
    }
    for (auto e : ev) (void)hipEventDestroy(e);
    return s;
}

pvr_status pvr_encoder_profile_span(pvr_encoder *enc, const uint8_t *frames, int32_t n, int32_t h, int32_t w, float *out, int64_t out_stride,
                                    void *hip_stream, int32_t first_op, int32_t last_op, float *span_ms) {
    PVR_REQUIRE(enc && span_ms, "pvr_encoder_profile_span: null argument");
    PVR_NO_HOST(enc, "pvr_encoder_profile_span");
    PVR_REQUIRE(n <= enc->desc.chunk, "profile: n=%d must fit one chunk (%d)", n, enc->desc.chunk);
    PVR_REQUIRE(first_op >= 0 && last_op >= first_op, "pvr_encoder_profile_span: bad launch range %d..%d", first_op, last_op);
    std::vector<hipEvent_t> ev;
    pvr_status s = (enc->finalized && !enc->vit && !enc->rnd) ? use_lane(enc, 0) : PVR_OK;
    if (!s && enc->finalized && enc->vit) s = vit_use_lane(enc, 0);
    if (!s) s = lane_wait(enc, 0, hip_stream);
    enc->span_first = first_op; enc->span_last = last_op + 1;
    if (!s) s = forward_impl(enc, frames, n, h, w, out, out_stride, hip_stream, &ev);
    enc->span_first = enc->span_last = -1;
    if (!s && hipStreamSynchronize((hipStream_t)hip_stream) != hipSuccess) { set_error("profile: sync failed"); s = PVR_ERR_HIP; }
    if (!s && last_op + 1 >= (int)ev.size()) { set_error("profile_span: launch %d past the plan's %d launches", last_op, (int)ev.size() - 1); s = PVR_ERR_INVALID; }
    if (!s && hipEventElapsedTime(span_ms, ev[first_op], ev[last_op + 1]) != hipSuccess) { set_error("profile_span: elapsed time failed"); s = PVR_ERR_HIP; }
    for (auto e : ev) (void)hipEventDestroy(e);
    return s;
}

pvr_status pvr_encoder_set_crop_position(pvr_encoder *enc, int32_t pos) {
    PVR_REQUIRE(enc, "null encoder");
    PVR_REQUIRE(pos >= 0 && pos <= 4, "crop position %d outside 0..4", pos);
    PVR_REQUIRE(pos == 0 || (!enc->vit && !enc->rnd && enc->desc.arch != PVR_ARCH_CLIP_RN50), "corner crops are built for the ResNet50 family only");
    enc->crop_pos = pos;
    return PVR_OK;
}

pvr_status pvr_encoder_set_low_latency(pvr_encoder *enc, int32_t on) {
    PVR_REQUIRE(enc, "null encoder");
    enc->low_latency = on != 0;
    if (!enc->finalized || enc->vit || enc->rnd || enc->host) return PVR_OK;
    pvr_status s = ensure_smallk(enc);
    if (s) return s;
    resolve_kinds(enc);
    return PVR_OK;
}

pvr_status pvr_encoder_debug_set_fusion(pvr_encoder *enc, int32_t on) {
    PVR_REQUIRE(enc, "null encoder");
    enc->fuse = on != 0;
    if (enc->finalized && !enc->vit && !enc->rnd && !enc->host) resolve_kinds(enc);
    return PVR_OK;
}

pvr_status pvr_encoder_debug_set_switch(pvr_encoder *enc, const char *name, int32_t value) {
    PVR_REQUIRE(enc && name, "pvr_encoder_debug_set_switch: null argument");
    const std::string nm = name;
    if (nm == "pool_fuse") enc->sw.pool_fuse = value;
    else if (nm == "stem_u8") enc->sw.stem_u8 = value;
    else if (nm == "frame_min_n") enc->sw.frame_min_n = value;
    else if (nm == "frame_run") enc->sw.frame_run = value;
    else if (nm == "frame_stagger") enc->sw.frame_stagger = value;
    else { set_error("pvr_encoder_debug_set_switch: '%s' is not a live switch (pool_fuse, stem_u8, frame_min_n, frame_run, frame_stagger); plan switches are read from the environment at create", name); return PVR_ERR_INVALID; }
    if (enc->finalized && !enc->vit && !enc->rnd && !enc->host) resolve_kinds(enc);
    return PVR_OK;
}

pvr_status pvr_encoder_check_range(pvr_encoder *enc, const uint8_t *frames, int32_t n, int32_t h, int32_t w, float *out, int64_t out_stride, void *hip_stream,
                                   int32_t *first_bad) {
    PVR_REQUIRE(enc && frames && out && first_bad, "pvr_encoder_check_range: null argument");
    PVR_NO_HOST(enc, "pvr_encoder_check_range");
    PVR_REQUIRE(enc->finalized && !enc->vit && !enc->rnd && enc->desc.arch != PVR_ARCH_CLIP_RN50 && enc->desc.dtype != PVR_F32,
                "pvr_encoder_check_range: built for the 16-bit plans of the torchvision ResNet family");
    PVR_REQUIRE(n > 0 && n <= enc->desc.chunk, "pvr_encoder_check_range: n=%d must fit one chunk (%d)", n, enc->desc.chunk);
    hipStream_t st = (hipStream_t)hip_stream;
    const size_t nl = enc->sched_plain.size();
    pvr_status s = use_lane(enc, 0);
    if (!s) s = lane_wait(enc, 0, hip_stream);
    if (s) return s;
    int *flags = nullptr;
    PVR_HIP_TRY(hipMalloc((void **)&flags, (nl + 1) * sizeof(int)));
    if (hipMemsetAsync(flags, 0, (nl + 1) * sizeof(int), st) != hipSuccess) { (void)hipFree(flags); set_error("check_range: memset failed"); return PVR_ERR_HIP; }
    const bool fuse0 = enc->fuse;
    enc->fuse = false; resolve_kinds(enc);
    enc->range_flags = flags;
    s = forward_impl(enc, frames, n, h, w, out, out_stride, hip_stream, nullptr);
    enc->range_flags = nullptr;
    enc->fuse = fuse0; resolve_kinds(enc);
    std::vector<int> hf(nl + 1, 0);
    if (!s && hipMemcpyAsync(hf.data(), flags, (nl + 1) * sizeof(int), hipMemcpyDeviceToHost, st) != hipSuccess) { set_error("check_range: copy failed"); s = PVR_ERR_HIP; }
    if (!s && hipStreamSynchronize(st) != hipSuccess) { set_error("check_range: sync failed"); s = PVR_ERR_HIP; }
    (void)hipFree(flags);
    if (s) return s;
    *first_bad = hf[nl] ? 1 : -1;
    for (size_t i = 0; i < nl && *first_bad < 0; ++i) if (hf[i]) *first_bad = (int32_t)i + 3;
    return lane_mark(enc, 0, hip_stream);
}

int32_t pvr_encoder_launch_kernel(const pvr_encoder *enc, int32_t n, int32_t index, char *buf, int32_t cap) {
    if (!enc || !buf || cap <= 0 || index < 3 || !enc->finalized || enc->vit || enc->rnd || enc->host || n < 1) return 0;
    const std::vector<Launch> &plan = cur_plan(enc);
    const int i = index - 3;
    if (i >= (int)plan.size()) return 0;
    const int nb = n < enc->desc.chunk ? n : enc->desc.chunk;
    const bool tab = enc->kinds_stride == plan.size() && enc->kinds.size() == (size_t)enc->desc.chunk * plan.size() && enc->kinds_algo == conv_algo();
    const int kind = tab ? enc->kinds[(size_t)(nb - 1) * plan.size() + i] : resolve_kind(enc, plan, (size_t)i, nb);
    const char *nm = enc->desc.dtype == PVR_F32 ? "conv_f32" : launch_kind_name(kind);
    if (enc->desc.dtype != PVR_F32 && kind == LK_CHAIN) nm = plan[i].wave == 2 ? "chain_wave128" : plan[i].wave == 1 ? "chain_wave" : "bottleneck_chain";
    snprintf(buf, (size_t)cap, "%s", nm);
    return (int32_t)strlen(nm);
}

int32_t pvr_encoder_launch_name(const pvr_encoder *enc, int32_t index, char *buf, int32_t cap) {
    if (!enc || !buf || cap <= 0 || index < 0) return 0;
    std::string nm;
    static const char *head[3] = {"preprocess", "stem", "maxpool"};
    if (index < 3) nm = head[index];
    else {
        const bool fused = enc->fuse && enc->desc.dtype != PVR_F32;
        const std::vector<Launch> &sc = fused ? enc->sched_fused : enc->sched_plain;
        const int i = index - 3;
        if (i < (int)sc.size()) {
            nm = enc->ops[sc[i].conv1 >= 0 ? sc[i].conv1 : sc[i].conv2].conv;
            if (sc[i].conv1 >= 0) nm += "+conv2";
            if (sc[i].conv3 >= 0) nm += "+" + enc->ops[sc[i].conv3].conv.substr(enc->ops[sc[i].conv3].conv.rfind('.') + 1);
            if (sc[i].ds >= 0 || sc[i].pair >= 0) nm += "&downsample";
            if (sc[i].next1 >= 0) nm += "+" + enc->ops[sc[i].next1].conv;
        } else if (i == (int)sc.size() && !enc->vit && !enc->rnd) nm = "pool/flatten";
    }
    snprintf(buf, (size_t)cap, "%s", nm.c_str());
    return (int32_t)nm.size();
}

pvr_status pvr_encoder_debug_stop_after(pvr_encoder *enc, const char *tap) {
    PVR_REQUIRE(enc, "null encoder");
    enc->stop_after = tap ? tap : "";
    return PVR_OK;
}

pvr_status pvr_encoder_tap(pvr_encoder *enc, const char *name, float *out, int64_t cap, int64_t *count, void *hip_stream) {
    PVR_REQUIRE(enc && name && out && count, "pvr_encoder_tap: null argument");
    PVR_NO_HOST(enc, "pvr_encoder_tap");
    if (!enc->finalized || enc->last_n == 0) { set_error("no forward has run"); return PVR_ERR_STATE; }
    hipStream_t st = (hipStream_t)hip_stream;
    if (enc->vit) return vit_tap(enc, name, out, cap, count, st);
    const int n = enc->last_n, crop = enc->desc.crop;
    const std::string nm = name;
    const void *src = nullptr;
    size_t elems = 0;
    int f32 = 0;
    if (nm == "pre") { src = enc->d_img; elems = (size_t)n * (crop + 6) * (crop + 8) * 4; }
    else if (nm == "stem") { src = enc->d_stem; elems = (size_t)n * 112 * 112 * 64; }
    else if (nm == "pool") { src = enc->d_buf[B_X0]; elems = (size_t)n * 56 * 56 * 64; }
    else if (nm.compare(0, 3, "buf") == 0 && nm.find(':') != std::string::npos) {
        const int b = atoi(nm.c_str() + 3);
        PVR_REQUIRE(b >= 0 && b < B_F32, "tap %s: 16-bit workspace buffers are 0..%d", name, B_F32 - 1);
        src = enc->d_buf[b]; elems = (size_t)atoll(nm.c_str() + nm.find(':') + 1);
    } else {
        auto it = enc->taps.find(nm);
        PVR_REQUIRE(it != enc->taps.end(), "unknown tap %s", name);
        const auto &g = it->second.second;
        if (it->second.first == B_F32 && enc->last_pooled) {
            set_error("tap %s: the last forward averaged inside its last convolution and never wrote this activation; run the forward with "
                      "pvr_encoder_debug_stop_after(enc, \"%s\") or pvr_encoder_debug_set_switch(enc, \"pool_fuse\", 0) first", name, name);
            return PVR_ERR_STATE;
        }
        src = enc->d_buf[it->second.first];
        elems = (size_t)n * g[0] * g[1] * g[2];
        f32 = g[3];
    }
    PVR_REQUIRE((int64_t)elems <= cap, "tap %s needs %zu elements, cap %lld", name, elems, (long long)cap);
    *count = (int64_t)elems;
    const bool img16 = nm == "pre";
    if (f32 || (enc->desc.dtype == PVR_F32 && !img16)) {
        PVR_HIP_TRY(hipMemcpyAsync(out, src, elems * 4, hipMemcpyDeviceToDevice, st));
        return PVR_OK;
    }
    return launch_h_to_f32(src, out, elems, enc->desc.dtype == PVR_F32 ? PVR_BF16 : enc->desc.dtype, st);
}

void pvr_encoder_destroy(pvr_encoder *enc) {
    if (!enc) return;
    if (enc->hplan) host_destroy(enc);
    if (enc->vit) vit_destroy(enc);
    if (enc->rnd) random5_destroy(enc);
    for (auto &op : enc->ops) { if (op.d_w) (void)hipFree(op.d_w); if (op.d_wp) (void)hipFree(op.d_wp); if (op.d_wpb) (void)hipFree(op.d_wpb); if (op.d_wfb) (void)hipFree(op.d_wfb); if (op.d_wcat) (void)hipFree(op.d_wcat); if (op.d_wf) (void)hipFree(op.d_wf); if (op.d_wsp) (void)hipFree(op.d_wsp); if (op.d_wsp_pair) (void)hipFree(op.d_wsp_pair); if (op.d_b_pair) (void)hipFree(op.d_b_pair); if (op.d_wpk) (void)hipFree(op.d_wpk); if (op.d_b) (void)hipFree(op.d_b); if (op.d_bsum) (void)hipFree(op.d_bsum); }
    if (enc->d_stem_wf) (void)hipFree(enc->d_stem_wf);
    if (enc->d_stem_c1w) (void)hipFree(enc->d_stem_c1w);
    bool any_lane = false;
    for (auto &l : enc->lane_ws) {
// ... 25 lines not shown
```

### pvr_habitat_amd/csrc/encoder_internal.h

```cpp
#pragma once
#include <map>
#include <string>
#include <vector>
#include <cmath>
#include "common.h"
#include "chain_params.h"

namespace pvr {

pvr_status launch_preprocess(const uint8_t *, int, int, int, int, int, void *, int, hipStream_t, int crop_pos = 0);
pvr_status launch_stem(const void *, const void *, const float *, void *, int, int, int, hipStream_t);
pvr_status launch_maxpool(const void *, void *, int, int, int, int, int, hipStream_t);
pvr_status launch_stem_pool(const void *, const void *, const float *, void *, int, int, int, hipStream_t, const void *c1_w = nullptr, const float *c1_b = nullptr,
                            void *c1_t1 = nullptr, int c1_blk = 0);
bool stem_pool_u8_ok(const void *, int, int, int, int);
pvr_status launch_stem_pool_u8(const uint8_t *, int, int, int, int, int, const void *, const float *, void *, int, hipStream_t, const void *c1_w = nullptr,
                               const float *c1_b = nullptr, void *c1_t1 = nullptr, int c1_blk = 0);
bool stem_conv1_capable();
void stem_c1_pack(const u16 *w, u16 *img);
void preprocess_geometry(int h, int w, int resize, int crop, int crop_pos, int *resize_needed, int *top, int *left);
pvr_status launch_avgpool(const void *, float *, int64_t, int, int, int, int, int, hipStream_t);
pvr_status launch_nhwc_to_chw(const float *, float *, int64_t, int, int, int, int, hipStream_t);
pvr_status launch_h_to_f32(const void *, float *, size_t, int, hipStream_t);
pvr_status launch_f32_to_h(const float *, void *, size_t, int, hipStream_t);
pvr_status launch_conv_splitk(const void *, const void *, const float *, const void *, void *, const void *, float *, int, int, int, int, int, int,
                              int, int, int, int, int, int, int, hipStream_t);
pvr_status launch_conv(const void *, const void *, const float *, const void *, void *, const void *, int, int, int, int,
                       int, int, int, int, int, int, int, int, hipStream_t);

bool conv_expand_supported(int64_t M, int h, int w, int cin, int cout, int kh, int kw, int stride, int pad, int relu, int out_f32, bool has_res);
pvr_status launch_conv_expand(const void *in, const void *wgt, const float *bias, const void *res, void *out, int n, int h, int w, int cin,
                              int cout, int stride, int relu, int dtype, hipStream_t stream, int out_blk = 0);

bool pp256_supported(int64_t M, int cin, int cout, int kh, int kw, int64_t in_bytes, int64_t w_bytes, int64_t out_bytes, int64_t res_bytes);
pvr_status launch_conv_pp256(const void *in, const void *wgt, const float *bias, const void *res, void *out, int n, int h, int w, int cin,
                             int cout, int kh, int kw, int stride, int pad, int act, int out_f32, int res_f32, int dtype, int bm, hipStream_t stream,
                             const void *in2 = nullptr, int h2 = 0, int w2 = 0, int cin2 = 0, int stride2 = 1);
int conv_algo();
void set_conv_algo(int a);

bool bneck_frame_supported(int n, int h, int w, int cm, int cout, int stride);
pvr_status launch_pack_frag_weights(const void *w, void *out, int rows, int K, hipStream_t stream);
pvr_status launch_bneck_frame(const void *t1, const void *w2p, const float *b2, const void *w3p, const float *b3, const void *res, void *y,
                              void *t2_out, int n, int phases, int dtype, hipStream_t stream, unsigned long long *stamps = nullptr,
                              const void *w1np = nullptr, const float *b1n = nullptr, void *t1n = nullptr, const void *w1fp = nullptr, const float *b1f = nullptr);
struct BFBlk {
    const unsigned short *w1f, *w2, *w3, *res;
    const float *b1f, *b2, *b3;
    unsigned short *y;
};
pvr_status launch_bneck_frame_run(const BFBlk *blocks, int nblk, int n, int dtype, hipStream_t stream, int stagger);
pvr_status launch_bneck_frame64(const void *w1p, const float *b1, const void *w2p, const float *b2, const void *w3p, const float *b3, const void *x, void *y, int n,
                                int dtype, hipStream_t stream, unsigned long long *stamps);
bool frame64_on();
void set_frame64(int mode);
long long bneck_frame64_launches();

bool conv_wfrag_supported(int64_t M, int64_t in_bytes, int cin, int cout, int kh, int kw, int pad, int act, int out_f32);
bool conv_wfrag_preferred(int64_t M, int cin, int cout, int kh, int kw);
pvr_status launch_conv_wfrag(const void *in, const void *wp, const float *bias, const void *res, void *out, int n, int h, int w, int cin, int cout,
                             int kh, int kw, int stride, int pad, int act, int out_f32, int dtype, hipStream_t stream, float *pool_out = nullptr,
                             int64_t pool_stride = 0);

struct HostTensor {
    std::vector<int64_t> shape;
    std::vector<float> data;
};

constexpr int PVR_MAX_LANES = 4;
enum BufId { B_NONE = -1, B_X0 = 0, B_X1, B_T1, B_T2, B_DS, B_F32, B_Y0, B_Y1, B_COUNT, B_STEM = B_COUNT };

struct ConvOp {
    std::string conv, bn;
    int in_buf, out_buf, res_buf;
    int h, w, cin, cin_real, cout, cout_real, k, stride, pad, relu, out_f32;
    int kind = 0;
    bool f32op = false;
    bool from32 = false;
    u16 *d_w = nullptr;
    u16 *d_wp = nullptr;
    u16 *d_wfb = nullptr;
    u16 *d_wpb = nullptr;
    std::vector<u16> h_w;
    float *d_wf = nullptr;
    u16 *d_wpk = nullptr;
    u16 *d_wsp_pair = nullptr;
    float *d_b_pair = nullptr;
    u16 *d_wsp = nullptr;
    float *d_b = nullptr;
    std::vector<float> h_b;
    float *d_bsum = nullptr;
    u16 *d_wcat = nullptr;
    std::string tap;
    int ksplit = 0, ks_buf = B_NONE;
};

struct Launch {
    int conv2 = -1, conv3 = -1, next1 = -1;
    int ds = -1;
    int t1_in = B_NONE, t1_out = B_NONE;
    int wave = 0;
    int conv1 = -1;
    int frame = 0;
    int pair = -1;
    int in_blk = 0, out_blk = 0;
};

enum LaunchKind : uint8_t {
    LK_CONV = 0,
    LK_FRAME_FRONT1,
    LK_FRAME,
    LK_FRAME_RUN,
    LK_FRAME_RUN_TAIL,
    LK_FRAME_MEMBERS,
    LK_DUAL,
    LK_DUAL_MEMBERS,
    LK_CHAIN,
    LK_CAST,
    LK_F32,
    LK_SPLIT16,
    LK_SPLIT16_PAIR,
    LK_SPLIT16_IN32,
    LK_SPLITK_SMALL,
    LK_SPLITK,
    LK_EXPAND_BLOCKED,
    LK_WFRAG_POOL,
    LK_WFRAG,
};
const char *launch_kind_name(int k);

struct PlanSwitches {
    int pool_fuse = 1;
    int stem_u8 = 1;
    int stem_lds = 1;
    int frame_front1 = 1;
    int frame_next1 = 0;
    int dual_ds = 1;
    int chain_ds = 1;
    int chain_blocked = 1;
    int splitk = 1;
    int smallk_div = 4;
    int frame_run = 0;
    int frame_stagger = 0;
    int frame_min_n = 128;
    int stem_conv1 = 1;
    int split16 = 1;
    int resid32 = 1;
    int tail_f32 = 1;
    int fuse = 1;
};

}

using namespace pvr;

namespace pvr { struct HostPlan; }

struct pvr_encoder {
    pvr_encoder_desc desc;
    std::map<std::string, HostTensor> weights;
    std::vector<ConvOp> ops;
    std::vector<Launch> sched_plain, sched_fused;
    bool fuse = true;
    bool low_latency = false;
    PlanSwitches sw;
    int stem_c1 = -1;
    int stem_c1_blk = 0;
    u16 *d_stem_c1w = nullptr;
    std::vector<uint8_t> kinds;
    size_t kinds_stride = 0;
    int kinds_algo = -2;
    int *range_flags = nullptr;
    bool last_pooled = false;
    float *d_smallk[PVR_MAX_LANES] = {nullptr};
    bool tail32 = false;
    bool resid32 = false;
    bool finalized = false;
    int out_size = 0;
    int final_hw = 0, final_c = 0, final_creal = 0;
    u16 *d_img = nullptr, *d_stem = nullptr, *d_pool = nullptr, *d_stem_w = nullptr, *d_zero = nullptr;
    float *d_stem_b = nullptr, *d_stem_wf = nullptr, *d_imgf = nullptr;
    void *d_buf[B_COUNT] = {nullptr};
    size_t buf_elems = 0;
    struct LaneWs { u16 *d_img = nullptr, *d_stem = nullptr; float *d_imgf = nullptr; void *d_buf[B_COUNT] = {nullptr}; bool valid = false; } lane_ws[PVR_MAX_LANES];
    int cur_lane = 0;
    hipEvent_t lane_done[PVR_MAX_LANES] = {nullptr};
    hipStream_t lane_stream[PVR_MAX_LANES] = {nullptr};
    int crop_pos = 0;
    int span_first = -1, span_last = -1;
    int last_n = 0;
    std::string stop_after;
    std::map<std::string, std::pair<int, std::vector<int>>> taps;
    struct pvr_vit *resizer = nullptr;
    u16 *ap_wqkv = nullptr, *ap_wc = nullptr;
    float *ap_bqkv = nullptr, *ap_bc = nullptr, *ap_pos = nullptr, *ap_out = nullptr;
    struct pvr_vit *vit = nullptr;
    bool host = false;
    struct pvr::HostPlan *hplan = nullptr;
    struct pvr_random5 *rnd = nullptr;
};


namespace pvr {
const HostTensor *enc_find(pvr_encoder *e, const std::string &name);
pvr_status enc_need(pvr_encoder *e, const std::string &name, const HostTensor **out, size_t numel);
template <typename T>
pvr_status enc_upload(T **dptr, const std::vector<T> &h) {
    PVR_HIP_TRY(hipMalloc((void **)dptr, h.size() * sizeof(T)));
    PVR_HIP_TRY(hipMemcpy(*dptr, h.data(), h.size() * sizeof(T), hipMemcpyHostToDevice));
    return PVR_OK;
}
pvr_status launch_conv_f32(const float *, const float *, const float *, const float *, float *, int, int, int, int, int, int, int, int, int, hipStream_t);
pvr_status launch_stem_f32(const float *, const float *, const float *, float *, int, int, hipStream_t);
pvr_status launch_maxpool_f32(const float *, float *, int, int, int, int, hipStream_t);
pvr_status launch_normalize_nhwc4(const void *img_h, float *out, int n, int crop, const float *mean, const float *std_, int dtype, hipStream_t);
pvr_status random5_create(pvr_encoder *e);
pvr_status random5_finalize(pvr_encoder *e);
pvr_status random5_forward(pvr_encoder *e, const uint8_t *frames, int n, int h, int w, float *out, int64_t out_stride, hipStream_t st);
void random5_destroy(pvr_encoder *e);
pvr_status host_finalize(pvr_encoder *e);
pvr_status host_forward(pvr_encoder *e, const uint8_t *frames, int n, int h, int w, float *out, int64_t out_stride);
void host_destroy(pvr_encoder *e);
pvr_status vit_create(pvr_encoder *e);
pvr_status vit_finalize(pvr_encoder *e);
pvr_status vit_use_lane(pvr_encoder *e, int lane);
pvr_status resizer_create(pvr_encoder *e);
pvr_status resizer_run(pvr_encoder *e, int lane, const uint8_t *frames, int nb, int h, int w, hipStream_t st, const uint8_t **u8, int *oh, int *ow);
void resizer_destroy(pvr_encoder *e);
pvr_status launch_attention(const void *qkv, void *out, int T, int W, int heads, int nb, int dtype, hipStream_t st);
pvr_status launch_avgpool2(const void *in, void *out, int n, int h, int w, int c, int dtype, hipStream_t st);
pvr_status launch_attnpool_tokens(const float *x, const float *pos, void *tokens, int n, int hw, int c, int dtype, hipStream_t st);
pvr_status launch_stem(const void *, const void *, const float *, void *, int, int, int, hipStream_t);
pvr_status vit_forward(pvr_encoder *e, const uint8_t *frames, int n, int h, int w, float *out, int64_t out_stride, hipStream_t st);
void vit_destroy(pvr_encoder *e);
pvr_status vit_tap(pvr_encoder *e, const char *name, float *out, int64_t cap, int64_t *count, hipStream_t st);
}
```

Measured before the change: 99190.

## Store only stride-2 subsampled chain output when its sole reader is a strided downsample

```diff
diff --git a/include/pvr_hip.h b/include/pvr_hip.h
--- a/include/pvr_hip.h
+++ b/include/pvr_hip.h
@@ -117,6 +117,7 @@
                              int32_t h, int32_t w, int32_t cin, int32_t cout, int32_t k, int32_t stride, int32_t pad, int32_t relu, void *hip_stream);
 int64_t pvr_debug_conv_split16_launches(void);
 int64_t pvr_debug_chain_wave128_launches(void);
+int64_t pvr_debug_chain_strided_y_launches(void);
 pvr_status pvr_debug_set_stem_regpool(int32_t mode);
 pvr_status pvr_debug_set_conv_algo(int32_t algo);
 pvr_status pvr_file_sizes(const char *const *paths, int32_t n, int64_t *sizes, int32_t threads);
diff --git a/pvr_habitat_amd/_lib.py b/pvr_habitat_amd/_lib.py
--- a/pvr_habitat_amd/_lib.py
+++ b/pvr_habitat_amd/_lib.py
@@ -72,6 +72,7 @@
     'pvr_debug_conv_split16_launches': (C.c_int64, []),
     'pvr_debug_set_stem_regpool': (C.c_int, [C.c_int32]),
     'pvr_debug_chain_wave128_launches': (C.c_int64, []),
+    'pvr_debug_chain_strided_y_launches': (C.c_int64, []),
     'pvr_op_nonfinite_flag': (C.c_int, [C.c_void_p, C.c_int64, C.c_int64, C.c_int64, C.c_void_p, C.c_void_p]),
 }
 
diff --git a/pvr_habitat_amd/csrc/api.hip b/pvr_habitat_amd/csrc/api.hip
--- a/pvr_habitat_amd/csrc/api.hip
+++ b/pvr_habitat_amd/csrc/api.hip
@@ -72,6 +72,7 @@
 void set_stem_regpool(int v);
 long long conv_split16_launches();
 long long chain_wave128_launches();
+long long chain_wave_y_s2_launches();
 pvr_status launch_split16_pack(const float *w, void *out, int rows, int K, hipStream_t stream);
 pvr_status launch_conv_split16(const float *in, const void *wsp, const float *bias, const float *res, float *out, int n, int h, int w, int cin,
                                int cout, int k, int stride, int pad, int relu, hipStream_t stream, float *out2 = nullptr, int n1 = 0, void *out16 = nullptr,
@@ -167,6 +168,7 @@
     return PVR_OK;
 }
 int64_t pvr_debug_chain_wave128_launches(void) { return (int64_t)chain_wave128_launches(); }
+int64_t pvr_debug_chain_strided_y_launches(void) { return (int64_t)chain_wave_y_s2_launches(); }
 int64_t pvr_debug_pp_persistent_launches(void) { return (int64_t)pp_persistent_launches(); }
 
 size_t pvr_last_error(char *buf, size_t cap) {
diff --git a/pvr_habitat_amd/csrc/bottleneck_chain.hip b/pvr_habitat_amd/csrc/bottleneck_chain.hip
--- a/pvr_habitat_amd/csrc/bottleneck_chain.hip
+++ b/pvr_habitat_amd/csrc/bottleneck_chain.hip
@@ -599,10 +599,12 @@
 pvr_status launch_bottleneck_chain(const void *t1, const void *w2, const float *b2, const void *w3p, const float *b3, const void *res,
                                    void *y, const void *w1np, const float *b1n, void *t1n, int n, int h, int w, int cm, int cmn,
                                    int stride, int dtype, hipStream_t stream, const void *xds, const void *wdsp, const void *w3pb, const void *wdspb,
-                                   int wave, int in_blk, int out_blk, const void *wpk) {
+                                   int wave, int in_blk, int out_blk, const void *wpk, int y_s2) {
     PVR_REQUIRE(chain_supported(cm, cmn), "bottleneck chain: unsupported widths Cm=%d next=%d", cm, cmn);
     PVR_REQUIRE(t1 && w2 && b2 && w3p && b3 && (res || xds) && y && (cmn == 0 || (w1np && b1n && t1n)), "bottleneck chain: null argument");
     PVR_REQUIRE(!xds || (wdsp && chain_ds_supported(cm, cmn, 64, stride)), "bottleneck chain with downsample: unsupported shape");
+    PVR_REQUIRE(!y_s2 || (wave == 1 && chain_wave_y_s2_supported(cm, cmn, stride, xds != nullptr, out_blk, h, w)),
+                "bottleneck chain: no strided-y form for Cm=%d next=%d stride=%d %dx%d", cm, cmn, stride, h, w);
     ChainP p;
     p.in = (const u16 *)t1; p.w2 = (const u16 *)w2; p.w3 = (const u16 *)w3p; p.w1n = (const u16 *)w1np; p.res = (const u16 *)res;
     p.b2 = b2; p.b3 = b3; p.b1n = b1n; p.y = (u16 *)y; p.t1n = (u16 *)t1n;
@@ -623,6 +625,7 @@
     if (wave) {
         PVR_REQUIRE(chain_wave_supported(cm, cmn, stride, xds != nullptr), "bottleneck chain: no wave form for Cm=%d next=%d stride=%d", cm, cmn, stride);
         p.w3b = (const u16 *)w3pb; p.wdsb = (const u16 *)wdspb; p.in_blk = in_blk; p.out_blk = out_blk;
+        p.y_s2 = y_s2; p.ys_bytes = y_s2 ? (unsigned)(yb / 4) : 0;
         return launch_chain_wave(p, cmn, dtype, stream);
     }
     PVR_REQUIRE(!(in_blk || out_blk) || M % 16 == 0, "bottleneck chain: the blocked layout needs a multiple of 16 pixels");
diff --git a/pvr_habitat_amd/csrc/chain_params.h b/pvr_habitat_amd/csrc/chain_params.h
--- a/pvr_habitat_amd/csrc/chain_params.h
+++ b/pvr_habitat_amd/csrc/chain_params.h
@@ -17,6 +17,8 @@
     const u16 *wpk = nullptr;
     unsigned wpk_bytes = 0;
     int t_blk = 0;
+    int y_s2 = 0;
+    unsigned ys_bytes = 0;
 };
 
 bool chain_supported(int cm, int cmn);
@@ -27,12 +29,13 @@
                                    void *y, const void *w1np, const float *b1n, void *t1n, int n, int h, int w, int cm, int cmn,
                                    int stride, int dtype, hipStream_t stream, const void *xds = nullptr, const void *wdsp = nullptr,
                                    const void *w3pb = nullptr, const void *wdspb = nullptr, int wave = 0, int in_blk = 0, int out_blk = 0,
-                                   const void *wpk = nullptr);
+                                   const void *wpk = nullptr, int y_s2 = 0);
 
 
 bool chain_wave_supported(int cm, int cmn, int stride, bool ds);
 bool chain_wave_blocked_ok(int cmn_first, int h, int w);
 bool chain_wave_halo_enabled();
+bool chain_wave_y_s2_supported(int cm, int cmn, int stride, bool ds, int out_blk, int h, int w);
 pvr_status launch_chain_wave(ChainP &p, int cmn, int dtype, hipStream_t stream);
 
 bool chain_wave128_supported(int cm, int cmn, int stride, int64_t M);
diff --git a/pvr_habitat_amd/csrc/chain_wave.hip b/pvr_habitat_amd/csrc/chain_wave.hip
--- a/pvr_habitat_amd/csrc/chain_wave.hip
+++ b/pvr_habitat_amd/csrc/chain_wave.hip
@@ -63,7 +63,7 @@
     int xs[2];
 };
 
-template <int CMN, bool INB, bool OUTB>
+template <int CMN, bool INB, bool OUTB, bool YS2>
 __device__ __forceinline__ void cw_setup(CwTile &a, int m0, int lane, int M, int H, int W) {
     const int fr = lane & 15, fq = lane >> 4, lp = lane >> 2, lc = (lane & 3) ^ ((lane >> 3) & 3);
     a.hb = ((m0 >> 4) - 4) * 2048 + fq * 256 + fr * 16;
@@ -88,11 +88,19 @@
         const int blk = (m0 >> 4) + j;
         a.yi[j] = INB ? blk * 8192 + fq * 256 + fr * 16 : (m0 + 16 * j + lp) * 512 + lc * 16;
         a.yo[j] = OUTB ? blk * 8192 + fq * 256 + fr * 16 : (m0 + 16 * j + (lane >> 3)) * 512 + (((lane & 7) ^ (lane >> 3)) << 4);
+        if constexpr (YS2) {
+            const int ym = m0 + 16 * j + (lane >> 3), hw = H * W;
+            const int yn = ym / hw, yr = ym - yn * hw, yh = yr / W, yw = yr - yh * W;
+            const int c = (yn * (H >> 1) + (yh >> 1)) * (W >> 1) + (yw >> 1);
+            const bool st_lo = ym < M && !((yh | yw) & 1);
+            const bool st_hi = ym + 8 < M && !(yw & 1) && !(((yw + 8 < W) ? yh : yh + 1) & 1);
+            a.yo[j] = (c * 512 + (((lane & 7) ^ (lane >> 3)) << 4)) | (st_lo ? 1 << 29 : 0) | (st_hi ? 1 << 30 : 0);
+        }
         a.to[j] = OUTB ? blk * (CMN * 32) + fq * 256 + fr * 16 : (m0 + 16 * j + (lane >> 3)) * (CMN * 2) + (((lane & 7) ^ (lane >> 3)) << 4);
     }
 }
 
-template <int CMN, bool F16, bool DS, bool W3G, bool INB, bool OUTB, bool HALO, int XD, int RD, int WD>
+template <int CMN, bool F16, bool DS, bool W3G, bool INB, bool OUTB, bool HALO, int XD, int RD, int WD, bool YS2 = false>
 __global__ __launch_bounds__(512, 2) void chain_wave_kernel(ChainP p) {
     typedef typename HT<F16>::V8 V8;
     constexpr int WW = 56, HB = 10;
@@ -104,6 +112,8 @@
     constexpr int YH = INB ? 1024 : 64;
     static_assert(XD >= 1 && XD <= NK && RD >= 1 && RD <= NH && NH % RD == 0 && WD >= 1 && WD <= NH, "prefetch depths (the residual ring must close over a tile)");
     static_assert(!HALO || INB, "the halo form reads the blocked layout");
+    static_assert(!YS2 || !OUTB, "the compact stride-2 y is NHWC");
+    constexpr int YOOB = 0x40000000;
     extern __shared__ __attribute__((aligned(16))) char smem[];
 
     const int tid = threadIdx.x, lane = tid & 63, wave = tid >> 6, fr = lane & 15, fq = lane >> 4;
@@ -115,7 +125,7 @@
     const auto rs_w1 = __builtin_amdgcn_make_buffer_rsrc(const_cast<u16 *>(p.w1n), 0, p.w1n_bytes, 0x00020000);
     const auto rs_res = __builtin_amdgcn_make_buffer_rsrc(const_cast<u16 *>(DS ? p.xds : p.res), 0, DS ? p.xds_bytes : p.y_bytes, 0x00020000);
     const auto rs_wd = __builtin_amdgcn_make_buffer_rsrc(const_cast<u16 *>(DS ? p.wdsb : p.w3b), 0, DS ? p.wds_bytes : p.w3_bytes, 0x00020000);
-    const auto rs_y = __builtin_amdgcn_make_buffer_rsrc(p.y, 0, p.y_bytes, 0x00020000);
+    const auto rs_y = __builtin_amdgcn_make_buffer_rsrc(p.y, 0, YS2 ? p.ys_bytes : p.y_bytes, 0x00020000);
     const auto rs_t = __builtin_amdgcn_make_buffer_rsrc(p.t1n, 0, p.t1n_bytes, 0x00020000);
 
 #pragma unroll
@@ -154,7 +164,7 @@
     const int Wb = p.W * 128;
 
     CwTile cur, nxt;
-    cw_setup<CMN, INB, OUTB>(cur, chunk * 256 + wave * 32, lane, p.M, p.H, p.W);
+    cw_setup<CMN, INB, OUTB, YS2>(cur, chunk * 256 + wave * 32, lane, p.M, p.H, p.W);
 
     u32x4 xr[HALO ? 1 : XD][2];
     u32x4 xh[HALO ? HB : 1][2];
@@ -278,7 +288,7 @@
             }
         }
 
-        cw_setup<CMN, INB, OUTB>(nxt, more ? chunk_n * 256 + wave * 32 : ((p.M + 31) & ~31), lane, p.M, p.H, p.W);
+        cw_setup<CMN, INB, OUTB, YS2>(nxt, more ? chunk_n * 256 + wave * 32 : ((p.M + 31) & ~31), lane, p.M, p.H, p.W);
         if (!more) nxt.hb = OOB;
         if constexpr (HALO) CW_ISSUE_HALO(nxt)
         else {
@@ -373,8 +383,14 @@
                 else if (h & 1) {
                     u32x4 lo, hi;
                     cw_f2m_pair(slot0, lane, oe[j], o[j], lo, hi);
-                    cw_store(lo, rs_y, cur.yo[j], (h >> 1) * 128, p.stride == 77);
-                    cw_store(hi, rs_y, cur.yo[j], (h >> 1) * 128 + 8 * 512, p.stride == 77);
+                    if constexpr (YS2) {
+                        const int yb = cur.yo[j] & 0x1fffffff;
+                        cw_store(lo, rs_y, ((cur.yo[j] >> 29) & 1) ? yb : YOOB, (h >> 1) * 128, p.stride == 77);
+                        cw_store(hi, rs_y, ((cur.yo[j] >> 30) & 1) ? yb + 4 * 512 : YOOB, (h >> 1) * 128, p.stride == 77);
+                    } else {
+                        cw_store(lo, rs_y, cur.yo[j], (h >> 1) * 128, p.stride == 77);
+                        cw_store(hi, rs_y, cur.yo[j], (h >> 1) * 128 + 8 * 512, p.stride == 77);
+                    }
                 } else oe[j] = o[j];
             }
             if constexpr (CMN > 0) {
@@ -432,12 +448,12 @@
     return v;
 }
 
-template <int CMN, bool F16, bool DS, bool W3G, bool INB, bool OUTB, bool HALO, int XD, int RD, int WD>
+template <int CMN, bool F16, bool DS, bool W3G, bool INB, bool OUTB, bool HALO, int XD, int RD, int WD, bool YS2 = false>
 static pvr_status launch_cw_one(ChainP &p, hipStream_t stream) {
     const size_t lds = (size_t)(W3G ? 73728 : 73728 + 32768) + (size_t)CMN * 512 + 256 + 1024 + 512 + 8 * 2048;
     static DeviceOnce attr_done;
     if (attr_done.needed()) {
-        PVR_HIP_TRY(hipFuncSetAttribute((const void *)chain_wave_kernel<CMN, F16, DS, W3G, INB, OUTB, HALO, XD, RD, WD>, hipFuncAttributeMaxDynamicSharedMemorySize, (int)lds));
+        PVR_HIP_TRY(hipFuncSetAttribute((const void *)chain_wave_kernel<CMN, F16, DS, W3G, INB, OUTB, HALO, XD, RD, WD, YS2>, hipFuncAttributeMaxDynamicSharedMemorySize, (int)lds));
         attr_done.mark();
     }
     const int nch = (p.M + 255) / 256;
@@ -445,7 +461,7 @@
     if (grid < 8) grid = 8;
     const int need = ((nch + 7) / 8) * 8;
     if (grid > need) grid = need;
-    hipLaunchKernelGGL((chain_wave_kernel<CMN, F16, DS, W3G, INB, OUTB, HALO, XD, RD, WD>), dim3(grid), dim3(512), lds, stream, p);
+    hipLaunchKernelGGL((chain_wave_kernel<CMN, F16, DS, W3G, INB, OUTB, HALO, XD, RD, WD, YS2>), dim3(grid), dim3(512), lds, stream, p);
     PVR_LAUNCH_CHECK();
     return PVR_OK;
 }
@@ -469,6 +485,10 @@
         if (!ib && ob) return launch_cw_one<64, F16, false, false, false, true, false, 4, 4, 1>(p, stream);
         return halo ? launch_cw_one<64, F16, false, false, true, false, true, 1, 4, 1>(p, stream)
                     : launch_cw_one<64, F16, false, false, true, false, false, 4, 4, 1>(p, stream);
+    } else if (cmn == 128 && !ob && p.y_s2) {
+        if (halo) return launch_cw_one<128, F16, false, true, true, false, true, 1, 1, 1, true>(p, stream);
+        return ib ? launch_cw_one<128, F16, false, true, true, false, false, 3, 4, 2, true>(p, stream)
+                  : launch_cw_one<128, F16, false, true, false, false, false, 3, 4, 2, true>(p, stream);
     } else if (cmn == 128 && !ob) {
         if (halo) return launch_cw_one<128, F16, false, true, true, false, true, 1, 1, 1>(p, stream);
         return ib ? launch_cw_one<128, F16, false, true, true, false, false, 3, 4, 2>(p, stream)
@@ -478,7 +498,8 @@
                             : launch_cw_one<0, F16, false, false, true, false, false, 4, 4, 1>(p, stream);
         return launch_cw_one<0, F16, false, false, false, false, false, 4, 4, 1>(p, stream);
     }
-    set_error("bottleneck chain (wave form): no instance for next Cm=%d%s, blocked in/out %d/%d", cmn, p.xds ? " with downsample" : "", (int)ib, (int)ob);
+    set_error("bottleneck chain (wave form): no instance for next Cm=%d%s, blocked in/out %d/%d%s", cmn, p.xds ? " with downsample" : "", (int)ib, (int)ob,
+              p.y_s2 ? ", strided y" : "");
     return PVR_ERR_INVALID;
 }
 
@@ -491,12 +512,20 @@
 
 bool chain_wave_blocked_ok(int cmn_first, int h, int w) { return cmn_first == 64 && (h * w) % 32 == 0; }
 bool chain_wave_halo_enabled() { return cw_halo() != 0; }
+bool chain_wave_y_s2_supported(int cm, int cmn, int stride, bool ds, int out_blk, int h, int w) {
+    return chain_wave_supported(cm, cmn, stride, ds) && cmn == 128 && !ds && !out_blk && h % 2 == 0 && w % 2 == 0 && w >= 8;
+}
+
+static long long g_y_s2_launches = 0;
+long long chain_wave_y_s2_launches() { return g_y_s2_launches; }
 
 pvr_status launch_chain_wave(ChainP &p, int cmn, int dtype, hipStream_t stream) {
     PVR_REQUIRE((int64_t)(p.M + 64) * 512 < 0x7ffffff0ll, "bottleneck chain (wave form): operand larger than 2 GiB (use a smaller chunk)");
     PVR_REQUIRE(p.xds ? p.wdsb != nullptr : (cmn != 128 || p.w3b != nullptr), "bottleneck chain (wave form): the blocked copy of W3 / Wd is missing");
     PVR_REQUIRE(!(p.in_blk || p.out_blk) || p.M % 32 == 0, "bottleneck chain (wave form): the blocked layout needs a multiple of 32 pixels");
-    return dtype == PVR_F16 ? launch_cw_dt<true>(p, cmn, stream) : launch_cw_dt<false>(p, cmn, stream);
-}
-
-}
+    const pvr_status s = dtype == PVR_F16 ? launch_cw_dt<true>(p, cmn, stream) : launch_cw_dt<false>(p, cmn, stream);
+    if (!s && p.y_s2) ++g_y_s2_launches;
+    return s;
+}
+
+}
diff --git a/pvr_habitat_amd/csrc/encoder.hip b/pvr_habitat_amd/csrc/encoder.hip
--- a/pvr_habitat_amd/csrc/encoder.hip
+++ b/pvr_habitat_amd/csrc/encoder.hip
@@ -29,6 +29,7 @@
     sw.resid32 = get("PVR_RESID32", 1);
     sw.tail_f32 = get("PVR_TAIL_F32", 1);
     sw.fuse = get("PVR_FUSE", 1);
+    sw.strided_y = get("PVR_STRIDED_Y", 1);
 }
 
 template <bool F32>
@@ -616,6 +617,35 @@
             }
         }
     }
+    if (e->sw.strided_y) {
+        std::vector<Launch> &sc = e->sched_fused;
+        auto members = [](const Launch &l) { return std::vector<int>{l.conv1, l.conv2, l.ds, l.conv3, l.pair, l.next1}; };
+        for (size_t a = 0; a < sc.size(); ++a) {
+            Launch &A = sc[a];
+            if (A.conv3 < 0 || A.next1 < 0 || A.frame || A.wave != 1 || A.ds >= 0) continue;
+            const ConvOp &a2 = e->ops[A.conv2], &a3 = e->ops[A.conv3];
+            if (a3.out_f32 || !chain_wave_y_s2_supported(a2.cout, e->ops[A.next1].cout, a2.stride, false, A.out_blk, a3.h, a3.w)) continue;
+            const int y = a3.out_buf;
+            int reader = -1;
+            bool ok = true, done = false;
+            for (size_t b = a + 1; b < sc.size() && ok && !done; ++b) {
+                for (int oi : members(sc[b])) {
+                    if (oi < 0) continue;
+                    const ConvOp &o = e->ops[oi];
+                    if (o.in_buf == y || o.res_buf == y) {
+                        const Launch &B = sc[b];
+                        const bool ds_alone = B.conv3 < 0 && B.ds < 0 && B.pair < 0 && B.conv1 < 0 && B.next1 < 0 && !B.frame && oi == B.conv2;
+                        if (reader < 0 && ds_alone && ends_with(o.conv, ".downsample.0") && o.kind == 0 && !o.f32op && !o.from32 && o.k == 1 && o.stride == 2 &&
+                            o.pad == 0 && o.in_buf == y && o.res_buf != y && o.ksplit <= 1 && o.h == a3.h && o.w == a3.w && o.cin == a3.cout && o.tap.empty())
+                            reader = (int)b;
+                        else ok = false;
+                    }
+                    if (o.out_buf == y) { done = true; break; }
+                }
+            }
+            if (ok && reader >= 0) A.y_s2_reader = reader;
+        }
+    }
     return PVR_OK;
 }
 
@@ -1048,6 +1078,7 @@
         int launch_idx = 0;
         const bool run_ok = enc->stop_after.empty() && !enc->range_flags;
         const int stop_idx = enc->stop_after.size() > 1 && enc->stop_after[0] == '#' ? atoi(enc->stop_after.c_str() + 1) : -1;
+        int ys2_reader = -1;
         auto member = [&](const ConvOp &o, const void *in, const void *r_, void *out_) -> pvr_status {
             if (const int ks = small_batch_ksplit(enc, o, nb)) {
                 if (!smallk) { set_error("low-latency plan without its scratch (pvr_encoder_set_low_latency allocates it)"); return PVR_ERR_STATE; }
@@ -1119,11 +1150,13 @@
                 const ConvOp &c2 = enc->ops[l.conv2];
                 const ConvOp *c1 = l.next1 >= 0 ? &enc->ops[l.next1] : nullptr;
                 const ConvOp *cd = l.ds >= 0 ? &enc->ops[l.ds] : nullptr;
+                const bool ys2 = l.y_s2_reader >= 0 && run_ok && kinds[l.y_s2_reader] == LK_CONV;
+                ys2_reader = ys2 ? l.y_s2_reader : -1;
                 s = launch_bottleneck_chain(enc->d_buf[l.t1_in], c2.d_w, c2.d_b, op.d_wp, cd ? op.d_bsum : op.d_b, res, enc->d_buf[op.out_buf],
                                             c1 ? c1->d_wp : nullptr, c1 ? c1->d_b : nullptr, c1 ? enc->d_buf[l.t1_out] : nullptr, nb,
                                             c2.h, c2.w, c2.cout, c1 ? c1->cout : 0, c2.stride, dt, st,
                                             cd ? enc->d_buf[cd->in_buf] : nullptr, cd ? cd->d_wp : nullptr, op.d_wpb, cd ? cd->d_wpb : nullptr,
-                                            l.wave, cd ? (l.in_blk && t1_blocked) : l.in_blk, l.out_blk, c2.d_wpk);
+                                            l.wave, cd ? (l.in_blk && t1_blocked) : l.in_blk, l.out_blk, c2.d_wpk, ys2 ? 1 : 0);
                 t1_blocked = false;
                 break;
             }
@@ -1169,8 +1202,12 @@
                                       op.stride, op.pad, op.relu, op.out_f32, dt, st);
                 break;
             default:
-                s = launch_conv(enc->d_buf[op.in_buf], op.d_w, op.d_b, res, enc->d_buf[op.out_buf], enc->d_zero, nb, op.h, op.w,
-                                op.cin, op.cout, op.k, op.k, op.stride, op.pad, op.relu, op.out_f32, dt, st);
+                if ((int)li == ys2_reader)
+                    s = launch_conv(enc->d_buf[op.in_buf], op.d_w, op.d_b, res, enc->d_buf[op.out_buf], enc->d_zero, nb, op.h / 2, op.w / 2,
+                                    op.cin, op.cout, 1, 1, 1, 0, op.relu, op.out_f32, dt, st);
+                else
+                    s = launch_conv(enc->d_buf[op.in_buf], op.d_w, op.d_b, res, enc->d_buf[op.out_buf], enc->d_zero, nb, op.h, op.w,
+                                    op.cin, op.cout, op.k, op.k, op.stride, op.pad, op.relu, op.out_f32, dt, st);
             }
             if (s) return s;
             if (enc->range_flags && kind != LK_WFRAG_POOL) {
diff --git a/pvr_habitat_amd/csrc/encoder_internal.h b/pvr_habitat_amd/csrc/encoder_internal.h
--- a/pvr_habitat_amd/csrc/encoder_internal.h
+++ b/pvr_habitat_amd/csrc/encoder_internal.h
@@ -104,6 +104,7 @@
     int frame = 0;
     int pair = -1;
     int in_blk = 0, out_blk = 0;
+    int y_s2_reader = -1;
 };
 
 enum LaunchKind : uint8_t {
@@ -148,6 +149,7 @@
     int resid32 = 1;
     int tail_f32 = 1;
     int fuse = 1;
+    int strided_y = 1;
 };
 
 }
```

Result: faster. 100,800, median of 6 (+1.6%).
